# yknishidate/single-file-vulkan-pathtracing

Hardware: AMD Instinct MI355X
Metric: Mrays/s, Cornell Box 1920x1080 @ 8 bounces (ms/frame in ms_per_step) (higher is better)
Workload: dtype f32; 1 GPU; C2: CornellBox-Original.obj 1920x1080, 32 spp/frame x 771 frames, 8 bounces, fused pipeline (library default); pipeline=fused

## Files before the change

single-file-vulkan-pathtracing_amd/csrc/aov.hip:

```cpp
#include "wavefront_host.h"

#include <algorithm>

#define PT_EXTEND_TEMPLATES_ONLY
#include "extend_kernel.h"

namespace {
using namespace ptw;

struct AovConst {
    ptm::Camera cam;
    float tmin, tmax;
    uint32_t width, height, spp;
    FastDiv div_spp;
    uint32_t cull_on;
    int32_t cull[4];
};
struct AovPlanes {
    float *albedo, *normal, *emission, *depth, *alpha;
    uint2 *id;
};
constexpr size_t AOV_RAY_BYTES = sizeof(float4) + sizeof(float2) + sizeof(float4) + sizeof(uint32_t);
constexpr size_t AOV_MAX_CHUNK_RAYS = (size_t)1 << 26;
constexpr uint32_t AOV_NEXT_TILE = 32;

__device__ __forceinline__ void tile_pixel(const uint32_t *__restrict__ tiles, uint32_t pix, uint32_t &px, uint32_t &py)
{
    const uint32_t g = tiles[pix >> 6];
    px = (g & 0xFFFFu) * 8u + (pix & 7u);
    py = (g >> 16) * 8u + ((pix >> 3) & 7u);
}

struct Guide {
    float ar, ag, ab, nx, ny, nz, er, eg, eb, d, a;
};
__device__ __forceinline__ void guide_add(Guide &g, const Guide &v)
{
    g.ar = g.ar + v.ar; g.ag = g.ag + v.ag; g.ab = g.ab + v.ab;
    g.nx = g.nx + v.nx; g.ny = g.ny + v.ny; g.nz = g.nz + v.nz;
    g.er = g.er + v.er; g.eg = g.eg + v.eg; g.eb = g.eb + v.eb;
    g.d = g.d + v.d; g.a = g.a + v.a;
}
__device__ __forceinline__ float blend1(float sum, float spp, float old, bool first, float ff, float f1)
{
    return ptm::fdiv(ptm::fdiv(sum, spp) + (first ? 0.f : old) * ff, f1);
}
__device__ __forceinline__ void guide_blend(Guide &acc, const Guide &sum, float spp, int32_t frame)
{
    const float ff = (float)frame, f1 = (float)(frame + 1);
    const bool first = frame == 0;
    acc.ar = blend1(sum.ar, spp, acc.ar, first, ff, f1); acc.ag = blend1(sum.ag, spp, acc.ag, first, ff, f1); acc.ab = blend1(sum.ab, spp, acc.ab, first, ff, f1);
    acc.nx = blend1(sum.nx, spp, acc.nx, first, ff, f1); acc.ny = blend1(sum.ny, spp, acc.ny, first, ff, f1); acc.nz = blend1(sum.nz, spp, acc.nz, first, ff, f1);
    acc.er = blend1(sum.er, spp, acc.er, first, ff, f1); acc.eg = blend1(sum.eg, spp, acc.eg, first, ff, f1); acc.eb = blend1(sum.eb, spp, acc.eb, first, ff, f1);
    acc.d = blend1(sum.d, spp, acc.d, first, ff, f1); acc.a = blend1(sum.a, spp, acc.a, first, ff, f1);
}
__device__ __forceinline__ Guide guide_load(const AovPlanes &pl, size_t pix)
{
    Guide g;
    g.ar = pl.albedo[3 * pix + 0]; g.ag = pl.albedo[3 * pix + 1]; g.ab = pl.albedo[3 * pix + 2];
    g.nx = pl.normal[3 * pix + 0]; g.ny = pl.normal[3 * pix + 1]; g.nz = pl.normal[3 * pix + 2];
    g.er = pl.emission[3 * pix + 0]; g.eg = pl.emission[3 * pix + 1]; g.eb = pl.emission[3 * pix + 2];
    g.d = pl.depth[pix]; g.a = pl.alpha[pix];
    return g;
}
__device__ __forceinline__ void guide_store(const AovPlanes &pl, size_t pix, const Guide &g)
{
    pl.albedo[3 * pix + 0] = g.ar; pl.albedo[3 * pix + 1] = g.ag; pl.albedo[3 * pix + 2] = g.ab;
    pl.normal[3 * pix + 0] = g.nx; pl.normal[3 * pix + 1] = g.ny; pl.normal[3 * pix + 2] = g.nz;
    pl.emission[3 * pix + 0] = g.er; pl.emission[3 * pix + 1] = g.eg; pl.emission[3 * pix + 2] = g.eb;
    pl.depth[pix] = g.d; pl.alpha[pix] = g.a;
}

__global__ __launch_bounds__(TB) void k_aov_generate(AovConst ac, const uint32_t *__restrict__ tiles, uint32_t n_rays, int32_t frame,
                                                     float4 *__restrict__ rayA, float2 *__restrict__ rayB, uint32_t *__restrict__ count)
{
    for (uint32_t r = blockIdx.x * TB + threadIdx.x; r < n_rays; r += gridDim.x * TB) {
        const uint32_t pix = ac.div_spp.div(r), s = r - pix * ac.spp;
        uint32_t px, py;
        tile_pixel(tiles, pix, px, py);
        uint32_t seed = ptm::make_seed(px, py, s, frame, ac.spp);
        ptm::f3 org, dir;
        ptm::primary_ray(ac.cam, px, py, seed, org, dir);
        ptm::st_stream<true>(rayA + r, make_float4(org.x, org.y, org.z, dir.x));
        ptm::st_stream<true>(rayB + r, make_float2(dir.y, dir.z));
    }
    if (blockIdx.x == 0 && threadIdx.x == 0) *count = n_rays;
}

template <bool INST>
__global__ __launch_bounds__(TB) void k_aov_reduce(AovConst ac, const uint32_t *__restrict__ tiles, uint32_t n_pix, int32_t frame, int last_frame,
                                                   const float4 *__restrict__ hit, const uint32_t *__restrict__ hit_inst,
                                                   const float4 *__restrict__ tri4, const float4 *__restrict__ rec64,
                                                   const float *__restrict__ faces, const float4 *__restrict__ inst6,
                                                   const float4 *__restrict__ inst_frame, const uint32_t *__restrict__ inst_id, uint32_t n_tris,
                                                   AovPlanes planes, unsigned long long *stats, unsigned long long n_valid_rays)
{
    if (blockIdx.x == 0 && threadIdx.x == 0 && stats) atomicAdd(stats, n_valid_rays);
    const uint32_t pix = blockIdx.x * TB + threadIdx.x;
    if (pix >= n_pix) return;
    uint32_t px, py;
    tile_pixel(tiles, pix, px, py);
    if (px >= ac.width || py >= ac.height) return;
    Guide sum = {};
    uint2 id = make_uint2(PT_MISS, PT_MISS);
    for (uint32_t s = 0; s < ac.spp; s++) {
        const size_t r = (size_t)pix * ac.spp + s;
        const float4 h = ptm::ld_stream<true>(hit + r);
        const uint32_t pos = __float_as_uint(h.x);
        Guide v = {};
        if (pos != PT_MISS) {
            const uint32_t prim = __float_as_uint(tri4[3 * (size_t)pos].w);
            const float *f = faces + 6 * (size_t)prim;
            ptm::f3 nrm = { rec64[4 * (size_t)pos + 0].w, rec64[4 * (size_t)pos + 1].w, rec64[4 * (size_t)pos + 2].w };
            uint32_t inst = 0u;
            if (INST) {
                const uint32_t ip = hit_inst[r];
                inst = inst_id[ip];
                if (inst_frame) {
                    const float4 f0 = inst_frame[2 * ((size_t)ip * n_tris + pos)];
                    nrm = { f0.x, f0.y, f0.z };
                } else {
                    const float4 i0 = inst6[6 * (size_t)ip + 3], i1 = inst6[6 * (size_t)ip + 4], i2 = inst6[6 * (size_t)ip + 5];
                    const float nx = (i0.x * nrm.x + i1.x * nrm.y) + i2.x * nrm.z;
                    const float ny = (i0.y * nrm.x + i1.y * nrm.y) + i2.y * nrm.z;
                    const float nz = (i0.z * nrm.x + i1.z * nrm.y) + i2.z * nrm.z;
                    const float l = ptm::fsqrt((nx * nx + ny * ny) + nz * nz);
                    nrm = { ptm::fdiv(nx, l), ptm::fdiv(ny, l), ptm::fdiv(nz, l) };
                }
            }
            v = { f[0], f[1], f[2], nrm.x, nrm.y, nrm.z, f[3], f[4], f[5], h.y, 1.0f };
            if (s == 0u) id = make_uint2(prim, inst);
        }
        guide_add(sum, v);
    }
    const size_t o = (size_t)py * ac.width + px;
    Guide acc = {};
    if (frame != 0) acc = guide_load(planes, o);
    guide_blend(acc, sum, (float)ac.spp, frame);
    guide_store(planes, o, acc);
    if (last_frame) planes.id[o] = id;
}

constexpr int AOV_START_IDLE = 16;
#ifndef PT_AOV_WAVES
#define PT_AOV_WAVES 4
#endif
template <bool PAIRS>
__global__ __launch_bounds__(TB, PT_AOV_WAVES) void k_aov_fused(AovConst ac_arg, const uint32_t *__restrict__ tiles, uint32_t n_tiles, int32_t frame0, uint32_t n_frames,
                                                  const float4 *__restrict__ g_wide, const float4 *__restrict__ g_tri4,
                                                  const float4 *__restrict__ g_shade4, const float *__restrict__ g_faces, uint32_t n_wide,
                                                  uint32_t n_tris, int lds_stack, AovPlanes planes_arg, uint32_t *next_tile,
                                                  unsigned long long *stats)
{
    const AovConst ac = ptm::own_sgprs(ac_arg);
    const AovPlanes planes = ptm::own_sgprs(planes_arg);
    constexpr uint32_t LEAF_BIT = C14_LEAF, DONE = C14_DONE;
    extern __shared__ __attribute__((aligned(16))) char smem[];
    float4 *s_wide = reinterpret_cast<float4 *>(smem + (size_t)lds_stack * TB * sizeof(uint32_t));
    float4 *s_tri = s_wide + LDS_NODE_F4 * (size_t)n_wide;
    float4 *s_rec = s_tri + 9 * (size_t)n_tris;
    lds_stage_nodes<TB, true>(s_wide, g_wide, n_wide);
    lds_stage_tris<TB>(s_tri, g_tri4, n_tris);
    for (uint32_t pos = threadIdx.x; pos < n_tris; pos += TB) {
        const float4 n = g_shade4[3 * (size_t)pos];
        const float prim_bits = g_tri4[3 * (size_t)pos].w;
        const float *f = g_faces + 6 * (size_t)__float_as_uint(prim_bits);
        s_rec[3 * pos + 0] = make_float4(n.x, n.y, n.z, prim_bits);
        s_rec[3 * pos + 1] = make_float4(f[0], f[1], f[2], f[3]);
        s_rec[3 * pos + 2] = make_float4(f[4], f[5], 0.f, 0.f);
    }
    __syncthreads();
    const float4 *wide = s_wide, *tri4 = s_tri;
    lds_u32 *my_stack32 = (lds_u32 *)reinterpret_cast<uint32_t *>(smem) + threadIdx.x;
    const int lane = threadIdx.x & 63;
    const float tmin = ac.tmin, tmax = ac.tmax;
    const float fspp = (float)ac.spp;
    unsigned long long n_rays_wave = 0, n_cull_wave = 0;

    for (;;) {
        uint32_t t = 0;
        if (lane == 0) t = atomicAdd(next_tile, 1u);
        t = (uint32_t)__builtin_amdgcn_readfirstlane((int)t);
        if (t >= n_tiles) break;
        uint32_t px, py;
        tile_pixel(tiles, t * 64u + (uint32_t)lane, px, py);
        const bool valid = px < ac.width && py < ac.height;
        const uint32_t o = py * ac.width + px;
        const bool culled = ac.cull_on && ((int32_t)px < ac.cull[0] || (int32_t)px > ac.cull[2] || (int32_t)py < ac.cull[1] || (int32_t)py > ac.cull[3]);
        n_rays_wave += (unsigned long long)__popcll(__ballot(valid)) * ac.spp * n_frames;
        n_cull_wave += (unsigned long long)__popcll(__ballot(valid && culled)) * ac.spp * n_frames;
        for (uint32_t k = 0; k < n_frames; k++) {
            const int32_t frame = frame0 + (int32_t)k;
            Guide sum = {};
            uint32_t s = valid && !culled ? 0u : ac.spp;
            bool have = false;
            ptm::f3 inv{}, invf{}, on{}, of{}, orgp{};
            ptm::RayPre pre{};
            uint32_t ax = 0, ay = 0, az = 0, tri_base = 0;
            float best_t = tmax, best_V = 0.f, best_W = 0.f, best_det = 1.f;
            uint32_t best_pos = PT_MISS, best_prim = PT_MISS;
            uint32_t cur = DONE;
            int sp = 0;
            auto pop = [&]() -> uint32_t {
                while (sp > 0) {
                    sp--;
                    const uint32_t e = my_stack32[sp * TB];
                    if (__uint_as_float(e & 0xFFFFC000u) <= best_t) return e & 0x3FFFu;
                }
                return DONE;
            };
            for (;;) {
                const bool wants = !have && s < ac.spp;
                const int n_idle = __popcll(__ballot(wants)), n_have = __popcll(__ballot(have));
                if (n_idle == 0 && n_have == 0) break;
                if (wants && (n_idle >= AOV_START_IDLE || n_have == 0)) {
                    uint32_t seed = ptm::make_seed(px, py, s, frame, ac.spp);
                    ptm::f3 org, dir;
                    ptm::primary_ray(ac.cam, px, py, seed, org, dir);
                    pre = ptm::ray_setup<PAIRS>(org, dir);
                    inv = { ptm::safe_inv(dir.x), ptm::safe_inv(dir.y), ptm::safe_inv(dir.z) };
                    slab_setup(org, inv, invf, on, of);
                    ax = inv.x < 0.f ? 48u : 0u; ay = inv.y < 0.f ? 48u : 0u; az = inv.z < 0.f ? 48u : 0u;
                    tri_base = (uint32_t)pre.kz * 3u * n_tris;
                    orgp = { ptm::sel3(pre.kz, org.y, org.z, org.x), ptm::sel3(pre.kz, org.z, org.x, org.y), ptm::sel3(pre.kz, org.x, org.y, org.z) };
                    best_t = tmax; best_V = 0.f; best_W = 0.f; best_det = 1.f;
                    best_pos = PT_MISS; best_prim = PT_MISS;
                    cur = 0u;
                    sp = 0;
                    have = true;
                }
                bool do_node = have && !(cur & LEAF_BIT);
                const int n_walk = __popcll(__ballot(have));
                while (do_node) {
                    cur = compact_node_step<TB>(wide, cur, inv, invf, on, of, ax, ay, az, tmin, best_t, my_stack32, sp, pop);
                    do_node = !(cur & LEAF_BIT);
                    if (__popcll(__ballot(do_node)) * 6 < n_walk) break;
                }
                if (have) {
                    if (cur != DONE && (cur & LEAF_BIT)) {
                        const uint32_t first = cur & 0x7FFu;
                        if (PAIRS) {
                            const bool two = ((cur >> 11) & 3u) != 0u;
                            ptl::pair_leaf_test(tri4, (size_t)tri_base + 3 * (size_t)first, two, first, pre, orgp, tmin, tmax,
                                                [&](float t_, float V, float W, float det, uint32_t pos, uint32_t) {
                                                    ptl::closer_single_level(tri4, tri_base, t_, V, W, det, pos, best_t, best_V, best_W, best_det, best_pos);
                                                },
                                                [] {});
                        } else {
                            const uint32_t cnt = ((cur >> 11) & 3u) + 1u;
                            for (uint32_t j = 0; j < cnt; j++) {
                                const uint32_t pos = first + j;
                                const size_t ti = (size_t)tri_base + 3 * (size_t)pos;
                                const float4 a = tri4[ti + 0], b = tri4[ti + 1], c = tri4[ti + 2];
                                float t_, V, W, det;
                                if (ptm::tri_test_perm(pre, orgp, { a.x, a.y, a.z }, { b.x, b.y, b.z }, { c.x, c.y, c.z }, tmin, tmax, t_, V, W, det, nullptr)) {
                                    const uint32_t prim = __float_as_uint(a.w);
                                    if (t_ < best_t || (t_ == best_t && prim < best_prim)) {
                                        best_t = t_; best_V = V; best_W = W; best_det = det; best_pos = pos; best_prim = prim;
                                    }
                                }
                            }
                        }
                        cur = pop();
                    }
                    if (cur == DONE) {
                        Guide v = {};
                        if (best_pos != PT_MISS) {
                            const float4 r0 = s_rec[3 * best_pos + 0], r1 = s_rec[3 * best_pos + 1], r2 = s_rec[3 * best_pos + 2];
                            v = { r1.x, r1.y, r1.z, r0.x, r0.y, r0.z, r1.w, r2.x, r2.y, best_t, 1.0f };
                            if (s == 0u && k + 1u == n_frames) planes.id[o] = make_uint2(__float_as_uint(r0.w), 0u);
                        } else if (s == 0u && k + 1u == n_frames) {
                            planes.id[o] = make_uint2(PT_MISS, PT_MISS);
                        }
                        guide_add(sum, v);
                        s++;
                        have = false;
                    }
                }
            }
            if (valid && culled && k + 1u == n_frames) planes.id[o] = make_uint2(PT_MISS, PT_MISS);
            if (valid) {
                Guide acc = {};
                if (frame != 0) acc = guide_load(planes, o);
                guide_blend(acc, sum, fspp, frame);
                guide_store(planes, o, acc);
            }
        }
    }
    if (lane == 0 && n_rays_wave && stats) atomicAdd(stats, n_rays_wave);
    if (lane == 0 && n_cull_wave && stats) atomicAdd(stats + 19, n_cull_wave);
}

pt_status ensure_tiles(pt_film *f, uint32_t rank, uint32_t world)
{
    pt_film::Aov &a = f->aov;
    if (a.d_tiles && a.rank == rank && a.world == world) return PT_OK;
    std::vector<uint32_t> tiles;
    std::vector<uint64_t> prefix;
    const uint64_t valid = pt_rank_tiles(f->w, f->h, rank, world, &tiles, &prefix);
    const size_t held = a.d_tiles ? sizeof(uint32_t) * std::max<size_t>(a.n_tiles, 1) : 0;
    a.n_tiles = 0;
    const pt_status rc = pt_scratch_alloc(f->ctx, "guide-buffer workspace", { pt_buf_of(a.d_tiles, sizeof(uint32_t) * std::max<size_t>(tiles.size(), 1)) }, &a.bytes, held);
    if (rc != PT_OK) return rc;
    if (!tiles.empty()) PT_HIP(f->ctx, hipMemcpy(a.d_tiles, tiles.data(), sizeof(uint32_t) * tiles.size(), hipMemcpyHostToDevice));
    a.rank = rank; a.world = world; a.n_tiles = (uint32_t)tiles.size(); a.valid_pixels = valid;
    a.h_valid.swap(prefix);
    return PT_OK;
}

pt_status ensure_count(pt_film *f)
{
    pt_film::Aov &a = f->aov;
    if (a.d_count) return PT_OK;
    return pt_scratch_alloc(f->ctx, "guide-buffer workspace", { pt_buf_of(a.d_count, sizeof(uint32_t) * 64) }, &a.bytes, 0);
}

pt_status ensure_rays(pt_film *f, size_t rays)
{
    pt_film::Aov &a = f->aov;
    if (rays <= a.cap_rays) return PT_OK;
    const size_t held = a.cap_rays * AOV_RAY_BYTES;
    a.cap_rays = 0;
    const pt_status rc = pt_scratch_alloc(f->ctx, "guide-buffer workspace", { pt_buf_of(a.d_rayA, sizeof(float4) * rays), pt_buf_of(a.d_rayB, sizeof(float2) * rays),
                                                                              pt_buf_of(a.d_hit, sizeof(float4) * rays), pt_buf_of(a.d_hit_inst, sizeof(uint32_t) * rays) }, &a.bytes, held);
    if (rc == PT_OK) a.cap_rays = rays;
    return rc;
}

AovPlanes planes_of(const pt_film *f)
{
    const pt_film::Aov &a = f->aov;
    return { static_cast<float *>(a.plane[PT_AOV_ALBEDO]), static_cast<float *>(a.plane[PT_AOV_NORMAL]), static_cast<float *>(a.plane[PT_AOV_EMISSION]),
             static_cast<float *>(a.plane[PT_AOV_DEPTH]), static_cast<float *>(a.plane[PT_AOV_ALPHA]), static_cast<uint2 *>(a.plane[PT_AOV_ID]) };
}

struct AovFusedPlan { size_t smem = 0; int grid = 0; bool pairs = false; };
using AovFusedFn = decltype(&k_aov_fused<true>);
AovFusedFn pick_aov_fused(bool pairs) { return pairs ? k_aov_fused<true> : k_aov_fused<false>; }
pt_status plan_aov_fused(pt_scene *s, const pt_params *p, const ExtendPlan &pl, AovFusedPlan &fp)
{
    pt_ctx *ctx = s->ctx;
    const size_t smem = pl.smem + sizeof(float4) * 3 * (size_t)s->n_tris;
    if (s->n_inst || p->extend != PT_EXTEND_AUTO || pl.variant != PT_EXTEND_LDS || pl.spill || !(p->tmin > 0.f) || smem > 64 * 1024) {
        ctx->err = "pt_render_aov: PT_PIPELINE_FUSED is for single-level scenes whose BVH4 and triangles live in LDS (the compact kernels' class: <= 24 KB, "
                   "stack bound <= 16), tmin > 0 and params.extend = PT_EXTEND_AUTO";
        return PT_ERR_UNSUPPORTED;
    }
    fp.smem = smem;
    fp.pairs = pl.pairs;
    int per_cu = 0;
    const pt_status rc = ptw_prepare_kernel(ctx, reinterpret_cast<const void *>(pick_aov_fused(pl.pairs)), TB, smem, &per_cu);
    fp.grid = ctx->num_cus * per_cu;
    return rc;
}

pt_status render_aov_fused(pt_scene *s, pt_film *f, const pt_params *p, const ExtendPlan &pl, const AovFusedPlan &fp, const AovConst &ac)
{
    pt_ctx *ctx = s->ctx;
    pt_film::Aov &a = f->aov;
    hipStream_t st = ctx->stream;
    if (a.n_tiles == 0) return PT_OK;
    PT_HIP(ctx, hipMemsetAsync(a.d_count + AOV_NEXT_TILE, 0, sizeof(uint32_t), st));
    const int grid = (int)std::min<uint32_t>((uint32_t)fp.grid, (a.n_tiles + TB / 64 - 1) / (TB / 64));
    hipLaunchKernelGGL(pick_aov_fused(fp.pairs), dim3(grid), dim3(TB), (uint32_t)fp.smem, st, ac, a.d_tiles, a.n_tiles, p->frame, p->frame_count, s->d_wide, s->d_tri4,
                       s->d_shade4, s->d_faces, s->n_wide, s->n_tris, pl.lds_stack, planes_of(f), a.d_count + AOV_NEXT_TILE, ctx->d_stats);
    PT_HIP(ctx, hipGetLastError());
    ctx->stats.launches_extend++;
    return PT_OK;
}

pt_status render_aov_queues(pt_scene *s, pt_film *f, const pt_params *p, const ExtendPlan &pl, const AovConst &ac)
{
    pt_ctx *ctx = s->ctx;
    pt_film::Aov &a = f->aov;
    hipStream_t st = ctx->stream;
    if (a.n_tiles == 0) return PT_OK;
    const float4 *inst_frame = nullptr;
    if (s->n_inst && ctx->tune.inst_frames != 0) {
        const pt_status rcf = ptb_ensure_inst_frames(s);
        if (rcf != PT_OK) return rcf;
        inst_frame = s->d_inst_frame;
    }
    const size_t tile_rays = 64 * (size_t)p->spp_per_frame;
    const size_t held = f->work.bytes + (a.bytes - a.cap_rays * AOV_RAY_BYTES);
    size_t fit_rays = AOV_MAX_CHUNK_RAYS;
    if (ctx->mem_budget) fit_rays = std::min(fit_rays, ctx->mem_budget > held ? (ctx->mem_budget - held) / AOV_RAY_BYTES : 0);
    size_t chunk_tiles = std::min<size_t>(a.n_tiles, fit_rays / tile_rays);
    if (chunk_tiles == 0) {
        if (ctx->mem_budget && tile_rays * AOV_RAY_BYTES + held > ctx->mem_budget) {
            ctx->err = "guide-buffer workspace exceeds the memory budget (" + std::to_string((held + tile_rays * AOV_RAY_BYTES) >> 20) + " MB wanted for one tile, " +
                       std::to_string(ctx->mem_budget >> 20) + " MB allowed)";
            return PT_ERR_OOM;
        }
        chunk_tiles = 1;
    }
    pt_status rc = ensure_rays(f, chunk_tiles * tile_rays);
    if (rc != PT_OK) return rc;
    const AovPlanes planes = planes_of(f);
    const float4 *tri4 = pl.bvh8 ? s->d_tri4_8 : s->d_tri4, *rec64 = pl.bvh8 ? s->d_shade64_8 : s->d_shade64;
    for (uint32_t k = 0; k < p->frame_count; k++) {
        const int32_t frame = p->frame + (int32_t)k;
        const int last = k + 1 == p->frame_count ? 1 : 0;
        for (uint32_t t0 = 0; t0 < a.n_tiles; t0 += (uint32_t)chunk_tiles) {
            const uint32_t nt = std::min<uint32_t>((uint32_t)chunk_tiles, a.n_tiles - t0);
            const uint32_t n_pix = nt * 64u, n_rays = n_pix * p->spp_per_frame;
            const unsigned long long valid = a.h_valid[t0 + nt] - a.h_valid[t0];
            const int grid_g = (int)std::min<uint32_t>((n_rays + TB - 1) / TB, (uint32_t)ctx->num_cus * 32u);
            k_aov_generate<<<grid_g, TB, 0, st>>>(ac, a.d_tiles + t0, n_rays, frame, a.d_rayA, a.d_rayB, a.d_count);
            ptw_launch_extend(pl, s, a.d_rayA, a.d_rayB, a.d_hit, a.d_hit_inst, a.d_count, nullptr, nullptr, p->tmin, p->tmax, false, false, st);
            const int grid_r = (int)((n_pix + TB - 1) / TB);
            if (s->n_inst)
                k_aov_reduce<true><<<grid_r, TB, 0, st>>>(ac, a.d_tiles + t0, n_pix, frame, last, a.d_hit, a.d_hit_inst, tri4, rec64, s->d_faces, s->d_inst6, inst_frame,
                                                          s->d_tlas_prim_of, s->n_tris, planes, ctx->d_stats, valid * p->spp_per_frame);
            else
                k_aov_reduce<false><<<grid_r, TB, 0, st>>>(ac, a.d_tiles + t0, n_pix, frame, last, a.d_hit, nullptr, tri4, rec64, s->d_faces, nullptr, nullptr, nullptr,
                                                           s->n_tris, planes, ctx->d_stats, valid * p->spp_per_frame);
            PT_HIP(ctx, hipGetLastError());
            ctx->stats.launches_extend++;
            ctx->stats.launches_other += 2;
        }
    }
    return PT_OK;
}

}

size_t pta_plane_bytes(const pt_film *f, uint32_t which)
{
    const size_t n = (size_t)f->w * f->h;
    return which <= PT_AOV_EMISSION ? sizeof(float) * 3 * n : which <= PT_AOV_ALPHA ? sizeof(float) * n : sizeof(uint32_t) * 2 * n;
}

pt_status pta_enable(pt_film *f, void *const *device_planes)
{
    pt_ctx *ctx = f->ctx;
    pt_film::Aov &a = f->aov;
    if (a.enabled) { ctx->err = "the film already has guide buffers"; return PT_ERR_INVALID_ARG; }
    for (uint32_t k = 0; k < PT_AOV_COUNT; k++) {
        void *ext = device_planes ? device_planes[k] : nullptr;
        a.own[k] = ext == nullptr;
        a.plane[k] = ext;
        if (!ext) {
            const hipError_t e = hipMalloc(&a.plane[k], pta_plane_bytes(f, k));
            if (e != hipSuccess) {
                (void)hipGetLastError();
                a.plane[k] = nullptr;
                ctx->err = std::string("hipMalloc: ") + hipGetErrorString(e);
                pta_free(f);
                return PT_ERR_OOM;
            }
        }
    }
    a.enabled = true;
    const pt_status rc = pta_clear(f, ctx->stream);
    if (rc != PT_OK) { pta_free(f); return rc; }
    PT_HIP(ctx, hipStreamSynchronize(ctx->stream));
    return PT_OK;
}

pt_status pta_clear(pt_film *f, hipStream_t st)
{
    if (!f->aov.enabled) return PT_OK;
    for (uint32_t k = 0; k < PT_AOV_COUNT; k++) PT_HIP(f->ctx, hipMemsetAsync(f->aov.plane[k], 0, pta_plane_bytes(f, k), st));
    return PT_OK;
}

void pta_free(pt_film *f)
{
    pt_film::Aov &a = f->aov;
    for (uint32_t k = 0; k < PT_AOV_COUNT; k++) {
        if (a.own[k] && a.plane[k]) (void)hipFree(a.plane[k]);
        a.plane[k] = nullptr;
        a.own[k] = false;
    }
    pt_scratch_free({ pt_buf_of(a.d_tiles), pt_buf_of(a.d_rayA), pt_buf_of(a.d_rayB), pt_buf_of(a.d_hit), pt_buf_of(a.d_hit_inst), pt_buf_of(a.d_count) },
                    &a.bytes, a.bytes);
    a = pt_film::Aov{};
}

pt_status pta_render(pt_scene *s, pt_film *f, const pt_params *p)
{
    pt_ctx *ctx = s->ctx;
    pt_status rc = s->broken ? ptb_repair(s) : PT_OK;
    if (rc != PT_OK) return rc;
    if (!f->aov.enabled) { ctx->err = "the film has no guide buffers: pt_film_enable_aov first"; return PT_ERR_INVALID_ARG; }
    if (p->width != f->w || p->height != f->h) { ctx->err = "params width/height differ from the film's"; return PT_ERR_INVALID_ARG; }
    if (p->world == 0 || p->rank >= p->world) { ctx->err = "rank/world invalid"; return PT_ERR_INVALID_ARG; }
    if (p->spp_per_frame == 0 || p->spp_per_frame > 0xFFFFu) { ctx->err = "spp_per_frame must be in 1..65535"; return PT_ERR_INVALID_ARG; }
    if (p->frame < 0 || p->frame_count == 0) { ctx->err = "frame must be >= 0 and frame_count >= 1"; return PT_ERR_INVALID_ARG; }
    if (p->pipeline > PT_PIPELINE_AUTO) { ctx->err = "unknown pipeline"; return PT_ERR_UNSUPPORTED; }
    if (p->pipeline == PT_PIPELINE_WAVEFRONT_NEE) { ctx->err = "pt_render_aov: the guides do not depend on the estimator (PT_PIPELINE_WAVEFRONT, _FUSED or _AUTO)"; return PT_ERR_UNSUPPORTED; }
    if (p->flags & ~(uint32_t)PT_FLAG_NEE) { ctx->err = "pt_render_aov takes no flag but PT_FLAG_NEE (ignored): blocking, not instrumented"; return PT_ERR_UNSUPPORTED; }
    ExtendPlan pl;
    rc = ptw_plan_extend(s, p->extend, pl);
    if (rc != PT_OK) return rc;
    AovFusedPlan fp;
    bool fused = false;
    if (p->pipeline != PT_PIPELINE_WAVEFRONT) {
        const std::string keep = ctx->err;
        rc = plan_aov_fused(s, p, pl, fp);
        if (rc == PT_OK) fused = true;
        else if (p->pipeline == PT_PIPELINE_FUSED) return rc;
        else ctx->err = keep;
    }
    ctx->stats.pipeline = fused ? PT_PIPELINE_FUSED : PT_PIPELINE_WAVEFRONT;
    rc = ensure_tiles(f, p->rank, p->world);
    if (rc == PT_OK) rc = ensure_count(f);
    if (rc != PT_OK) return rc;
    AovConst ac{};
    ac.cam = ptw_camera(p);
    ac.tmin = p->tmin; ac.tmax = p->tmax;
    ac.width = p->width; ac.height = p->height; ac.spp = p->spp_per_frame;
    ac.div_spp.init(p->spp_per_frame);
    if (fused && ctx->tune.cull != 0) {
        int32_t rect[4];
        ptw_subject_rect(s, p, rect);
        ac.cull_on = rect[2] >= rect[0] && rect[3] >= rect[1] ? 1u : 0u;
        std::copy(rect, rect + 4, ac.cull);
    }
    hipStream_t st = ctx->stream;
    PT_HIP(ctx, hipEventRecord(ctx->ev_a, st));
    rc = fused ? render_aov_fused(s, f, p, pl, fp, ac) : render_aov_queues(s, f, p, pl, ac);
    if (rc != PT_OK) { (void)hipStreamSynchronize(st); return rc; }
    PT_HIP(ctx, hipEventRecord(ctx->ev_b, st));
    PT_HIP(ctx, hipStreamSynchronize(st));
    PT_HIP(ctx, hipGetLastError());
    float ms = 0.f;
    PT_HIP(ctx, hipEventElapsedTime(&ms, ctx->ev_a, ctx->ev_b));
    ctx->stats.ms_total += ms;
    ctx->stats.paths += f->aov.valid_pixels * p->spp_per_frame * p->frame_count;
    return PT_OK;
}
```

single-file-vulkan-pathtracing_amd/csrc/extend_inst.h:

```cpp
#pragma once
#include "extend_kernel.h"

namespace {

constexpr uint32_t EXIT_MARK = 0x7FFFFFFFu;

template <bool COUNT, bool LDS_BLAS, bool SHADOW = false>
__global__ __launch_bounds__(TB) void k_extend_inst(const float4 *__restrict__ tlas, const float4 *__restrict__ g_blas,
                                                    const float4 *__restrict__ g_tri4, uint32_t n_blas_wide,
                                                    uint32_t n_tris, const float4 *__restrict__ inst6,
                                                    const uint32_t *__restrict__ inst_id, const float4 *__restrict__ rayA,
                                                    const float2 *__restrict__ rayB, float4 *__restrict__ hit,
                                                    uint32_t *__restrict__ hit_inst, const uint32_t *__restrict__ count_in,
                                                    uint32_t *count_zero, unsigned long long *stats,
                                                    uint2 *__restrict__ spill, uint32_t spill_stride, int refill_min_idle,
                                                    float tmin, float tmax, int raw_hit, const float *__restrict__ ray_tmax)
{
    extern __shared__ __attribute__((aligned(16))) char smem[];
    uint2 *stack = reinterpret_cast<uint2 *>(smem);
    const float4 *blas = g_blas;
    const float4 *tri4 = g_tri4;
    if (LDS_BLAS) {
        float4 *s_blas = reinterpret_cast<float4 *>(smem + (size_t)LDS_STACK * TB * sizeof(uint2));
        float4 *s_tri = s_blas + LDS_NODE_F4 * (size_t)n_blas_wide;
        lds_stage_nodes<TB, false>(s_blas, g_blas, n_blas_wide);
        lds_stage_tris<TB>(s_tri, g_tri4, n_tris);
        __syncthreads();
        blas = s_blas;
        tri4 = s_tri;
    }
    const uint32_t n = *count_in;
    if (blockIdx.x == 0 && threadIdx.x == 0) {
        if (count_zero) *count_zero = 0u;
        if (stats) atomicAdd(stats, (unsigned long long)n);
    }
    lds_u64 *my_stack = (lds_u64 *)reinterpret_cast<unsigned long long *>(stack) + threadIdx.x;
    unsigned long long *my_spill = reinterpret_cast<unsigned long long *>(spill) + (size_t)blockIdx.x * TB + threadIdx.x;
    const float INF = __builtin_inff();
    const int lane = threadIdx.x & 63;
    const unsigned long long lt = (1ull << lane) - 1ull;

    bool have = false, exhausted = false, in_blas = false;
    uint32_t q = 0;
    ptm::f3 org_w{}, dir_w{}, inv_w{};
    ptm::f3 inv{}, invf{}, on{}, of{}, orgp{};
    uint32_t tri_base = 0;
    uint32_t ax = 0, ay = 0, az = 0;
    ptm::RayPre pre{};
    float best_t = tmax, best_V = 0.f, best_W = 0.f, best_det = 1.f;
    uint32_t best_pos = PT_MISS, best_prim = PT_MISS, best_ipos = PT_MISS, best_iid = PT_MISS;
    uint32_t cur = SENTINEL, cur_ipos = 0, cur_iid = 0;
    float cur_t = 0.f;
    int sp = 0;
    unsigned long long c_nodes = 0, c_tris = 0;
    const uint32_t wave_base = (blockIdx.x * (TB / 64) + (threadIdx.x >> 6)) * 64u;
    const uint32_t wave_stride = gridDim.x * TB;
    uint32_t cursor = 0;

    auto push = [&](uint32_t w, float t) {
        const unsigned long long e = stack_entry(w, t);
        if (sp < LDS_STACK) my_stack[sp * TB] = e;
        else my_spill[(size_t)(sp - LDS_STACK) * spill_stride] = e;
        sp++;
    };
    auto pop = [&]() -> uint32_t {
        while (sp > 0) {
            sp--;
            unsigned long long e64;
            if (sp < LDS_STACK) e64 = my_stack[sp * TB];
            else e64 = my_spill[(size_t)(sp - LDS_STACK) * spill_stride];
            const uint2 e = make_uint2((uint32_t)e64, (uint32_t)(e64 >> 32));
            if (e.x == EXIT_MARK) {
                inv = inv_w;
                slab_setup(org_w, inv_w, invf, on, of);
                ax = inv.x < 0.f ? 48u : 0u;
                ay = inv.y < 0.f ? 48u : 0u;
                az = inv.z < 0.f ? 48u : 0u;
                in_blas = false;
                continue;
            }
            if (__uint_as_float(e.y) <= best_t) {
                cur_t = __uint_as_float(e.y);
                return e.x;
            }
        }
        return SENTINEL;
    };

    for (;;) {
        const unsigned long long idle = __ballot(!have);
        const int n_idle = __popcll(idle);
        if (!exhausted && n_idle >= refill_min_idle) {
            if (!have) {
                const uint32_t v = cursor + (uint32_t)__popcll(idle & lt);
                const uint32_t qq = (v >> 6) * wave_stride + wave_base + (v & 63u);
                if (qq < n) {
                    q = qq;
                    const float4 ra = rayA[q];
                    const float2 rb = rayB[q];
                    org_w = { ra.x, ra.y, ra.z };
                    dir_w = { ra.w, rb.x, rb.y };
                    inv_w = { ptm::safe_inv(dir_w.x), ptm::safe_inv(dir_w.y), ptm::safe_inv(dir_w.z) };
                    inv = inv_w;
                    slab_setup(org_w, inv_w, invf, on, of);
                    ax = inv.x < 0.f ? 48u : 0u;
                    ay = inv.y < 0.f ? 48u : 0u;
                    az = inv.z < 0.f ? 48u : 0u;
                    in_blas = false;
                    best_t = SHADOW ? ray_tmax[q] : tmax; best_V = 0.f; best_W = 0.f; best_det = 1.f;
                    best_pos = PT_MISS; best_prim = PT_MISS; best_ipos = PT_MISS; best_iid = PT_MISS;
                    cur = 0u;
                    cur_t = tmin;
                    sp = 0;
                    have = true;
                }
            }
            cursor += (uint32_t)n_idle;
            exhausted = (cursor >> 6) * wave_stride + wave_base >= n;
        }
        if (__ballot(have) == 0ull) break;

        while (have && !(cur & PT_LEAF)) {
            float4 nx, fx, ny, fy, nz, fz, cw;
            if (LDS_BLAS && in_blas) {
                const char *nd = reinterpret_cast<const char *>(blas + LDS_NODE_F4 * (size_t)cur);
                nx = PT_F4(nd + ax); fx = PT_F4(nd - ax + 48); ny = PT_F4(nd + ay + 16); fy = PT_F4(nd - ay + 64);
                nz = PT_F4(nd + az + 32); fz = PT_F4(nd - az + 80); cw = PT_F4(nd + 96);
            } else {
                const char *nd = reinterpret_cast<const char *>((LDS_BLAS ? tlas : (in_blas ? g_blas : tlas)) + 8 * (size_t)cur);
                nx = PT_F4(nd + ax); fx = PT_F4(nd - ax + 48); ny = PT_F4(nd + ay + 16); fy = PT_F4(nd - ay + 64);
                nz = PT_F4(nd + az + 32); fz = PT_F4(nd - az + 80); cw = PT_F4(nd + 96);
            }
            if (COUNT) c_nodes++;
            float t0, t1, t2, t3;
            uint32_t w0 = __float_as_uint(cw.x), w1 = __float_as_uint(cw.y), w2 = __float_as_uint(cw.z),
                     w3 = __float_as_uint(cw.w);
            PT_SLAB4(t0, x)
            PT_SLAB4(t1, y)
            PT_SLAB4(t2, z)
            PT_SLAB4(t3, w)
#define PT_CSWAP(TA, WA, TB_, WB)                            \
    {                                                        \
        const bool sw = TB_ < TA;                            \
        const float ta = sw ? TB_ : TA, tb = sw ? TA : TB_;  \
        const uint32_t wa = sw ? WB : WA, wb = sw ? WA : WB; \
        TA = ta; TB_ = tb; WA = wa; WB = wb;                 \
    }
            PT_CSWAP(t0, w0, t1, w1)
            PT_CSWAP(t2, w2, t3, w3)
            PT_CSWAP(t0, w0, t2, w2)
            PT_CSWAP(t1, w1, t3, w3)
            PT_CSWAP(t1, w1, t2, w2)
#undef PT_CSWAP
            if (t3 < INF) push(w3, t3);
            if (t2 < INF) push(w2, t2);
            if (t1 < INF) push(w1, t1);
            if (t0 < INF) { cur = w0; cur_t = t0; }
            else cur = pop();
        }
        constexpr int ENTER_MIN = 16;
        const int n_enter = __popcll(__ballot(have && cur != SENTINEL && !in_blas));
        const bool others = __ballot(have && cur != SENTINEL && in_blas) != 0ull;
        const bool do_enter = n_enter >= ENTER_MIN || !others;
        if (have) {
            if (cur != SENTINEL && (in_blas || do_enter)) {
                const uint32_t first = cur & 0x0FFFFFFFu, cnt = ((cur >> 28) & 7u) + 1u;
                if (in_blas) {
                    if (COUNT) c_tris += cnt;
                    for (uint32_t k = 0; k < cnt; k++) {
                        const uint32_t pos = first + k;
                        const size_t ti = LDS_BLAS ? (size_t)tri_base + 3 * (size_t)pos : 3 * (size_t)pos;
                        const float4 a = tri4[ti + 0], b = tri4[ti + 1], c = tri4[ti + 2];
                        float t, V, W, det;
                        const bool th = LDS_BLAS
                            ? ptm::tri_test_perm(pre, orgp, { a.x, a.y, a.z }, { b.x, b.y, b.z }, { c.x, c.y, c.z }, tmin, tmax, t, V, W, det)
                            : ptm::tri_test(pre, { a.x, a.y, a.z }, { b.x, b.y, b.z }, { c.x, c.y, c.z }, tmin, tmax, t, V, W, det);
                        if (th) {
                            const uint32_t prim = __float_as_uint(a.w);
                            if (t < best_t || (t == best_t && (cur_iid < best_iid || (cur_iid == best_iid && prim < best_prim)))) {
                                best_t = t; best_V = V; best_W = W; best_det = det; best_pos = pos; best_prim = prim;
                                best_ipos = cur_ipos; best_iid = cur_iid;
                                if (SHADOW) sp = 0;
                            }
                        }
                    }
                    cur = pop();
                } else {
                    for (uint32_t k = cnt - 1u; k >= 1u; k--) push(PT_LEAF | (first + k), cur_t);
                    cur_ipos = first;
                    cur_iid = inst_id[first];
                    const float4 r0 = inst6[6 * (size_t)first + 3], r1 = inst6[6 * (size_t)first + 4],
                                 r2 = inst6[6 * (size_t)first + 5];
                    const ptm::f3 oo = { ((r0.x * org_w.x + r0.y * org_w.y) + r0.z * org_w.z) + r0.w,
                                         ((r1.x * org_w.x + r1.y * org_w.y) + r1.z * org_w.z) + r1.w,
                                         ((r2.x * org_w.x + r2.y * org_w.y) + r2.z * org_w.z) + r2.w };
                    const ptm::f3 od = { (r0.x * dir_w.x + r0.y * dir_w.y) + r0.z * dir_w.z,
                                         (r1.x * dir_w.x + r1.y * dir_w.y) + r1.z * dir_w.z,
                                         (r2.x * dir_w.x + r2.y * dir_w.y) + r2.z * dir_w.z };
                    inv = { ptm::safe_inv(od.x), ptm::safe_inv(od.y), ptm::safe_inv(od.z) };
                    slab_setup(oo, inv, invf, on, of);
                    ax = inv.x < 0.f ? 48u : 0u;
                    ay = inv.y < 0.f ? 48u : 0u;
                    az = inv.z < 0.f ? 48u : 0u;
                    pre = ptm::ray_setup(oo, od);
                    if (LDS_BLAS) {
                        tri_base = (uint32_t)pre.kz * 3u * n_tris;
                        orgp = { ptm::sel3(pre.kz, oo.y, oo.z, oo.x), ptm::sel3(pre.kz, oo.z, oo.x, oo.y),
                                 ptm::sel3(pre.kz, oo.x, oo.y, oo.z) };
                    }
                    push(EXIT_MARK, 0.f);
                    in_blas = true;
                    cur = 0u;
                    cur_t = tmin;
                }
            }
            if (cur == SENTINEL) {
                const bool miss = best_pos == PT_MISS;
                hit[q] = raw_hit ? make_float4(__uint_as_float(best_pos), best_V, best_W, best_det)
                                 : make_float4(__uint_as_float(best_pos), miss ? 0.f : best_t,
                                               miss ? 0.f : ptm::fdiv(best_V, best_det), miss ? 0.f : ptm::fdiv(best_W, best_det));
                if (!SHADOW) hit_inst[q] = best_ipos;
                have = false;
            }
        }
    }
    if (COUNT) {
        for (int o = 32; o > 0; o >>= 1) {
            c_nodes += __shfl_xor(c_nodes, o, 64);
            c_tris += __shfl_xor(c_tris, o, 64);
        }
        if (lane == 0 && stats) {
            atomicAdd(stats + 2, c_nodes);
            atomicAdd(stats + 3, c_tris);
        }
    }
}

}
```

single-file-vulkan-pathtracing_amd/csrc/extend_kernel.h:

```cpp
#pragma once
#include "pt_internal.h"
#include "pt_math.h"
#include "pair_leaf.h"
#include "lds_scene.h"

#include <hip/hip_ext.h>

namespace {

constexpr int LDS_STACK = 8;
typedef __attribute__((address_space(3))) unsigned long long lds_u64;
typedef __attribute__((address_space(3))) uint32_t lds_u32;
__device__ __forceinline__ unsigned long long stack_entry(uint32_t w, float t)
{
    return (unsigned long long)w | ((unsigned long long)__float_as_uint(t) << 32);
}

#define PT_F4(P) (*reinterpret_cast<const float4 *>(P))
#define PT_NODE_LOAD(ND)                                                                                 \
    const char *nb_ = reinterpret_cast<const char *>(ND);                                                \
    const float4 nx = PT_F4(nb_ + ax), fx = PT_F4(nb_ - ax + 48), ny = PT_F4(nb_ + ay + 16),             \
                 fy = PT_F4(nb_ - ay + 64), nz = PT_F4(nb_ + az + 32), fz = PT_F4(nb_ - az + 80),        \
                 cw = PT_F4(nb_ + 96);
#define PT_SLAB4(T, C)                                                                                           \
    {                                                                                                            \
        const float tn = fmaxf(fmaxf(__builtin_fmaf(nx.C, inv.x, on.x), __builtin_fmaf(ny.C, inv.y, on.y)),      \
                               max_raw_s(__builtin_fmaf(nz.C, inv.z, on.z), tmin));                              \
        const float tf = fminf(fminf(__builtin_fmaf(fx.C, invf.x, of.x), __builtin_fmaf(fy.C, invf.y, of.y)),    \
                               min_raw(__builtin_fmaf(fz.C, invf.z, of.z), best_t));                             \
        T = tn <= tf ? tn : INF;                                                                                 \
    }
__device__ __forceinline__ float max_raw_s(float a, float uniform_b)
{
    float r;
    asm("v_max_f32_e32 %0, %1, %2" : "=v"(r) : "s"(uniform_b), "v"(a));
    return r;
}
__device__ __forceinline__ float min_raw(float a, float b)
{
    float r;
    asm("v_min_f32_e32 %0, %1, %2" : "=v"(r) : "v"(a), "v"(b));
    return r;
}

template <int STRIDE, class Pop>
__device__ __forceinline__ uint32_t compact_node_step(const float4 *wide, uint32_t cur, const ptm::f3 &inv, const ptm::f3 &invf, const ptm::f3 &on,
                                                      const ptm::f3 &of, uint32_t ax, uint32_t ay, uint32_t az, float tmin, float best_t,
                                                      lds_u32 *my_stack32, int &sp, Pop &&pop)
{
    const float INF = __builtin_inff();
    float t0, t1, t2, t3;
    const float4 *nd = reinterpret_cast<const float4 *>(reinterpret_cast<const char *>(wide) + __umul24(cur, 16u * LDS_NODE_F4));
    PT_NODE_LOAD(nd)
    const uint32_t w0 = __float_as_uint(cw.x), w1 = __float_as_uint(cw.y), w2 = __float_as_uint(cw.z), w3 = __float_as_uint(cw.w);
    PT_SLAB4(t0, x)
    PT_SLAB4(t1, y)
    PT_SLAB4(t2, z)
    PT_SLAB4(t3, w)
    uint32_t k0 = (__float_as_uint(t0) & 0xFFFFC000u) | w0, k1 = (__float_as_uint(t1) & 0xFFFFC000u) | w1,
             k2 = (__float_as_uint(t2) & 0xFFFFC000u) | w2, k3 = (__float_as_uint(t3) & 0xFFFFC000u) | w3;
#define PT_KSWAP(A, B) { const uint32_t lo_ = min(A, B), hi_ = max(A, B); A = lo_; B = hi_; }
    PT_KSWAP(k0, k1)
    PT_KSWAP(k2, k3)
    PT_KSWAP(k0, k2)
    PT_KSWAP(k1, k3)
    PT_KSWAP(k1, k2)
#undef PT_KSWAP
    constexpr uint32_t KINF = 0x7F800000u;
    if (k3 < KINF) { my_stack32[sp * STRIDE] = k3; sp++; }
    if (k2 < KINF) { my_stack32[sp * STRIDE] = k2; sp++; }
    if (k1 < KINF) { my_stack32[sp * STRIDE] = k1; sp++; }
    return k0 < KINF ? (k0 & 0x3FFFu) : pop();
}
__device__ __forceinline__ void slab_setup(const ptm::f3 org, const ptm::f3 inv, ptm::f3 &invf, ptm::f3 &on, ptm::f3 &of)
{
    const float ox = -(org.x * inv.x), oy = -(org.y * inv.y), oz = -(org.z * inv.z);
    const float px = fabsf(ox) * 0x1p-21f, py = fabsf(oy) * 0x1p-21f, pz = fabsf(oz) * 0x1p-21f;
    on = { ox - px, oy - py, oz - pz };
    of = { (ox + px) * 1.0000004f, (oy + py) * 1.0000004f, (oz + pz) * 1.0000004f };
    invf = { inv.x * 1.0000004f, inv.y * 1.0000004f, inv.z * 1.0000004f };
}
struct NormBox { float cx, cy, cz, sx, sy, sz, rsx, rsy, rsz; };
inline NormBox norm_box(const float *c, const float *s, const float *rs) { return { c[0], c[1], c[2], s[0], s[1], s[2], rs[0], rs[1], rs[2] }; }
inline NormBox norm_box_blas(const pt_scene *s) { return norm_box(s->norm_c, s->norm_s, s->norm_rs); }
inline NormBox norm_box_tlas(const pt_scene *s) { return norm_box(s->tlas_norm_c, s->tlas_norm_s, s->tlas_norm_rs); }
#define PT_MIXH(DST, REG, HI, INVC, ONC) \
    asm("v_fma_mix_f32 %0, %1, %2, %3 op_sel:[" #HI ",0,0] op_sel_hi:[1,0,0]" : "=v"(DST) : "v"(REG), "v"(INVC), "v"(ONC))
#define PT_SLAB4H(T, REGC, HI)                                                                      \
    {                                                                                               \
        float nxv, nyv, nzv, fxv, fyv, fzv;                                                         \
        PT_MIXH(nxv, hnx.REGC, HI, inv.x, on.x); PT_MIXH(nyv, hny.REGC, HI, inv.y, on.y);           \
        PT_MIXH(nzv, hnz.REGC, HI, inv.z, on.z); PT_MIXH(fxv, hfx.REGC, HI, invf.x, of.x);          \
        PT_MIXH(fyv, hfy.REGC, HI, invf.y, of.y); PT_MIXH(fzv, hfz.REGC, HI, invf.z, of.z);         \
        const float tn = fmaxf(fmaxf(nxv, nyv), max_raw_s(nzv, tmin));                              \
        const float tf = fminf(fminf(fxv, fyv), min_raw(fzv, best_t));                              \
        T = tn <= tf ? tn : INF;                                                                    \
    }
#ifndef PT_HBM_SELECT_BFI
#define PT_HBM_SELECT_BFI 1
#endif
#if PT_HBM_SELECT_BFI
#define PT_BFI(M, A, B) (((M) & (A)) | (~(M) & (B)))
#else
#define PT_BFI(M, A, B) ((M) ? (A) : (B))
#endif
#ifndef PT_EXTEND_WAVES
#define PT_EXTEND_WAVES 7
#endif
constexpr int REFILL_MIN_IDLE = 16;

template <bool LDS_SCENE, bool COUNT, bool SPILL, bool PAIRS = false, bool REC64 = false>
__device__ __forceinline__ void extend_body(const float4 *__restrict__ g_wide, const uint2 *__restrict__ g_wide16,
                                               NormBox nb, const float4 *__restrict__ g_tri4,
                                               uint32_t n_wide, uint32_t n_tris, const float4 *__restrict__ rayA,
                                               const float2 *__restrict__ rayB, float4 *__restrict__ hit,
                                               const uint32_t *__restrict__ count_in, uint32_t *count_zero,
                                               unsigned long long *stats, uint2 *__restrict__ spill,
                                               uint32_t spill_stride, int refill_vote, float tmin, float tmax,
                                               int lds_stack, int raw_hit, const uint32_t *__restrict__ perm,
                                               const float *__restrict__ ray_tmax, const float4 *__restrict__ g_rec64 = nullptr)
{
    const int refill_min_idle = refill_vote & 0xFF, tri_enter = (refill_vote >> 8) & 0xFF;
    constexpr bool VOTE = !LDS_SCENE;
    constexpr int VOTE_NODE_NUM = 1, VOTE_NODE_DEN = 1;
    constexpr bool COMPACT = LDS_SCENE && !SPILL;
    static_assert(!PAIRS || COMPACT, "pair leaves are implemented for the compact LDS kernel");
    static_assert(!REC64 || (!LDS_SCENE && SPILL), "64-B triangle records are the vote-scheduled HBM kernel's");
    constexpr uint32_t LEAF_BIT = COMPACT ? C14_LEAF : PT_LEAF;
    constexpr uint32_t DONE = COMPACT ? C14_DONE : SENTINEL;

    extern __shared__ __attribute__((aligned(16))) char smem[];
    uint2 *stack = reinterpret_cast<uint2 *>(smem);
    const float4 *wide = g_wide;
    const float4 *tri4 = g_tri4;
    if (LDS_SCENE) {
        float4 *s_wide = reinterpret_cast<float4 *>(smem + (size_t)lds_stack * TB * (COMPACT ? sizeof(uint32_t) : sizeof(uint2)));
        float4 *s_tri = s_wide + LDS_NODE_F4 * (size_t)n_wide;
        lds_stage_nodes<TB, COMPACT>(s_wide, g_wide, n_wide);
        lds_stage_tris<TB>(s_tri, g_tri4, n_tris);
        __syncthreads();
        wide = s_wide;
        tri4 = s_tri;
    }
    const uint32_t n = *count_in;
    if (blockIdx.x == 0 && threadIdx.x == 0) {
        if (count_zero) *count_zero = 0u;
        if (stats) atomicAdd(stats, (unsigned long long)n);
    }
    lds_u64 *my_stack = (lds_u64 *)reinterpret_cast<unsigned long long *>(stack) + threadIdx.x;
    lds_u32 *my_stack32 = (lds_u32 *)reinterpret_cast<uint32_t *>(stack) + threadIdx.x;
    unsigned long long *my_spill = reinterpret_cast<unsigned long long *>(spill) + (size_t)blockIdx.x * TB + threadIdx.x;
    const float INF = __builtin_inff();
    const int lane = threadIdx.x & 63;
    const unsigned long long lt = (1ull << lane) - 1ull;

    bool have = false, exhausted = false;
    uint32_t q = 0;
    const uint32_t wave_base = (blockIdx.x * (TB / 64) + (threadIdx.x >> 6)) * 64u;
    const uint32_t wave_stride = gridDim.x * TB;
    uint32_t cursor = 0;
    ptm::f3 inv{}, invf{}, on{}, of{}, orgp{};
    ptm::RayPre pre{};
    uint32_t ax = 0, ay = 0, az = 0;
    uint32_t tri_base = 0;
    float best_t = tmax, best_V = 0.f, best_W = 0.f, best_det = 1.f;
    uint32_t best_pos = PT_MISS, best_prim = PT_MISS;
    uint32_t cur = DONE;
    int sp = 0;
    unsigned long long c_nodes = 0, c_tris = 0, c_node_steps = 0, c_tri_steps = 0;
    unsigned long long c_refills = 0, c_pops = 0, c_hit_blocks = 0, c_finishes = 0, c_iters = 0;
    unsigned long long c_leaf_lanes = 0, c_pop_lanes = 0, c_hit_lanes = 0;
#define PT_COUNT_WAVE(C) \
    if (COUNT && lane == __ffsll((long long)__ballot(1)) - 1) (C)++

    auto push = [&](uint32_t w, float t) {
        if (COMPACT) {
            my_stack32[sp * TB] = (__float_as_uint(t) & 0xFFFFC000u) | w;
            sp++;
            return;
        }
        const unsigned long long e = stack_entry(w, t);
        if (!SPILL || sp < lds_stack) my_stack[sp * TB] = e;
        else my_spill[(size_t)(sp - lds_stack) * spill_stride] = e;
        sp++;
    };
    auto pop = [&]() -> uint32_t {
        if (COMPACT) {
            while (sp > 0) {
                PT_COUNT_WAVE(c_pops);
                if (COUNT) c_pop_lanes++;
                sp--;
                const uint32_t e = my_stack32[sp * TB];
                if (__uint_as_float(e & 0xFFFFC000u) <= best_t) return e & 0x3FFFu;
            }
            return DONE;
        }
        while (sp > 0) {
            PT_COUNT_WAVE(c_pops);
            if (COUNT) c_pop_lanes++;
            sp--;
            unsigned long long e;
            if (!SPILL || sp < lds_stack) e = my_stack[sp * TB];
            else e = my_spill[(size_t)(sp - lds_stack) * spill_stride];
            if (__uint_as_float((uint32_t)(e >> 32)) <= best_t) return (uint32_t)e;
        }
        return DONE;
    };

    for (;;) {
        PT_COUNT_WAVE(c_iters);
        const unsigned long long idle = __ballot(!have);
        const int n_idle = __popcll(idle);
        if (!exhausted && n_idle >= refill_min_idle) {
            if (!have) {
                const uint32_t v = cursor + (PAIRS ? __builtin_amdgcn_mbcnt_hi((uint32_t)(idle >> 32), __builtin_amdgcn_mbcnt_lo((uint32_t)idle, 0u))
                                                       : (uint32_t)__popcll(idle & lt));
                const uint32_t qq = (v >> 6) * wave_stride + wave_base + (v & 63u);
                if (qq < n) {
                    PT_COUNT_WAVE(c_refills);
                    q = (!LDS_SCENE && perm) ? perm[qq] : qq;
                    const float4 ra = ptm::ld_stream<false>(rayA + q);
                    const float2 rb = ptm::ld_stream<false>(rayB + q);
                    const ptm::f3 org = { ra.x, ra.y, ra.z };
                    const ptm::f3 dir = { ra.w, rb.x, rb.y };
                    pre = ptm::ray_setup<!(LDS_SCENE && !PAIRS)>(org, dir);
                    inv = { ptm::safe_inv(dir.x), ptm::safe_inv(dir.y), ptm::safe_inv(dir.z) };
                    if (LDS_SCENE) {
                        slab_setup(org, inv, invf, on, of);
                    } else {
                        const ptm::f3 orgn = { (org.x - nb.cx) * nb.rsx, (org.y - nb.cy) * nb.rsy, (org.z - nb.cz) * nb.rsz };
                        inv = { inv.x * nb.sx, inv.y * nb.sy, inv.z * nb.sz };
                        slab_setup(orgn, inv, invf, on, of);
                    }
                    ax = inv.x < 0.f ? (LDS_SCENE ? 48u : 24u) : 0u;
                    ay = inv.y < 0.f ? (LDS_SCENE ? 48u : 24u) : 0u;
                    az = inv.z < 0.f ? (LDS_SCENE ? 48u : 24u) : 0u;
                    if (LDS_SCENE) {
                        tri_base = (uint32_t)pre.kz * 3u * n_tris;
                        orgp = { ptm::sel3(pre.kz, org.y, org.z, org.x), ptm::sel3(pre.kz, org.z, org.x, org.y),
                                 ptm::sel3(pre.kz, org.x, org.y, org.z) };
                    }
                    best_t = ray_tmax ? ray_tmax[q] : tmax; best_V = 0.f; best_W = 0.f; best_det = 1.f;
                    best_pos = PT_MISS; best_prim = PT_MISS;
                    cur = 0u;
                    sp = 0;
                    have = true;
                }
            }
            cursor += (uint32_t)n_idle;
            exhausted = (cursor >> 6) * wave_stride + wave_base >= n;
        }
        if (__ballot(have) == 0ull) break;

        bool do_leaf = true;
        bool do_node = have && !(cur & LEAF_BIT);
        const int n_have = __popcll(__ballot(have));
        if (VOTE) {
            const bool want_leaf = have && (cur & LEAF_BIT) && cur != DONE;
            const int nn = __popcll(__ballot(do_node)), nl = __popcll(__ballot(want_leaf));
            const bool node_turn = nn * VOTE_NODE_NUM >= nl * VOTE_NODE_DEN && !(tri_enter && nl >= tri_enter);
            do_node = do_node && node_turn;
            do_leaf = !node_turn;
        }
        while (do_node) {
            if (COUNT) {
                c_nodes++;
                if (lane == __ffsll((long long)__ballot(1)) - 1) c_node_steps++;
            }
            if constexpr (LDS_SCENE && COMPACT) {
                cur = compact_node_step<TB>(wide, cur, inv, invf, on, of, ax, ay, az, tmin, best_t, my_stack32, sp, pop);
            } else {
            float t0, t1, t2, t3;
            uint32_t w0, w1, w2, w3;
            if (LDS_SCENE) {
                const float4 *nd = reinterpret_cast<const float4 *>(reinterpret_cast<const char *>(wide) + __umul24(cur, 16u * LDS_NODE_F4));
                PT_NODE_LOAD(nd)
                w0 = __float_as_uint(cw.x); w1 = __float_as_uint(cw.y); w2 = __float_as_uint(cw.z); w3 = __float_as_uint(cw.w);
                PT_SLAB4(t0, x)
                PT_SLAB4(t1, y)
                PT_SLAB4(t2, z)
                PT_SLAB4(t3, w)
            } else {
                const char *nb_ = reinterpret_cast<const char *>(g_wide16) + 64 * (size_t)cur;
                const uint4 q0 = *reinterpret_cast<const uint4 *>(nb_), q1 = *reinterpret_cast<const uint4 *>(nb_ + 16),
                            q2 = *reinterpret_cast<const uint4 *>(nb_ + 32);
                const uint4 cw = *reinterpret_cast<const uint4 *>(nb_ + 48);
                const uint32_t mx = ax ? 0xFFFFFFFFu : 0u, my = ay ? 0xFFFFFFFFu : 0u, mz = az ? 0xFFFFFFFFu : 0u;
                const uint2 hnx = { PT_BFI(mx, q1.z, q0.x), PT_BFI(mx, q1.w, q0.y) }, hfx = { PT_BFI(mx, q0.x, q1.z), PT_BFI(mx, q0.y, q1.w) };
                const uint2 hny = { PT_BFI(my, q2.x, q0.z), PT_BFI(my, q2.y, q0.w) }, hfy = { PT_BFI(my, q0.z, q2.x), PT_BFI(my, q0.w, q2.y) };
                const uint2 hnz = { PT_BFI(mz, q2.z, q1.x), PT_BFI(mz, q2.w, q1.y) }, hfz = { PT_BFI(mz, q1.x, q2.z), PT_BFI(mz, q1.y, q2.w) };
                w0 = cw.x; w1 = cw.y; w2 = cw.z; w3 = cw.w;
                PT_SLAB4H(t0, x, 0)
                PT_SLAB4H(t1, x, 1)
                PT_SLAB4H(t2, y, 0)
                PT_SLAB4H(t3, y, 1)
            }
            {
#define PT_CSWAP(TA, WA, TB_, WB)                            \
    {                                                        \
        const bool sw = TB_ < TA;                            \
        const float ta = sw ? TB_ : TA, tb = sw ? TA : TB_;  \
        const uint32_t wa = sw ? WB : WA, wb = sw ? WA : WB; \
        TA = ta; TB_ = tb; WA = wa; WB = wb;                 \
    }
            PT_CSWAP(t0, w0, t1, w1)
            PT_CSWAP(t2, w2, t3, w3)
            PT_CSWAP(t0, w0, t2, w2)
            PT_CSWAP(t1, w1, t3, w3)
            PT_CSWAP(t1, w1, t2, w2)
#undef PT_CSWAP
            if (t3 < INF) push(w3, t3);
            if (t2 < INF) push(w2, t2);
            if (t1 < INF) push(w1, t1);
            cur = t0 < INF ? w0 : pop();
            }
            }
            do_node = !VOTE && !(cur & LEAF_BIT);
            if (!VOTE) {
                const int n_cont = __popcll(__ballot(do_node));
                if (n_cont * 6 < n_have) break;
            }
        }
        if (have) {
            if (PAIRS) {
                if (cur != DONE && (cur & LEAF_BIT)) {
                    const uint32_t first = cur & 0x7FFu;
                    const bool two = ((cur >> 11) & 3u) != 0u;
                    if (COUNT) { c_tris += two ? 2u : 1u; c_leaf_lanes++; }
                    PT_COUNT_WAVE(c_tri_steps);
                    ptl::pair_leaf_test(tri4, (size_t)tri_base + 3 * (size_t)first, two, first, pre, orgp, tmin, tmax,
                                        [&](float t, float V, float W, float det, uint32_t pos, uint32_t) {
                                            if (ptl::closer_single_level(tri4, tri_base, t, V, W, det, pos, best_t, best_V, best_W, best_det, best_pos) && ray_tmax)
                                                sp = 0;
                                        },
                                        [&] {
                                            PT_COUNT_WAVE(c_hit_blocks);
                                            if (COUNT) c_hit_lanes++;
                                        });
                    cur = pop();
                }
            } else
            if (cur != DONE && (cur & LEAF_BIT) && (!VOTE || do_leaf)) {
                const uint32_t first = COMPACT ? (cur & 0x7FFu) : (cur & 0x0FFFFFFFu);
                const uint32_t cnt = (COMPACT ? ((cur >> 11) & 3u) : ((cur >> 28) & 7u)) + 1u;
                if (COUNT) c_tris += cnt;
                for (uint32_t k = 0; k < cnt; k++) {
                    if (COUNT && lane == __ffsll((long long)__ballot(1)) - 1) c_tri_steps++;
                    if (COUNT) c_leaf_lanes++;
                    const uint32_t pos = first + k;
                    const size_t ti = LDS_SCENE ? (size_t)tri_base + 3 * (size_t)pos : (REC64 ? 4 : 3) * (size_t)pos;
                    const float4 *tp = REC64 ? g_rec64 : tri4;
                    const float4 a = tp[ti + 0], b = tp[ti + 1], c = tp[ti + 2];
                    float t, V, W, det;
                    bool divided = false;
                    const bool th = LDS_SCENE
                        ? ptm::tri_test_perm(pre, orgp, { a.x, a.y, a.z }, { b.x, b.y, b.z }, { c.x, c.y, c.z }, tmin, tmax, t, V, W, det, COUNT ? &divided : nullptr)
                        : ptm::tri_test(pre, { a.x, a.y, a.z }, { b.x, b.y, b.z }, { c.x, c.y, c.z }, tmin, tmax, t, V, W, det, COUNT ? &divided : nullptr);
                    if (COUNT && divided) { PT_COUNT_WAVE(c_hit_blocks); c_hit_lanes++; }
                    if (th) {
                        if constexpr (REC64) {
                            bool closer = t < best_t;
                            if (!closer && t == best_t)
                                closer = best_pos == PT_MISS ||
                                         __float_as_uint(g_tri4[3 * (size_t)pos].w) < __float_as_uint(g_tri4[3 * (size_t)best_pos].w);
                            if (closer) {
                                best_t = t; best_V = V; best_W = W; best_det = det; best_pos = pos;
                                if (ray_tmax) sp = 0;
                            }
                        } else {
                        const uint32_t prim = __float_as_uint(a.w);
                        if (t < best_t || (t == best_t && prim < best_prim)) {
                            best_t = t; best_V = V; best_W = W; best_det = det; best_pos = pos; best_prim = prim;
                            if (ray_tmax) sp = 0;
                        }
                        }
                    }
                }
                cur = pop();
            }
            if (cur == DONE) {
                PT_COUNT_WAVE(c_finishes);
                const bool miss = best_pos == PT_MISS;
                ptm::st_stream<false>(hit + q, raw_hit ? make_float4(__uint_as_float(best_pos), best_V, best_W, best_det)
                                 : make_float4(__uint_as_float(best_pos), miss ? 0.f : best_t,
                                               miss ? 0.f : ptm::fdiv(best_V, best_det), miss ? 0.f : ptm::fdiv(best_W, best_det)));
                have = false;
            }
        }
    }
#undef PT_COUNT_WAVE
    if (COUNT) {
        for (int o = 32; o > 0; o >>= 1) {
            c_nodes += __shfl_xor(c_nodes, o, 64);
            c_tris += __shfl_xor(c_tris, o, 64);
            c_node_steps += __shfl_xor(c_node_steps, o, 64);
            c_tri_steps += __shfl_xor(c_tri_steps, o, 64);
            c_refills += __shfl_xor(c_refills, o, 64);
            c_pops += __shfl_xor(c_pops, o, 64);
            c_hit_blocks += __shfl_xor(c_hit_blocks, o, 64);
            c_finishes += __shfl_xor(c_finishes, o, 64);
            c_iters += __shfl_xor(c_iters, o, 64);
            c_leaf_lanes += __shfl_xor(c_leaf_lanes, o, 64);
            c_pop_lanes += __shfl_xor(c_pop_lanes, o, 64);
            c_hit_lanes += __shfl_xor(c_hit_lanes, o, 64);
        }
        if (lane == 0 && stats) {
            atomicAdd(stats + 2, c_nodes);
            atomicAdd(stats + 3, c_tris);
            atomicAdd(stats + 4, c_node_steps);
            atomicAdd(stats + 5, c_tri_steps);
            atomicAdd(stats + 8, c_refills);
            atomicAdd(stats + 9, c_pops);
            atomicAdd(stats + 10, c_hit_blocks);
            atomicAdd(stats + 11, c_finishes);
            atomicAdd(stats + 12, c_iters);
            atomicAdd(stats + 13, c_leaf_lanes);
            atomicAdd(stats + 14, c_pop_lanes);
            atomicAdd(stats + 15, c_hit_lanes);
        }
    }
}

#define PT_EXTEND_PARAMS                                                                                    \
    const float4 *__restrict__ g_wide, const uint2 *__restrict__ g_wide16, NormBox nb,                \
        const float4 *__restrict__ g_tri4, uint32_t n_wide, uint32_t n_tris, const float4 *__restrict__ rayA,       \
        const float2 *__restrict__ rayB, float4 *__restrict__ hit, const uint32_t *__restrict__ count_in,           \
        uint32_t *count_zero, unsigned long long *stats, uint2 *__restrict__ spill, uint32_t spill_stride,          \
        int refill_min_idle, float tmin, float tmax, int lds_stack, int raw_hit, const uint32_t *__restrict__ perm,       \
        const float *__restrict__ ray_tmax, const float4 *__restrict__ g_rec64
#define PT_EXTEND_ARGS                                                                                               \
    g_wide, g_wide16, nb, g_tri4, n_wide, n_tris, rayA, rayB, hit, count_in, count_zero, stats, spill, spill_stride, \
        refill_min_idle, tmin, tmax, lds_stack, raw_hit, perm, ray_tmax, g_rec64
template <bool LDS_SCENE, bool COUNT, bool SPILL, bool PAIRS = false, bool REC64 = false>
__global__ __launch_bounds__(TB) void k_extend(PT_EXTEND_PARAMS)
{
    extend_body<LDS_SCENE, COUNT, SPILL, PAIRS, REC64>(PT_EXTEND_ARGS);
}
#ifndef PT_EXTEND_TEMPLATES_ONLY
#define PT_EXTEND_ARGS_PLAIN                                                                                         \
    g_wide, g_wide16, nb, g_tri4, n_wide, n_tris, rayA, rayB, hit, count_in, count_zero, stats, spill, spill_stride, \
        refill_min_idle, tmin, tmax, lds_stack, raw_hit, nullptr, nullptr
__global__ __launch_bounds__(TB, PT_EXTEND_WAVES) void k_extend_lds7(PT_EXTEND_PARAMS)
{
    extend_body<true, false, false>(PT_EXTEND_ARGS_PLAIN);
}
__global__ __launch_bounds__(TB, PT_EXTEND_WAVES) void k_extend_lds7_sh(PT_EXTEND_PARAMS)
{
    extend_body<true, false, false>(PT_EXTEND_ARGS);
}
__global__ __launch_bounds__(TB, PT_EXTEND_WAVES) void k_extend_lds7p(PT_EXTEND_PARAMS)
{
    extend_body<true, false, false, true>(PT_EXTEND_ARGS_PLAIN);
}
__global__ __launch_bounds__(TB, PT_EXTEND_WAVES) void k_extend_lds7p_sh(PT_EXTEND_PARAMS)
{
    extend_body<true, false, false, true>(PT_EXTEND_ARGS);
}
#undef PT_EXTEND_ARGS_PLAIN
#endif
#undef PT_EXTEND_PARAMS
#undef PT_EXTEND_ARGS

}
```

single-file-vulkan-pathtracing_amd/csrc/extend_launch.hip:

```cpp
#include "wavefront_host.h"

#include <algorithm>

#include "extend_kernel.h"
#include "extend_inst16.h"
#include "extend_inst.h"

namespace {

using ExtendFn = decltype(&k_extend<true, false, true>);
ExtendFn pick_extend_lds(bool compact, bool pairs, bool count, bool shadow)
{
    if (!compact) return count ? k_extend<true, true, true> : k_extend<true, false, true>;
    if (count) return pairs ? k_extend<true, true, false, true> : k_extend<true, true, false>;
    if (pairs) return shadow ? k_extend_lds7p_sh : k_extend_lds7p;
    return shadow ? k_extend_lds7_sh : k_extend_lds7;
}
using ExtendInstFn = decltype(&k_extend_inst<false, false>);
ExtendInstFn pick_extend_inst(bool lds_blas, bool count, bool shadow)
{
    if (shadow) return lds_blas ? k_extend_inst<false, true, true> : k_extend_inst<false, false, true>;
    if (count) return lds_blas ? k_extend_inst<true, true> : k_extend_inst<true, false>;
    return lds_blas ? k_extend_inst<false, true> : k_extend_inst<false, false>;
}
using ExtendInst16Fn = decltype(&k_extend_inst16<false, false>);
ExtendInst16Fn pick_extend_inst16(bool pairs, bool count, bool shadow)
{
    if (shadow) return pairs ? k_extend_inst16<false, true, true> : k_extend_inst16<false, false, true>;
    if (count) return pairs ? k_extend_inst16<true, true> : k_extend_inst16<true, false>;
    return pairs ? k_extend_inst16<false, true> : k_extend_inst16<false, false>;
}

}

pt_status ptw_plan_extend(pt_scene *s, uint32_t want, ExtendPlan &pl)
{
    pt_ctx *ctx = s->ctx;
    if (want > PT_EXTEND_HBM8) { ctx->err = "unknown extend variant"; return PT_ERR_INVALID_ARG; }
    if (want == PT_EXTEND_FLAT_REMOVED) {
        ctx->err = "PT_EXTEND_FLAT (the brute-force loop, never AUTO) was removed in API version 5: every tree walk returns the brute-force closest hit";
        return PT_ERR_UNSUPPORTED;
    }
    if (s->broken) {
        const pt_status rcb = ptb_repair(s);
        if (rcb != PT_OK) return rcb;
    }
    const uint64_t ws4 = 64ull * (s->n_wide16t ? s->n_wide16t : s->n_wide) + 64ull * s->n_tris;
    const bool auto8_big = want == PT_EXTEND_AUTO && ctx->tune.hbm8 != 0 && ws4 > (1ull << 20) && s->n_tris > PT_SAH_MAX_TRIS;
    if ((want == PT_EXTEND_HBM8 || (want == PT_EXTEND_AUTO && ctx->tune.hbm8 == 1) || auto8_big) && !s->n_inst && !s->d_wide8) {
        const pt_status rc8 = ptb_ensure_wide8(s);
        if (rc8 != PT_OK) return rc8;
    }
    if (want == PT_EXTEND_HBM8 && (s->n_inst || !s->d_wide8)) { ctx->err = "no 8-wide nodes for this scene (instanced, or <= 2048 triangles)"; return PT_ERR_UNSUPPORTED; }
    if (s->n_inst) {
        if (want == PT_EXTEND_LDS) { ctx->err = "instanced scenes only have the HBM extend variant"; return PT_ERR_UNSUPPORTED; }
        pl.variant = PT_EXTEND_HBM;
        const size_t blas_bytes = lds_scene_bytes(s->n_wide, s->n_tris);
        pl.lds_scene = blas_bytes <= 24 * 1024;
        pl.smem = (size_t)LDS_STACK * TB * sizeof(uint2) + (pl.lds_scene ? blas_bytes : 0);
        int per_cu_i = 0;
        const pt_status rci = ptw_prepare_kernel(ctx, reinterpret_cast<const void *>(pick_extend_inst(pl.lds_scene, false, false)), TB, pl.smem, &per_cu_i);
        if (rci != PT_OK) return rci;
        pl.refill = 64;
        pl.refill = pt_tuned(ctx->tune.refill, pl.refill, 1, 64);
        pl.grid = ctx->num_cus * per_cu_i;
        pl.smem_inst_fallback = pl.smem; pl.grid_inst_fallback = pl.grid;
        const size_t smem16_scene = lds_scene16_bytes(s->n_wide, s->n_tris);
        const int lds16 = pt_tuned(ctx->tune.lds_stack, 16, 1, 32);
        pl.inst16 = s->d_tlas16 && s->d_wide16 && s->n_inst < 32768u && s->n_tlas16 < 32767u && s->n_wide < 32767u && s->n_tris <= 2047u &&
                    smem16_scene <= 24 * 1024 && ctx->tune.inst16 != 0;
        if (pl.inst16) {
            pl.lds_stack = lds16;
            const size_t tlas_lds_bytes = (size_t)pt_tuned(ctx->tune.tlas_lds_kb, 8, 0, 96) * 1024;
            pl.n_tlas_lds = (uint32_t)std::min<size_t>(s->n_tlas16, tlas_lds_bytes / lds_nodes16_bytes(1));
            pl.smem = (size_t)lds16 * TB * sizeof(uint32_t) + smem16_scene + lds_nodes16_bytes(pl.n_tlas_lds);
            int per16 = 0;
            const auto prepare16 = [&](bool count, bool shadow, int *per_cu) {
                return ptw_prepare_kernel(ctx, reinterpret_cast<const void *>(pick_extend_inst16(s->pair_leaves, count, shadow)), TB, pl.smem, per_cu);
            };
            pt_status rc16 = prepare16(true, false, nullptr);
            if (rc16 == PT_OK) rc16 = prepare16(false, true, nullptr);
            if (rc16 == PT_OK) rc16 = prepare16(false, false, &per16);
            if (rc16 != PT_OK) return rc16;
            per16 = pt_tuned(ctx->tune.inst16_blocks, std::min(per16, 4), 1, 8);
            pl.grid = ctx->num_cus * per16;
            pl.refill = pt_tuned(ctx->tune.refill, 48, 1, 64);
        }
        const uint32_t blas_bound = s->stack_need != 0xFFFFFFFFu ? s->stack_need + 1u : 3u * (s->height_tree / 2u + 1u);
        const uint32_t bound_i = 3u * (std::max(s->tlas_height / 2u + 1u, s->tlas16_levels)) + 4u + blas_bound + 2u;
        pl.spill_levels = bound_i > (uint32_t)LDS_STACK ? bound_i - (uint32_t)LDS_STACK : 0u;
        return ptw_reserve_spill(ctx, PT_MAX_PIPES * (size_t)std::max(pl.spill_levels, 1u) * (size_t)std::max(pl.grid, pl.grid_inst_fallback) * TB * sizeof(uint2));
    }
    const size_t scene_bytes = lds_scene_bytes(s->n_wide, s->n_tris);
    const bool auto8 = want == PT_EXTEND_AUTO && scene_bytes > 24 * 1024 && s->d_wide8 && (ctx->tune.hbm8 == 1 || auto8_big);
    if (want == PT_EXTEND_HBM8 || auto8) {
        pl.variant = PT_EXTEND_HBM8;
        pl.bvh8 = true;
        pl.lds_scene = false;
        const uint32_t bound8 = s->levels8 + 1u;
        pl.lds_stack = pt_tuned(ctx->tune.lds_stack, (int)std::min(std::max(bound8, 4u), 12u), 1, 32);
        pl.smem = (size_t)pl.lds_stack * TB * sizeof(uint2);
        const bool spills8 = bound8 > (uint32_t)pl.lds_stack;
        pl.waves7 = !spills8 && pl.lds_stack <= 10 &&
                    (ctx->tune.extend_blocks == 7 || (ctx->tune.extend_blocks < 0 && 64ull * s->n_wide8 + 64ull * s->n_tris > (256ull << 20)));
        int per_cu8 = 0;
        const pt_status rc8b = ptw_prepare_kernel(ctx, ptw_extend8_fn(false, spills8, pl.waves7), TB, pl.smem, &per_cu8);
        if (rc8b != PT_OK) return rc8b;
        pl.refill = pt_tuned(ctx->tune.refill, 12, 1, 64);
        pl.grid = ctx->num_cus * per_cu8;
        pl.spill_levels = bound8 > (uint32_t)pl.lds_stack ? bound8 - (uint32_t)pl.lds_stack : 0u;
        return ptw_reserve_spill(ctx, PT_MAX_PIPES * (size_t)std::max(pl.spill_levels, 1u) * (size_t)pl.grid * TB * sizeof(uint2));
    }
    if (want == PT_EXTEND_LDS && scene_bytes > 96 * 1024) { ctx->err = "scene does not fit LDS"; return PT_ERR_UNSUPPORTED; }
    pl.lds_scene = want == PT_EXTEND_LDS || (want == PT_EXTEND_AUTO && scene_bytes <= 24 * 1024);
    pl.variant = pl.lds_scene ? PT_EXTEND_LDS : PT_EXTEND_HBM;
    pl.lds_stack = pl.lds_scene ? LDS_STACK : 12;
    pl.spill = !(pl.lds_scene && s->stack_need <= 16u && s->n_tris <= 2047u && s->n_wide <= 8191u);
    if (!pl.spill) pl.lds_stack = (int)std::max(s->stack_need, 1u);
    pl.pairs = !pl.spill && s->pair_leaves && ctx->tune.pair_kernel != 0;
    pl.smem_wide_entries = (size_t)pl.lds_stack * TB * sizeof(uint2) + (pl.lds_scene ? scene_bytes : 0);
    pl.smem = pl.spill ? pl.smem_wide_entries : (size_t)pl.lds_stack * TB * sizeof(uint32_t) + scene_bytes;
    const auto kernel_of = [&](bool compact, bool count, bool shadow) {
        return pl.lds_scene ? reinterpret_cast<const void *>(pick_extend_lds(compact, pl.pairs, count, shadow)) : ptw_extend_hbm_fn(count, ctx->tune.rec64 != 0);
    };
    int per_cu = 0;
    pt_status rck = PT_OK;
    if (!pl.spill)
        for (const bool count : { false, true })
            if (rck == PT_OK) rck = ptw_prepare_kernel(ctx, kernel_of(false, count, false), TB, pl.smem_wide_entries);
    if (rck == PT_OK) rck = ptw_prepare_kernel(ctx, kernel_of(!pl.spill, true, false), TB, pl.smem);
    if (rck == PT_OK && !pl.spill) rck = ptw_prepare_kernel(ctx, kernel_of(true, false, true), TB, pl.smem);
    if (rck == PT_OK) rck = ptw_prepare_kernel(ctx, kernel_of(!pl.spill, false, false), TB, pl.smem, &per_cu);
    if (rck != PT_OK) return rck;
    per_cu = ptw_tuned_blocks(ctx, per_cu);
    pl.refill = pt_tuned(ctx->tune.refill, pl.lds_scene ? REFILL_MIN_IDLE : 32, 1, 64);
    pl.grid = ctx->num_cus * per_cu;
    pl.topdown4 = !pl.lds_scene && s->bvh4_builder != 1 && s->d_wide16t && ctx->tune.topdown4 != 0;
    const uint32_t bound = pl.topdown4 ? 3u * s->levels4t + 1u
                           : s->stack_need != 0xFFFFFFFFu ? s->stack_need + 1u : 3u * (s->height_tree / 2u + 1u) + 1u;
    pl.spill_levels = bound > (uint32_t)pl.lds_stack ? bound - (uint32_t)pl.lds_stack : 0u;
    return ptw_reserve_spill(ctx, PT_MAX_PIPES * (size_t)std::max(pl.spill_levels, 1u) * (size_t)pl.grid * TB * sizeof(uint2));
}

void ptw_launch_extend(const ExtendPlan &pl, pt_scene *s, const float4 *rayA, const float2 *rayB, float4 *hit, uint32_t *hit_inst,
                       const uint32_t *count_in, uint32_t *count_zero, unsigned long long *stats, float tmin, float tmax, bool count,
                       bool raw_hit, hipStream_t st, int pipe, hipEvent_t ev0, hipEvent_t ev1, const uint32_t *perm, const float *ray_tmax)
{
    const int raw = raw_hit ? 1 : 0;
    const size_t spill_off = (size_t)pipe * std::max(pl.spill_levels, 1u) * (size_t)pl.grid * TB;
    if (s->n_inst && pl.inst16 && tmin > 0.f) {
        uint32_t *sp32 = reinterpret_cast<uint32_t *>(reinterpret_cast<uint2 *>(s->ctx->d_spill) + (size_t)pipe * std::max(pl.spill_levels, 1u) * (size_t)std::max(pl.grid, pl.grid_inst_fallback) * TB);
        const uint32_t str = (uint32_t)pl.grid * TB;
        const int enter_min = pt_tuned(s->ctx->tune.enter_min, 16, 1, 64);
        const int leaf_min = pt_tuned(s->ctx->tune.leaf_min, 14, 1, 64);
        const int node_yield = pt_tuned(s->ctx->tune.node_yield, 6, 0, 64);
        hipExtLaunchKernelGGL(pick_extend_inst16(s->pair_leaves, count, ray_tmax != nullptr), dim3(pl.grid), dim3(TB), (uint32_t)pl.smem, st, ev0, ev1, 0u, s->d_tlas16,
                              norm_box_tlas(s), reinterpret_cast<const uint4 *>(s->d_wide16), norm_box_blas(s), s->d_tri4, s->n_wide, s->n_tris, s->d_inst6,
                              s->d_tlas_prim_of, rayA, rayB, hit, hit_inst, count_in, count_zero, stats, sp32, str, pl.refill, tmin,
                              tmax, raw, pl.lds_stack, enter_min, leaf_min, node_yield, pl.n_tlas_lds, ray_tmax);
        return;
    }
    if (s->n_inst) {
        const int grid_i = pl.inst16 ? pl.grid_inst_fallback : pl.grid;
        const size_t smem_i = pl.inst16 ? pl.smem_inst_fallback : pl.smem;
        uint2 *sp = reinterpret_cast<uint2 *>(s->ctx->d_spill) + (size_t)pipe * std::max(pl.spill_levels, 1u) * (size_t)std::max(pl.grid, pl.grid_inst_fallback) * TB;
        const uint32_t str = (uint32_t)grid_i * TB;
        hipExtLaunchKernelGGL(pick_extend_inst(pl.lds_scene, count, ray_tmax != nullptr), dim3(grid_i), dim3(TB), (uint32_t)smem_i, st, ev0, ev1, 0u, s->d_tlas_wide,
                              s->d_wide, s->d_tri4, s->n_wide, s->n_tris, s->d_inst6, s->d_tlas_prim_of, rayA, rayB, hit,
                              hit_inst, count_in, count_zero, stats, sp, str, pl.refill, tmin, tmax, raw, ray_tmax);
        return;
    }
    uint2 *spill = reinterpret_cast<uint2 *>(s->ctx->d_spill) + spill_off;
    const uint32_t stride = (uint32_t)pl.grid * TB;
    if (pl.bvh8) {
        const int tri_enter = pt_tuned(s->ctx->tune.tri_enter, 16, 1, 64), tri_stay = pt_tuned(s->ctx->tune.tri_stay, 65, 1, 65);
        ptw_launch_extend8(count, pl.spill_levels > 0u, pl.waves7, pl.grid, pl.smem, st, ev0, ev1, s->d_wide8, s->norm_c, s->norm_s, s->norm_rs, s->d_tri4_8, s->d_shade64_8, rayA, rayB, hit,
                           count_in, count_zero, stats, spill, stride, pl.refill | (tri_enter << 8) | (tri_stay << 16), tmin, tmax, pl.lds_stack, raw, perm, ray_tmax);
        return;
    }
    const bool no_spill = !pl.spill && tmin > 0.f;
    const size_t smem = (!pl.spill && !no_spill) ? pl.smem_wide_entries : pl.smem;
    if (!pl.lds_scene) {
        ptw_launch_extend_hbm(count, s->ctx->tune.rec64 != 0, pl.grid, smem, st, ev0, ev1, s->d_wide, pl.topdown4 ? reinterpret_cast<const uint2 *>(s->d_wide16t) : s->d_wide16, s->norm_c, s->norm_s, s->norm_rs, s->d_tri4,
                              s->d_shade64, s->n_wide, s->n_tris, rayA, rayB, hit, count_in, count_zero, stats, spill, stride,
                              pl.refill | (pt_tuned(s->ctx->tune.tri_enter, 0, 0, 64) << 8), tmin, tmax, pl.lds_stack, raw, perm, ray_tmax);
        return;
    }
    hipExtLaunchKernelGGL(pick_extend_lds(no_spill, pl.pairs, count, ray_tmax != nullptr), dim3(pl.grid), dim3(TB), (uint32_t)smem, st, ev0, ev1, 0u, s->d_wide,
                          s->d_wide16, norm_box_blas(s), s->d_tri4, s->n_wide, s->n_tris, rayA, rayB, hit, count_in, count_zero, stats, spill, stride,
                          pl.refill, tmin, tmax, pl.lds_stack, raw, nullptr, ray_tmax, nullptr);
}
```

single-file-vulkan-pathtracing_amd/csrc/fused.hip:

```cpp
#include "wavefront_host.h"

#include <algorithm>

#define PT_EXTEND_TEMPLATES_ONLY
#include "extend_kernel.h"
#include "extend_inst16.h"

#ifdef PT_FUSED_TIMELINE
__device__ unsigned long long *g_fused_timeline = nullptr;
extern "C" int pt_debug_fused_timeline(void *device_u64x4_per_wave)
{
    return (int)hipMemcpyToSymbol(HIP_SYMBOL(g_fused_timeline), &device_u64x4_per_wave, sizeof(void *));
}
#endif

#ifdef PT_FUSED_HIST
__device__ uint32_t *g_fused_hist = nullptr;
extern "C" int pt_debug_fused_hist(void *device_u32_2x8192x16)
{
    return (int)hipMemcpyToSymbol(HIP_SYMBOL(g_fused_hist), &device_u32_2x8192x16, sizeof(void *));
}
#endif

#include "fused_cull.h"
#include "nee_sample.h"

namespace {
using namespace ptw;
#include "fused_dev.h"
#include "fused_kernel.h"
#include "fused_inst_kernel.h"
constexpr size_t FUSED_COUNT_LDS = sizeof(uint32_t) * 2 * FB_N * (FTB / 64);
static_assert((int)FB_N == (int)PT_FB_COUNT && FB_N <= PT_N_BLOCKS, "fused_kernel.h FusedBlock mirrors include/pt_api.h pt_fused_block");

using FusedFn = decltype(&k_fused<0, true>);
template <int MODE>
FusedFn pick_fused_mode(bool pairs, bool count)
{
    if (count) return k_fused_count<MODE, true>;
    return pairs ? k_fused<MODE, true> : k_fused<MODE, false>;
}
FusedFn pick_fused(int mode, bool pairs, bool count)
{
    return mode == 2 ? pick_fused_mode<2>(pairs, count) : mode == 1 ? pick_fused_mode<1>(pairs, count) : pick_fused_mode<0>(pairs, count);
}
using FusedNeeFn = decltype(&k_fused_nee<true>);
FusedNeeFn pick_fused_nee(bool pairs) { return pairs ? k_fused_nee<true> : k_fused_nee<false>; }
using FusedInstFn = decltype(&k_fused_inst<false, true>);
FusedInstFn pick_fused_inst(bool grouped, bool pairs)
{
    if (grouped) return pairs ? k_fused_inst<true, true> : k_fused_inst<true, false>;
    return pairs ? k_fused_inst<false, true> : k_fused_inst<false, false>;
}

template <class Prepare>
pt_status fused_blocks_per_cu(pt_ctx *ctx, int family, size_t smem, bool pairs, int &per_cu, Prepare &&prepare)
{
    const size_t key = (smem << 1) | (pairs ? 1u : 0u);
    if (ctx->fused_smem[family] != key || ctx->fused_per_cu[family] <= 0) {
        int n = 0;
        const pt_status rc = prepare(&n);
        if (rc != PT_OK) return rc;
        ctx->fused_smem[family] = key;
        ctx->fused_per_cu[family] = n;
    }
    per_cu = ptw_tuned_blocks(ctx, ctx->fused_per_cu[family]);
    return PT_OK;
}

pt_status plan_fused_inst(pt_scene *s, const ExtendPlan &pl, float tmin, FusedPlan &fp)
{
    pt_ctx *ctx = s->ctx;
    const size_t tables = sizeof(float4) * 3 * (size_t)s->n_tris;
    if (!pl.inst16 || !(tmin > 0.f) || tables > 16 * 1024) {
        ctx->err = "PT_PIPELINE_FUSED takes instanced scenes of the fp16 two-level kernel's class: 2 .. 32767 instances, a BLAS of <= 2047 "
                   "triangles that fits LDS, tmin > 0";
        return PT_ERR_UNSUPPORTED;
    }
    fp.inst = true;
    fp.lds_stack = pl.lds_stack;
    const size_t tlas_lds_bytes = (size_t)pt_tuned(ctx->tune.tlas_lds_kb, PT_FUSEDI_TLAS_KB, 0, 96) * 1024;
    fp.n_tlas_lds = (uint32_t)std::min<size_t>(s->n_tlas16, tlas_lds_bytes / lds_nodes16_bytes(1));
    fp.smem = (size_t)fp.lds_stack * FITB * sizeof(uint32_t) + lds_nodes16_bytes((size_t)s->n_wide + fp.n_tlas_lds) + lds_tris_bytes(s->n_tris) + tables +
              sizeof(uint32_t) * FS_FIELDS * FITB + sizeof(uint32_t) * (FITB / 64) * PT_FUSED_WTILES;
    if (fp.smem > 160 * 1024) { ctx->err = "PT_PIPELINE_FUSED: the two-level kernel's LDS plan exceeds 160 KB (pt_tuning lds_stack / tlas_lds_kb)"; return PT_ERR_UNSUPPORTED; }
    int per_cu = 0;
    const pt_status rcp = fused_blocks_per_cu(ctx, 1, fp.smem, s->pair_leaves, per_cu, [&](int *n) {
        const pt_status rcg = ptw_prepare_kernel(ctx, reinterpret_cast<const void *>(pick_fused_inst(true, s->pair_leaves)), FITB, fp.smem);
        return rcg != PT_OK ? rcg : ptw_prepare_kernel(ctx, reinterpret_cast<const void *>(pick_fused_inst(false, s->pair_leaves)), FITB, fp.smem, n);
    });
    if (rcp != PT_OK) return rcp;
    fp.grid = ctx->num_cus * per_cu;
    fp.block = FITB;
    fp.refill = pt_tuned(ctx->tune.refill, 48, 1, 64);
    const pt_status rcs = ptw_reserve_spill(ctx, (size_t)std::max(pl.spill_levels, 1u) * (size_t)fp.grid * FITB * sizeof(uint32_t));
    if (rcs != PT_OK) return rcs;
    fp.spill = reinterpret_cast<uint32_t *>(ctx->d_spill);
    if (ctx->tune.inst_frames != 0) {
        const pt_status rcf = ptb_ensure_inst_frames(s);
        if (rcf != PT_OK) return rcf;
        fp.inst_frame = s->d_inst_frame;
    }
    return PT_OK;
}
}

pt_status ptw_plan_fused(pt_scene *s, const ExtendPlan &pl, float tmin, FusedPlan &fp, bool nee)
{
    pt_ctx *ctx = s->ctx;
    if (s->n_inst && nee) {
        ctx->err = "PT_PIPELINE_FUSED with PT_FLAG_NEE is for single-level scenes (instanced scenes: PT_PIPELINE_WAVEFRONT_NEE)";
        return PT_ERR_UNSUPPORTED;
    }
    if (s->n_inst) return plan_fused_inst(s, pl, tmin, fp);
    const size_t tables = sizeof(float4) * 5 * (size_t)s->n_tris;
    if (pl.variant != PT_EXTEND_LDS || pl.spill || !(tmin > 0.f) || tables > 16 * 1024) {
        ctx->err = "PT_PIPELINE_FUSED is for single-level scenes whose BVH4, triangles and shading tables fit LDS (the compact "
                   "kernels' class: <= 2047 triangles in <= 24 KB, stack bound <= 16, tmin > 0)";
        return PT_ERR_UNSUPPORTED;
    }
    fp.lds_stack = pl.lds_stack + 1;
    fp.smem = (size_t)fp.lds_stack * FTB * sizeof(uint32_t) + lds_scene_bytes(s->n_wide, s->n_tris) + tables +
              sizeof(uint32_t) * FS_FIELDS * FTB + sizeof(uint32_t) * (FTB / 64) * PT_FUSED_WTILES;
    fp.pairs = pl.pairs;
    fp.block = FTB;
    int per_cu = 0;
    pt_status rcp;
    if (nee) {
        fp.nee = true;
        fp.smem += sizeof(uint32_t) * FS_NEE_FIELDS * FTB;
        rcp = fused_blocks_per_cu(ctx, 2, fp.smem, pl.pairs, per_cu,
                                  [&](int *n) { return ptw_prepare_kernel(ctx, reinterpret_cast<const void *>(pick_fused_nee(pl.pairs)), FTB, fp.smem, n); });
    } else {
        rcp = fused_blocks_per_cu(ctx, 0, fp.smem, pl.pairs, per_cu, [&](int *n) {
            pt_status rc = PT_OK;
            for (int mode = 2; mode >= 0 && rc == PT_OK; mode--) {
                rc = ptw_prepare_kernel(ctx, reinterpret_cast<const void *>(pick_fused(mode, pl.pairs, true)), FTB, fp.smem + FUSED_COUNT_LDS);
                if (rc == PT_OK) rc = ptw_prepare_kernel(ctx, reinterpret_cast<const void *>(pick_fused(mode, pl.pairs, false)), FTB, fp.smem, mode == 0 ? n : nullptr);
            }
            return rc;
        });
    }
    if (rcp != PT_OK) return rcp;
    fp.grid = ctx->num_cus * per_cu;
    fp.refill = pt_tuned(ctx->tune.refill, 36, 1, 64);
    return PT_OK;
}

void ptw_launch_fused(const FusedPlan &fp, bool grouped, const ptw::RenderConst &rc, const uint32_t *tiles, const ptw::Radiance &rad,
                      const pt_scene *s, uint32_t n_slots, uint32_t *next_slot, unsigned long long *stats, float tmin, float tmax,
                      hipStream_t st, hipEvent_t ev0, hipEvent_t ev1)
{
    if (fp.inst) {
        const int enter_min = pt_tuned(s->ctx->tune.enter_min, 12, 1, 64), leaf_min = pt_tuned(s->ctx->tune.leaf_min, 14, 1, 64);
        const int node_yield = pt_tuned(s->ctx->tune.node_yield, 6, 0, 64);
        hipExtLaunchKernelGGL(pick_fused_inst(grouped, s->pair_leaves), dim3(fp.grid), dim3(FITB), (uint32_t)fp.smem, st, ev0, ev1, 0u, rc, tiles, rad, s->d_tlas16,
                              norm_box_tlas(s), reinterpret_cast<const uint4 *>(s->d_wide16), norm_box_blas(s), s->d_tri4, s->d_shade4, s->n_wide, s->n_tris, s->d_inst6,
                              s->d_tlas_prim_of, fp.inst_frame, 0u, n_slots, next_slot, stats, fp.spill, (uint32_t)fp.grid * FITB, fp.refill,
                              tmin, tmax, fp.lds_stack, enter_min, leaf_min, node_yield, fp.n_tlas_lds);
        return;
    }
    FastDiv div_frames;
    div_frames.init(std::max(rc.lanes_active, 1u));
    const int mode = rc.tail ? 2 : (grouped ? 1 : 0);
    if (fp.nee) {
        if (mode != 0) return;
        hipExtLaunchKernelGGL(pick_fused_nee(fp.pairs), dim3(fp.grid), dim3(FTB), (uint32_t)fp.smem, st, ev0, ev1, 0u, rc, tiles, rad, s->d_wide, s->d_tri4, s->d_shade4,
                              s->d_frame4, s->n_wide, s->n_tris, 0u, n_slots, next_slot, stats, fp.refill, tmin, tmax, fp.lds_stack, div_frames, s->d_lights,
                              s->n_lights, s->light_area);
        return;
    }
    hipExtLaunchKernelGGL(pick_fused(mode, fp.pairs, fp.count), dim3(fp.grid), dim3(FTB), (uint32_t)(fp.smem + (fp.count ? FUSED_COUNT_LDS : 0)), st, ev0, ev1, 0u, rc, tiles,
                          rad, s->d_wide, s->d_tri4, s->d_shade4, s->d_frame4, s->n_wide, s->n_tris, 0u, n_slots, next_slot, stats, fp.refill, tmin, tmax, fp.lds_stack,
                          div_frames);
}
```

single-file-vulkan-pathtracing_amd/csrc/fused_inst_kernel.h:

```cpp
#pragma once

#ifndef PT_FUSEDI_WAVES
#define PT_FUSEDI_WAVES 4
#endif
#ifndef PT_FUSEDI_TB
#define PT_FUSEDI_TB 512
#endif
#ifndef PT_FUSEDI_TLAS_KB
#define PT_FUSEDI_TLAS_KB 8
#endif
constexpr int FITB = PT_FUSEDI_TB;

template <bool GROUPED, bool PAIRS>
__global__ __launch_bounds__(FITB, PT_FUSEDI_WAVES) void k_fused_inst(
    RenderConst rc_arg, const uint32_t *__restrict__ tiles_arg, Radiance rad_arg, const uint4 *__restrict__ tlas16_arg, NormBox nbt_arg,
    const uint4 *__restrict__ g_blas16, NormBox nbb_arg, const float4 *__restrict__ g_tri4, const float4 *__restrict__ g_shade4,
    uint32_t n_blas_wide, uint32_t n_tris, const float4 *__restrict__ inst6_arg, const uint32_t *__restrict__ inst_id_arg,
    const float4 *__restrict__ inst_frame_arg, uint32_t slot_base_arg, uint32_t n_slots_arg, uint32_t *next_slot_arg, unsigned long long *stats_arg,
    uint32_t *__restrict__ spill_arg, uint32_t spill_stride_arg, int refill_arg, float tmin_arg, float tmax_arg, int lds_stack, int enter_min_arg,
    int leaf_min_arg, int node_yield_arg, uint32_t n_tlas_lds_arg)
{
    const RenderConst rc = ptm::own_sgprs(rc_arg);
    const Radiance rad = ptm::own_sgprs(rad_arg);
    const NormBox nbt = ptm::own_sgprs(nbt_arg), nbb = ptm::own_sgprs(nbb_arg);
    const uint32_t *tiles = ptm::own_sgprs(static_cast<const uint32_t *>(tiles_arg));
    const uint4 *tlas16 = ptm::own_sgprs(static_cast<const uint4 *>(tlas16_arg));
    const float4 *inst6 = ptm::own_sgprs(static_cast<const float4 *>(inst6_arg)), *inst_frame = ptm::own_sgprs(static_cast<const float4 *>(inst_frame_arg));
    const uint32_t *inst_id = ptm::own_sgprs(static_cast<const uint32_t *>(inst_id_arg));
    uint32_t *next_slot = ptm::own_sgprs(next_slot_arg), *spill = ptm::own_sgprs(static_cast<uint32_t *>(spill_arg));
    unsigned long long *stats = ptm::own_sgprs(stats_arg);
    const uint32_t slot_base = ptm::own_sgprs(slot_base_arg), n_slots = ptm::own_sgprs(n_slots_arg), spill_stride = ptm::own_sgprs(spill_stride_arg),
                   n_tlas_lds = ptm::own_sgprs(n_tlas_lds_arg);
    const int refill = ptm::own_sgprs(refill_arg), enter_min = ptm::own_sgprs(enter_min_arg), leaf_min = ptm::own_sgprs(leaf_min_arg),
              node_yield = ptm::own_sgprs(node_yield_arg);
    const float tmin = ptm::own_sgprs(tmin_arg), tmax = ptm::own_sgprs(tmax_arg);
    extern __shared__ __attribute__((aligned(16))) char smem[];
    uint32_t *s_stack = reinterpret_cast<uint32_t *>(smem);
    uint32_t *s_blas = s_stack + (size_t)lds_stack * FITB;
    float4 *s_tri = reinterpret_cast<float4 *>(s_blas + (size_t)I16_NODE_DW * (n_blas_wide + n_tlas_lds));
    float4 *s_shade = s_tri + 9 * (size_t)n_tris;
    lds_u32 *my_state = (lds_u32 *)reinterpret_cast<uint32_t *>(s_shade + 3 * (size_t)n_tris) + threadIdx.x;
    for (uint32_t i = threadIdx.x; i < 4 * n_tlas_lds; i += FITB)
        *reinterpret_cast<uint4 *>(s_blas + (size_t)(n_blas_wide + (i >> 2)) * I16_NODE_DW + 4 * (i & 3u)) = tlas16[i];
    for (uint32_t i = threadIdx.x; i < 4 * n_blas_wide; i += FITB) {
        uint4 v = g_blas16[i];
        if ((i & 3u) == 3u) {
            auto code = [](uint32_t w) {
                if (w == SENTINEL) return I16_DONE;
                return (w & PT_LEAF) ? (I16_LEAF | (((w >> 28) & 3u) << 11) | (w & 0x7FFu)) : (w & 0x7FFFu);
            };
            v = make_uint4(code(v.x), code(v.y), code(v.z), code(v.w));
        }
        *reinterpret_cast<uint4 *>(s_blas + (size_t)(i >> 2) * I16_NODE_DW + 4 * (i & 3u)) = v;
    }
    for (uint32_t i = threadIdx.x; i < 3 * n_tris; i += FITB) {
        const float4 v = g_tri4[i];
        s_tri[i] = make_float4(v.y, v.z, v.x, v.w);
        s_tri[3 * n_tris + i] = make_float4(v.z, v.x, v.y, v.w);
        s_tri[6 * n_tris + i] = v;
        s_shade[i] = g_shade4[i];
    }
    __syncthreads();
    const float4 *verts = s_tri + 6 * (size_t)n_tris;

    lds_u32 *my_stack = (lds_u32 *)s_stack + threadIdx.x;
    uint32_t *my_spill = spill + (size_t)blockIdx.x * FITB + threadIdx.x;
    const float INF = __builtin_inff();
    const int lane = threadIdx.x & 63;

    bool out_of_slots = false, in_blas = false;
    uint32_t n_rays_wave = 0, n_cull_wave = 0;
    uint32_t w_next = 0, w_end = 0, w_base = 0;
    uint32_t w_part = blockIdx.x % (uint32_t)PT_FUSED_PARTS, w_tried = 0;
    const uint32_t part_len = ((n_slots + PT_FUSED_PARTS - 1) / PT_FUSED_PARTS + 63u) & ~63u;
    lds_u32 *s_wtile = (lds_u32 *)reinterpret_cast<uint32_t *>(s_shade + 3 * (size_t)n_tris) + FS_FIELDS * FITB + (threadIdx.x >> 6) * PT_FUSED_WTILES;
    ptm::f3 org_w{}, dir_w{};
    ptm::f3 inv{}, invf{}, on{}, of{}, orgp{};
    uint32_t mx = 0, my = 0, mz = 0;
    ptm::f3 w_inv{}, w_invf{}, w_on{}, w_of{};
    uint32_t w_mx = 0, w_my = 0, w_mz = 0;
    uint32_t tri_base = 0;
    ptm::RayPre pre{};
    float best_t = tmax, best_V = 0.f, best_W = 0.f, best_det = 1.f;
    uint32_t best_pos = PT_MISS, best_prim = PT_MISS, best_ipos = PT_MISS, best_iid = PT_MISS;
    uint32_t cur = I16_DONE, cur_ipos = 0, cur_iid = 0;
    int sp = -1, sp_exit = 0;

    auto level_setup = [&](const ptm::f3 o, const ptm::f3 d, const NormBox &nb) {
        const ptm::f3 on_ = { (o.x - nb.cx) * nb.rsx, (o.y - nb.cy) * nb.rsy, (o.z - nb.cz) * nb.rsz };
        inv = { ptm::safe_inv(d.x) * nb.sx, ptm::safe_inv(d.y) * nb.sy, ptm::safe_inv(d.z) * nb.sz };
        slab_setup(on_, inv, invf, on, of);
        mx = inv.x < 0.f ? 0xFFFFFFFFu : 0u; my = inv.y < 0.f ? 0xFFFFFFFFu : 0u; mz = inv.z < 0.f ? 0xFFFFFFFFu : 0u;
    };
    auto push = [&](uint32_t e) {
        if (sp < lds_stack) my_stack[sp * FITB] = e;
        else my_spill[(size_t)(sp - lds_stack) * spill_stride] = e;
        sp++;
    };
    auto pop = [&]() -> uint32_t {
        constexpr uint32_t PENDING = 0xFFFFFFFFu;
        uint32_t r = PENDING;
        while (__ballot(r == PENDING)) {
            if (r == PENDING) {
                if (sp > 0) {
                    if (in_blas && sp == sp_exit) in_blas = false;
                    sp--;
                    uint32_t e;
                    if (sp < lds_stack) e = my_stack[sp * FITB];
                    else e = my_spill[(size_t)(sp - lds_stack) * spill_stride];
                    r = __uint_as_float(e & 0xFFFF0000u) <= best_t ? (e & 0xFFFFu) : PENDING;
                } else {
                    in_blas = false;
                    r = I16_DONE;
                }
            }
        }
        return r;
    };
    auto pop_and_restore = [&]() -> uint32_t {
        const bool was_in = in_blas;
        const uint32_t c = pop();
        if (was_in && !in_blas) {
            inv = w_inv; invf = w_invf; on = w_on; of = w_of;
            mx = w_mx; my = w_my; mz = w_mz;
        }
        return c;
    };

    for (;;) {
        const bool have = cur != I16_DONE, path = sp >= 0;
        const unsigned long long m_have = __ballot(have), m_path = __ballot(path);
        const unsigned long long m_in_blk = ~m_have & (out_of_slots ? m_path : ~0ull);
        const bool in_blk = !have && (path || !out_of_slots);
        const int n_work = __popcll(m_in_blk);
        if (n_work && n_work * 64 >= refill * (n_work + __popcll(m_have))) {
            uint32_t slot = 0, ctr = 0, seed = 0, pxy = 0;
            float wr = 0.f, wg = 0.f, wb = 0.f;
            ptm::f3 org{}, dir{};
            bool got_ray = false, need_primary = false, bounce = false;
            if (in_blk && path) {
                slot = my_state[FS_SLOT * FITB]; ctr = my_state[FS_CTR * FITB]; seed = my_state[FS_SEED * FITB];
                wr = __uint_as_float(my_state[FS_WR * FITB]); wg = __uint_as_float(my_state[FS_WG * FITB]); wb = __uint_as_float(my_state[FS_WB * FITB]);
                pxy = my_state[FS_PXY * FITB];
                uint32_t sample = ctr & 0xFFFFu, depth = ctr >> 16;
                float er, eg, eb;
                bool terminated, add;
                const uint32_t pos = best_pos;
                if (pos == PT_MISS) {
                    er = wr * rc.env[0]; eg = wg * rc.env[1]; eb = wb * rc.env[2];
                    add = true;
                    terminated = true;
                } else {
                    const float4 s1 = s_shade[3 * pos + 1], s2 = s_shade[3 * pos + 2];
                    er = wr * s1.z; eg = wg * s1.w; eb = wb * s2.x;
                    add = !(er == 0.f && eg == 0.f && eb == 0.f);
                    depth++;
                    terminated = depth >= rc.max_depth;
                }
                if (add) {
                    if (!GROUPED) {
                        my_state[FS_A * FITB] = __float_as_uint(__uint_as_float(my_state[FS_A * FITB]) + er);
                        my_state[FS_B * FITB] = __float_as_uint(__uint_as_float(my_state[FS_B * FITB]) + eg);
                        my_state[FS_C * FITB] = __float_as_uint(__uint_as_float(my_state[FS_C * FITB]) + eb);
                    } else {
                        const uint32_t k = my_state[FS_A * FITB];
                        if (k < rc.term_pcap) ptm::st_stream<true>(rad.terms + ((size_t)k * rc.n_slots + slot), make_float4(er, eg, eb, 0.f));
                        else if (k < rc.term_cap) ptm::st_stream<true>(rad.dev->terms_over + ((size_t)slot * (rc.term_cap - rc.term_pcap) + (k - rc.term_pcap)), make_float4(er, eg, eb, 0.f));
                        else {
                            const Radiance rr = *rad.dev;
                            const unsigned long long idx = atomicAdd(rr.spill_count, 1ull);
                            if (idx < rr.spill_cap) {
                                rr.spill[idx] = make_float4(er, eg, eb, __uint_as_float(k == rc.term_cap ? SPILL_NONE : rr.spill_head[slot]));
                                rr.spill_head[slot] = (uint32_t)idx;
                            } else {
                                *rr.overflow = 1ull;
                            }
                        }
                        my_state[FS_A * FITB] = k + 1u;
                    }
                }
                if (!terminated) {
                    bounce = true;
                } else {
                    sample++;
                    depth = 0;
                    bool more;
                    if (!GROUPED) {
                        more = sample < rc.spp;
                    } else {
                        const uint32_t lane_slot = rc.div_spl.div(slot);
                        const uint32_t g = lane_slot - rc.div_groups.div(lane_slot) * rc.groups;
                        more = sample < min(rc.spp, (g + 1u) * rc.group_size);
                    }
                    if (more) {
                        need_primary = true;
                    } else {
                        if (!GROUPED) rad.color[slot] = make_float4(__uint_as_float(my_state[FS_A * FITB]), __uint_as_float(my_state[FS_B * FITB]),
                                                                   __uint_as_float(my_state[FS_C * FITB]), 0.f);
                        else rad.nterm[slot] = my_state[FS_A * FITB];
                        sp = -1;
                    }
                }
                ctr = sample | (depth << 16);
            }
            const unsigned long long m_want = __ballot(in_blk && sp < 0);
            if (m_want && !out_of_slots) {
                if (w_next >= w_end) {
                    for (;;) {
                        const uint32_t part_begin = w_part * part_len, part_end = min(part_begin + part_len, n_slots);
                        uint32_t rel = 0, size = 0;
                        if (lane == 0) {
                            uint32_t *cnt = next_slot + w_part * (uint32_t)PT_FUSED_PART_STRIDE;
                            size = (uint32_t)(GROUPED ? PT_FUSED_BATCH : PT_FUSED_BATCH1);
                            rel = atomicAdd(cnt, size);
                        }
                        rel = __builtin_amdgcn_readfirstlane(rel);
                        size = __builtin_amdgcn_readfirstlane(size);
                        if (part_begin < part_end && rel < part_end - part_begin) {
                            w_base = w_next = part_begin + rel;
                            w_end = min(w_next + size, part_end);
                            break;
                        }
                        w_part = (w_part + 1u) % (uint32_t)PT_FUSED_PARTS;
                        if (++w_tried >= (uint32_t)PT_FUSED_PARTS) { out_of_slots = true; w_end = w_next; break; }
                    }
                    if (!out_of_slots && (uint32_t)lane < (w_end - w_base + 63u) / 64u) {
                        const uint32_t c = slot_base + w_base + 64u * (uint32_t)lane;
                        s_wtile[lane] = tiles[(c - rc.div_spl.div(c) * rc.slots_per_lane) >> 6];
                    }
                    __builtin_amdgcn_wave_barrier();
                }
                const uint32_t take = min((uint32_t)__popcll(m_want), w_end - w_next);
                const uint32_t rank = (uint32_t)__popcll(m_want & ((1ull << lane) - 1ull));
                uint32_t cull_n = 0u;
                if (in_blk && sp < 0 && rank < take) {
                    const uint32_t mine = w_next + rank;
                    slot = slot_base + mine;
                    const uint32_t lane_slot = rc.div_spl.div(slot);
                    const uint32_t f = rc.div_groups.div(lane_slot), g = lane_slot - f * rc.groups;
                    const uint32_t local = slot - lane_slot * rc.slots_per_lane;
                    const uint32_t tw = s_wtile[(mine - w_base) >> 6];
                    const uint32_t px = (tw & 0xFFFFu) * 8u + (local & 7u), py = (tw >> 16) * 8u + ((local >> 3) & 7u);
                    const uint32_t sample0 = g * rc.group_size;
                    const bool in_image = px < rc.width && py < rc.height && f < rc.lanes_active && sample0 < rc.spp;
                    if (in_image && ptc::pixel_culled(rc, px, py)) {
                        cull_n = GROUPED ? ptc::finish_group(rc, rad, slot, g) : ptc::finish_plain(rc, rad, slot);
                    } else if (in_image) {
                        pxy = px | (py << 16);
                        ctr = sample0;
                        my_state[FS_A * FITB] = 0u;
                        if (!GROUPED) { my_state[FS_B * FITB] = 0u; my_state[FS_C * FITB] = 0u; }
                        my_state[FS_MB * FITB] = (uint32_t)((int32_t)rc.spp * (rc.frame_base + (int32_t)f)) + 1u;
                        sp = 0;
                        need_primary = true;
                    } else if (GROUPED) {
                        rad.nterm[slot] = 0u;
                    }
                }
                w_next += take;
                if (rc.cull_on) {
                    const uint32_t n_c = ptc::rays_finished<GROUPED>(rc, cull_n);
                    n_rays_wave += n_c;
                    n_cull_wave += n_c;
                }
            }
            if (need_primary) {
                const uint32_t m = (ctr & 0xFFFFu) + my_state[FS_MB * FITB];
                const uint2 sd = ptm::pcg2d(make_uint2((pxy & 0xFFFFu) * m, (pxy >> 16) * m));
                seed = sd.x + sd.y;
                wr = wg = wb = 1.0f;
            }
            if (bounce || need_primary) {
                const float r1 = ptm::rnd(seed);
                const float r2 = ptm::rnd(seed);
                float vx = 0.f, vy = 0.f, vz = 0.f, sq_arg;
                if (need_primary) {
                    ptm::primary_target(rc.cam, pxy & 0xFFFFu, pxy >> 16, r1, r2, vx, vy, vz);
                    sq_arg = (vx * vx + vy * vy) + vz * vz;
                } else {
                    sq_arg = 1.0f - r1 * r1;
                }
                const float sq = ptm::fsqrt(sq_arg);
                float q1, q2, q3;
                ptm::div3_dominant(need_primary ? vx : best_V, need_primary ? vy : best_W, need_primary ? vz : best_W, need_primary ? sq : best_det, q1, q2, q3);
                if (need_primary) {
                    org = { rc.cam.ox, rc.cam.oy, rc.cam.oz };
                    dir = { q1, q2, q3 };
                } else {
                    const uint32_t pos = best_pos;
                    const float4 s0 = s_shade[3 * pos + 0], s1 = s_shade[3 * pos + 1];
                    const float4 a = verts[3 * pos + 0], b = verts[3 * pos + 1], c = verts[3 * pos + 2];
                    const float hu = q1, hv = q2;
                    const float b0 = (1.0f - hu) - hv;
                    org = { (a.x * b0 + b.x * hu) + c.x * hv, (a.y * b0 + b.y * hu) + c.y * hv, (a.z * b0 + b.z * hu) + c.z * hv };
                    ptm::f3 nrm = { s0.x, s0.y, s0.z };
                    ptm::f3 tng{};
                    const uint32_t ip = best_ipos;
                    const float4 m0 = inst6[6 * (size_t)ip + 0], m1 = inst6[6 * (size_t)ip + 1], m2 = inst6[6 * (size_t)ip + 2];
                    const ptm::f3 pw = { ((m0.x * org.x + m0.y * org.y) + m0.z * org.z) + m0.w,
                                         ((m1.x * org.x + m1.y * org.y) + m1.z * org.z) + m1.w,
                                         ((m2.x * org.x + m2.y * org.y) + m2.z * org.z) + m2.w };
                    org = pw;
                    if (inst_frame) {
                        const size_t e = 2 * ((size_t)ip * n_tris + pos);
                        const float4 f0 = inst_frame[e], f1 = inst_frame[e + 1];
                        nrm = { f0.x, f0.y, f0.z };
                        tng = { f0.w, f1.x, f1.y };
                        const ptm::f3 btg = { nrm.y * tng.z - nrm.z * tng.y, nrm.z * tng.x - nrm.x * tng.z, nrm.x * tng.y - nrm.y * tng.x };
                        dir = ptm::sample_direction_frame_sq(r1, r2, sq, nrm, tng, btg);
                    } else {
                        const float4 i0 = inst6[6 * (size_t)ip + 3], i1 = inst6[6 * (size_t)ip + 4], i2 = inst6[6 * (size_t)ip + 5];
                        const float nx = (i0.x * nrm.x + i1.x * nrm.y) + i2.x * nrm.z;
                        const float ny = (i0.y * nrm.x + i1.y * nrm.y) + i2.y * nrm.z;
                        const float nz = (i0.z * nrm.x + i1.z * nrm.y) + i2.z * nrm.z;
                        const float l = ptm::fsqrt((nx * nx + ny * ny) + nz * nz);
                        nrm = { ptm::fdiv(nx, l), ptm::fdiv(ny, l), ptm::fdiv(nz, l) };
                        ptm::f3 T, B;
                        ptm::tangent_frame(nrm, T, B);
                        dir = ptm::sample_direction_frame_sq(r1, r2, sq, nrm, T, B);
                    }
                    const float dt = (dir.x * nrm.x + dir.y * nrm.y) + dir.z * nrm.z;
                    float fr = s0.w * dt, fg = s1.x * dt, fb = s1.y * dt;
                    ptm::div3_by_pdf(fr, fg, fb);
                    wr = wr * fr; wg = wg * fg; wb = wb * fb;
                }
                got_ray = true;
            }
            if (got_ray) {
                my_state[FS_SLOT * FITB] = slot; my_state[FS_CTR * FITB] = ctr; my_state[FS_SEED * FITB] = seed;
                my_state[FS_WR * FITB] = __float_as_uint(wr); my_state[FS_WG * FITB] = __float_as_uint(wg); my_state[FS_WB * FITB] = __float_as_uint(wb);
                my_state[FS_PXY * FITB] = pxy;
                org_w = org;
                dir_w = dir;
                level_setup(org_w, dir_w, nbt);
                w_inv = inv; w_invf = invf; w_on = on; w_of = of; w_mx = mx; w_my = my; w_mz = mz;
                in_blas = false;
                best_t = tmax; best_V = 0.f; best_W = 0.f; best_det = 1.f;
                best_pos = PT_MISS; best_prim = PT_MISS; best_ipos = PT_MISS; best_iid = PT_MISS;
                cur = 0u;
                sp = 0;
            }
            n_rays_wave += (uint32_t)__popcll(__ballot(got_ray));
        }
        const bool tracing = cur != I16_DONE;
        const unsigned long long m_tracing = __ballot(tracing);
        if (m_tracing == 0ull && __ballot(sp >= 0) == 0ull && out_of_slots) break;

        const int n_have = __popcll(m_tracing);
        bool do_node = cur < I16_LEAF;
        if (__ballot(do_node) != 0ull) for (;;) {
            if (do_node) {
            uint4 q0, q1, q2, cw;
            if (in_blas || cur < n_tlas_lds) {
                typedef uint32_t u32x4 __attribute__((ext_vector_type(4)));
                typedef __attribute__((address_space(3))) const u32x4 lds_cu4;
                const uint32_t li = in_blas ? cur : cur + n_blas_wide;
                lds_cu4 *nd = (lds_cu4 *)reinterpret_cast<const u32x4 *>(s_blas + (size_t)li * I16_NODE_DW);
                const u32x4 r0 = nd[0], r1 = nd[1], r2 = nd[2], r3 = nd[3];
                q0 = make_uint4(r0.x, r0.y, r0.z, r0.w); q1 = make_uint4(r1.x, r1.y, r1.z, r1.w);
                q2 = make_uint4(r2.x, r2.y, r2.z, r2.w); cw = make_uint4(r3.x, r3.y, r3.z, r3.w);
                PT_REG_BARRIER16(q0, q1, q2, cw)
            } else {
                const uint4 *nd = tlas16 + 4 * (size_t)cur;
                q0 = nd[0]; q1 = nd[1]; q2 = nd[2]; cw = nd[3];
                PT_REG_BARRIER16(q0, q1, q2, cw)
            }
            auto sel = [](uint32_t m, uint32_t a, uint32_t b) { return (m & a) | (~m & b); };
            const uint2 hnx = { sel(mx, q1.z, q0.x), sel(mx, q1.w, q0.y) }, hfx = { sel(mx, q0.x, q1.z), sel(mx, q0.y, q1.w) };
            const uint2 hny = { sel(my, q2.x, q0.z), sel(my, q2.y, q0.w) }, hfy = { sel(my, q0.z, q2.x), sel(my, q0.w, q2.y) };
            const uint2 hnz = { sel(mz, q2.z, q1.x), sel(mz, q2.w, q1.y) }, hfz = { sel(mz, q1.x, q2.z), sel(mz, q1.y, q2.w) };
            float t0, t1, t2, t3;
            PT_SLAB4H(t0, x, 0)
            PT_SLAB4H(t1, x, 1)
            PT_SLAB4H(t2, y, 0)
            PT_SLAB4H(t3, y, 1)
            uint32_t k0 = (__float_as_uint(t0) & 0xFFFF0000u) | cw.x, k1 = (__float_as_uint(t1) & 0xFFFF0000u) | cw.y,
                     k2 = (__float_as_uint(t2) & 0xFFFF0000u) | cw.z, k3 = (__float_as_uint(t3) & 0xFFFF0000u) | cw.w;
#define PT_KSWAP(A, B) { const uint32_t lo_ = min(A, B), hi_ = max(A, B); A = lo_; B = hi_; }
            PT_KSWAP(k0, k1)
            PT_KSWAP(k2, k3)
            PT_KSWAP(k0, k2)
            PT_KSWAP(k1, k3)
            PT_KSWAP(k1, k2)
#undef PT_KSWAP
            constexpr uint32_t KINF = 0x7F800000u;
            if (k3 < KINF) push(k3);
            if (k2 < KINF) push(k2);
            if (k1 < KINF) push(k1);
            cur = k0 < KINF ? (k0 & 0xFFFFu) : pop_and_restore();
            }
            do_node = cur < I16_LEAF;
            const int n_cont = __popcll(__ballot(do_node));
            if (n_cont == 0 || (node_yield > 0 && n_cont * node_yield < n_have)) break;
        }
        const bool at_leaf = (uint32_t)(cur - I16_LEAF) < I16_DONE - I16_LEAF;
        const int n_enter = __popcll(__ballot(at_leaf && !in_blas));
        const int n_leaf = __popcll(__ballot(at_leaf && in_blas));
        const bool descending = __ballot(cur < I16_LEAF) != 0ull;
        const bool do_leaf = n_leaf >= leaf_min || !(descending || n_enter >= enter_min);
        const bool others = descending || (do_leaf && n_leaf > 0);
        const bool do_enter = n_enter >= enter_min || !others;
        {
            if (at_leaf && in_blas && do_leaf) {
                const uint32_t first = cur & 0x7FFu, cnt = ((cur >> 11) & 3u) + 1u;
                auto accept = [&](float t, float V, float W, float det, uint32_t pos, uint32_t prim) {
                    ptl::closer_instanced(t, V, W, det, pos, prim, cur_ipos, cur_iid, best_t, best_V, best_W, best_det, best_pos, best_prim, best_ipos, best_iid);
                };
                if (PAIRS) {
                    ptl::pair_leaf_test<true>(s_tri, (size_t)tri_base + 3 * (size_t)first, cnt == 2u, first, pre, orgp, tmin, tmax, accept,
                                        [] {});
                } else {
                    for (uint32_t k = 0; k < cnt; k++) {
                        const uint32_t pos = first + k;
                        const size_t ti = (size_t)tri_base + 3 * (size_t)pos;
                        const float4 a = s_tri[ti + 0], b = s_tri[ti + 1], c = s_tri[ti + 2];
                        float t, V, W, det;
                        if (ptm::tri_test_perm(pre, orgp, { a.x, a.y, a.z }, { b.x, b.y, b.z }, { c.x, c.y, c.z }, tmin, tmax, t, V, W, det, nullptr))
                            accept(t, V, W, det, pos, __float_as_uint(a.w));
                    }
                }
                cur = pop_and_restore();
            } else if (at_leaf && !in_blas && do_enter) {
                const uint32_t first = cur & 0x7FFFu;
                cur_ipos = first;
                cur_iid = inst_id[first];
                const float4 r0 = inst6[6 * (size_t)first + 3], r1 = inst6[6 * (size_t)first + 4], r2 = inst6[6 * (size_t)first + 5];
                const ptm::f3 oo = { ((r0.x * org_w.x + r0.y * org_w.y) + r0.z * org_w.z) + r0.w,
                                     ((r1.x * org_w.x + r1.y * org_w.y) + r1.z * org_w.z) + r1.w,
                                     ((r2.x * org_w.x + r2.y * org_w.y) + r2.z * org_w.z) + r2.w };
                const ptm::f3 od = { (r0.x * dir_w.x + r0.y * dir_w.y) + r0.z * dir_w.z,
                                     (r1.x * dir_w.x + r1.y * dir_w.y) + r1.z * dir_w.z,
                                     (r2.x * dir_w.x + r2.y * dir_w.y) + r2.z * dir_w.z };
                level_setup(oo, od, nbb);
                pre = ptm::ray_setup(oo, od);
                tri_base = (uint32_t)pre.kz * 3u * n_tris;
                orgp = { ptm::sel3(pre.kz, oo.y, oo.z, oo.x), ptm::sel3(pre.kz, oo.z, oo.x, oo.y), ptm::sel3(pre.kz, oo.x, oo.y, oo.z) };
                sp_exit = sp;
                in_blas = true;
                cur = 0u;
            }
        }
    }
    if (lane == 0 && n_rays_wave) atomicAdd(stats, (unsigned long long)n_rays_wave);
    if (lane == 0 && n_cull_wave) atomicAdd(stats + 19, (unsigned long long)n_cull_wave);
}
```

single-file-vulkan-pathtracing_amd/csrc/fused_kernel.h:

```cpp
#pragma once

#ifndef PT_FUSED_WAVES
#define PT_FUSED_WAVES 6
#endif

#ifndef PT_FUSED_TB
#define PT_FUSED_TB 512
#endif
constexpr int FTB = PT_FUSED_TB;

#ifndef PT_FUSED_BATCH
#define PT_FUSED_BATCH 256
#endif
#ifndef PT_FUSED_BATCH1
#define PT_FUSED_BATCH1 64
#endif
#define PT_FUSED_WTILES (PT_FUSED_BATCH / 64)
#define PT_FUSED_PARTS 8
#define PT_FUSED_PART_STRIDE 32

enum : int { FS_SLOT = 0, FS_CTR, FS_SEED, FS_WR, FS_WG, FS_WB, FS_PXY, FS_A, FS_B, FS_C, FS_MB, FS_FIELDS };
enum : int { FS_NEE_POS = 0, FS_NEE_R, FS_NEE_G, FS_NEE_B, FS_NEE_FIELDS };
#ifndef PT_FUSED_WAVES_NEE
#define PT_FUSED_WAVES_NEE 4
#endif

#ifndef PT_FUSED_NODE_EXIT
#define PT_FUSED_NODE_EXIT 3
#endif
#ifndef PT_FUSED_NODE_EXIT_B
#define PT_FUSED_NODE_EXIT_B 1
#endif
enum FusedBlock : int {
    FB_ITER = 0,
    FB_SHADE,
    FB_HIT,
    FB_MISS,
    FB_SURFACE,
    FB_ADD,
    FB_BOUNCE,
    FB_NEXT,
    FB_DONE,
    FB_HANDOUT,
    FB_DRAW,
    FB_TAKE,
    FB_CULLED,
    FB_PRIMARY,
    FB_SETUP,
    FB_NODE,
    FB_POP,
    FB_LEAF,
    FB_DIV,
    FB_FINISH,
    FB_TRACE,
    FB_SPAWN,
    FB_PTARGET,
    FB_PDIR,
    FB_POPTOP,
    FB_N
};
template <int MODE, bool PAIRS, bool COUNT, bool NEE = false>
__device__ __forceinline__ void fused_body(RenderConst rc_arg, const uint32_t *__restrict__ tiles_arg, Radiance rad_arg,
                                           const float4 *__restrict__ g_wide, const float4 *__restrict__ g_tri4,
                                           const float4 *__restrict__ g_shade4, const float4 *__restrict__ g_frame4,
                                           uint32_t n_wide, uint32_t n_tris, uint32_t slot_base_arg, uint32_t n_slots_arg,
                                           uint32_t *next_slot_arg, unsigned long long *stats_arg, int refill_arg, float tmin_arg,
                                           float tmax_arg, int lds_stack, FastDiv div_frames_arg,
                                           const float4 *__restrict__ lights_arg = nullptr, uint32_t n_lights_arg = 0u, float light_area_arg = 0.f)
{
    constexpr uint32_t LEAF_BIT = C14_LEAF, DONE = C14_DONE;
    constexpr bool GROUPED = MODE == 1, HYB = MODE == 2;
    static_assert(!NEE || (MODE == 0 && !COUNT), "NEE: one sample group, no instrumented twin");
    const RenderConst rc = ptm::own_sgprs(rc_arg);
    const Radiance rad = ptm::own_sgprs(rad_arg);
    const FastDiv div_frames = ptm::own_sgprs(div_frames_arg);
    const uint32_t *tiles = ptm::own_sgprs(static_cast<const uint32_t *>(tiles_arg));
    uint32_t *next_slot = ptm::own_sgprs(next_slot_arg);
    unsigned long long *stats = ptm::own_sgprs(stats_arg);
    const uint32_t slot_base = ptm::own_sgprs(slot_base_arg), n_slots = ptm::own_sgprs(n_slots_arg);
    const int refill = ptm::own_sgprs(refill_arg);
    const float tmin = ptm::own_sgprs(tmin_arg), tmax = ptm::own_sgprs(tmax_arg);
    const float4 *lights = nullptr;
    uint32_t n_lights = 0u;
    float light_area = 0.f;
    if constexpr (NEE) {
        lights = ptm::own_sgprs(lights_arg);
        n_lights = ptm::own_sgprs(n_lights_arg);
        light_area = ptm::own_sgprs(light_area_arg);
    }
    extern __shared__ __attribute__((aligned(16))) char smem[];
    float4 *s_wide = reinterpret_cast<float4 *>(smem + (size_t)lds_stack * FTB * sizeof(uint32_t));
    float4 *s_tri = s_wide + LDS_NODE_F4 * (size_t)n_wide;
    float4 *s_shade = s_tri + 9 * (size_t)n_tris;
    float4 *s_frame = s_shade + 3 * (size_t)n_tris;
    lds_u32 *my_state = (lds_u32 *)reinterpret_cast<uint32_t *>(s_frame + 2 * (size_t)n_tris) + threadIdx.x;
    lds_stage_nodes<FTB, true>(s_wide, g_wide, n_wide);
    lds_stage_tris<FTB, true>(s_tri, g_tri4, n_tris, s_shade, g_shade4);
    for (uint32_t i = threadIdx.x; i < 2 * n_tris; i += FTB) s_frame[i] = g_frame4[i];
    __syncthreads();
    const float4 *wide = s_wide, *tri4 = s_tri;
    const float4 *verts = s_tri + 6 * (size_t)n_tris;

    lds_u32 *my_stack32 = (lds_u32 *)reinterpret_cast<uint32_t *>(smem) + FTB + threadIdx.x;
    const int lane = threadIdx.x & 63;

    FusedDev dev;
    dev.kernel_begin();
    lds_u32 *s_fb = (lds_u32 *)reinterpret_cast<uint32_t *>(s_frame + 2 * (size_t)n_tris) + FS_FIELDS * FTB + (FTB / 64) * PT_FUSED_WTILES + (threadIdx.x >> 6) * (2 * FB_N);
    if constexpr (COUNT) {
        if (lane < 2 * FB_N) s_fb[lane] = 0u;
    }
#define PT_FB(B)                                                                                        \
    if constexpr (COUNT) {                                                                              \
        const unsigned long long m_fb = __ballot(1);                                                    \
        if (lane == __ffsll((long long)m_fb) - 1) { s_fb[2 * (B)] += 1u; s_fb[2 * (B) + 1] += (uint32_t)__popcll(m_fb); } \
    }
    bool out_of_slots = false;
    uint32_t n_rays_wave = 0;
    uint32_t n_cull_wave = 0;
    uint32_t w_next = 0, w_end = 0, w_base = 0;
    uint32_t w_part = blockIdx.x % (uint32_t)PT_FUSED_PARTS, w_tried = 0;
    bool w_tails = false;
    const uint32_t n_tail_slots = HYB ? rc.lanes_active * rc.tail * rc.slots_per_lane : 0u;
    const uint32_t part_len = ((n_slots + PT_FUSED_PARTS - 1) / PT_FUSED_PARTS + 63u) & ~63u;
    lds_u32 *s_wtile = (lds_u32 *)reinterpret_cast<uint32_t *>(s_frame + 2 * (size_t)n_tris) + FS_FIELDS * FTB + (threadIdx.x >> 6) * PT_FUSED_WTILES;
    lds_u32 *my_nee = (lds_u32 *)reinterpret_cast<uint32_t *>(s_frame + 2 * (size_t)n_tris) + FS_FIELDS * FTB + (FTB / 64) * PT_FUSED_WTILES + threadIdx.x;
    ptm::f3 inv{}, invf{}, on{}, of{}, orgp{};
    ptm::RayPre pre{};
    uint32_t ax = 0, ay = 0, az = 0, tri_base = 0;
    float best_t = tmax, best_V = 0.f, best_W = 0.f, best_det = 1.f;
    uint32_t best_pos = PT_MISS;
    uint32_t cur = DONE;
    int sp = -1;

    constexpr uint32_t PENDING = 0xFFFFFFFFu;
    auto pop_pending = [&](uint32_t r) -> uint32_t {
        while (__ballot(r == PENDING)) {
            if (r == PENDING) {
                PT_FB(FB_POP)
                sp--;
                const uint32_t e = my_stack32[sp * FTB];
                const uint32_t miss = sp == 0 ? DONE : PENDING;
                r = __uint_as_float(e & 0xFFFFC000u) <= best_t ? (e & 0x3FFFu) : miss;
            }
        }
        return r;
    };
    auto pop = [&]() -> uint32_t { return pop_pending(sp > 0 ? PENDING : DONE); };

    for (;;) {
        PT_FB(FB_ITER)
        const bool have = cur != DONE, path = sp >= 0;
        const unsigned long long m_have = __ballot(have), m_path = __ballot(path);
        const unsigned long long m_in_blk = ~m_have & (out_of_slots ? m_path : ~0ull);
        const bool in_blk = !have && (path || !out_of_slots);
        const int n_work = __popcll(m_in_blk);
        if (n_work && n_work * 64 >= refill * (n_work + __popcll(m_have))) {
            uint32_t slot = 0, ctr = 0, seed = 0, pxy = 0;
            float wr = 0.f, wg = 0.f, wb = 0.f;
            ptm::f3 org{}, dir{};
            bool got_ray = false, need_primary = false, bounce = false;
            bool shadow = false;
            uint32_t bpos = 0u;
            float4 nc{};
            if (in_blk) { PT_FB(FB_SHADE) }
            if (in_blk && path) {
                PT_FB(FB_HIT)
                slot = my_state[FS_SLOT * FTB]; ctr = my_state[FS_CTR * FTB]; seed = my_state[FS_SEED * FTB];
                wr = __uint_as_float(my_state[FS_WR * FTB]); wg = __uint_as_float(my_state[FS_WG * FTB]); wb = __uint_as_float(my_state[FS_WB * FTB]);
                pxy = my_state[FS_PXY * FTB];
                uint32_t sample = ctr & 0xFFFFu, depth = ctr >> 16;
                float er, eg, eb;
                bool terminated, add;
                const uint32_t pos = best_pos;
                const uint32_t npos = NEE ? (uint32_t)my_nee[FS_NEE_POS * FTB] : PT_MISS;
                if (NEE && npos != PT_MISS) {
                    er = __uint_as_float(my_nee[FS_NEE_R * FTB]); eg = __uint_as_float(my_nee[FS_NEE_G * FTB]); eb = __uint_as_float(my_nee[FS_NEE_B * FTB]);
                    add = pos == PT_MISS;
                    terminated = false;
                    bpos = npos;
                    org = { ptm::sel3(pre.kz, orgp.z, orgp.y, orgp.x), ptm::sel3(pre.kz, orgp.x, orgp.z, orgp.y), ptm::sel3(pre.kz, orgp.y, orgp.x, orgp.z) };
                } else if (pos == PT_MISS) {
                    PT_FB(FB_MISS)
                    er = wr * rc.env[0]; eg = wg * rc.env[1]; eb = wb * rc.env[2];
                    add = true;
                    terminated = true;
                } else {
                    PT_FB(FB_SURFACE)
                    const float4 s1 = s_shade[3 * pos + 1], s2 = s_shade[3 * pos + 2];
                    er = wr * s1.z; eg = wg * s1.w; eb = wb * s2.x;
                    add = !(er == 0.f && eg == 0.f && eb == 0.f);
                    if (NEE) add = add && depth == 0u;
                    depth++;
                    terminated = depth >= rc.max_depth;
                    if (NEE && !terminated) {
                        float hu, hv;
                        ptm::div2_dominant(best_V, best_W, best_det, hu, hv);
                        const float4 a = verts[3 * pos + 0], b = verts[3 * pos + 1], c = verts[3 * pos + 2];
                        const float b0 = (1.0f - hu) - hv;
                        org = { (a.x * b0 + b.x * hu) + c.x * hv, (a.y * b0 + b.y * hu) + c.y * hv, (a.z * b0 + b.z * hu) + c.z * hv };
                        bpos = pos;
                        if (n_lights) {
                            const float4 s0 = s_shade[3 * pos + 0];
                            ptm::f3 wi;
                            shadow = ptn::nee_sample(lights, n_lights, light_area, seed, org, { s0.x, s0.y, s0.z }, s0.w, s1.x, s1.y, wr, wg, wb, wi, nc);
                            if (shadow) dir = wi;
                        }
                    }
                }
                const bool logs = GROUPED || (HYB && slot >= rc.n_head);
                const uint32_t lslot = HYB ? slot - rc.n_head : slot;
                const uint32_t lstride = HYB ? rc.n_tail : rc.n_slots;
                if (add) {
                    PT_FB(FB_ADD)
                    if (!logs) {
                        my_state[FS_A * FTB] = __float_as_uint(__uint_as_float(my_state[FS_A * FTB]) + er);
                        my_state[FS_B * FTB] = __float_as_uint(__uint_as_float(my_state[FS_B * FTB]) + eg);
                        my_state[FS_C * FTB] = __float_as_uint(__uint_as_float(my_state[FS_C * FTB]) + eb);
                    } else {
                        const uint32_t k = my_state[FS_A * FTB];
                        if (dbg_no_terms && k != 0xFFFFFFFFu) {}
                        else if (k < rc.term_pcap) ptm::st_stream<true>(rad.terms + ((size_t)k * lstride + lslot), make_float4(er, eg, eb, 0.f));
                        else if (k < rc.term_cap) ptm::st_stream<true>(rad.dev->terms_over + ((size_t)lslot * (rc.term_cap - rc.term_pcap) + (k - rc.term_pcap)), make_float4(er, eg, eb, 0.f));
                        else {
                            const Radiance rr = *rad.dev;
                            const unsigned long long idx = atomicAdd(rr.spill_count, 1ull);
                            if (idx < rr.spill_cap) {
                                rr.spill[idx] = make_float4(er, eg, eb, __uint_as_float(k == rc.term_cap ? SPILL_NONE : rr.spill_head[lslot]));
                                rr.spill_head[lslot] = (uint32_t)idx;
                            } else {
                                *rr.overflow = 1ull;
                            }
                        }
                        my_state[FS_A * FTB] = k + 1u;
                    }
                }
                if (!terminated) {
                    bounce = !shadow;
                    got_ray = shadow;
                } else {
                    PT_FB(FB_NEXT)
                    sample++;
                    depth = 0;
                    bool more;
                    if (HYB) {
                        more = !logs && sample < rc.head_samples;
                    } else if (!GROUPED) {
                        more = sample < rc.spp;
                    } else {
                        const uint32_t lane_slot = rc.div_spl.div(slot);
                        const uint32_t g = lane_slot - rc.div_groups.div(lane_slot) * rc.groups;
                        more = sample < min(rc.spp, (g + 1u) * rc.group_size);
                    }
                    if (more) {
                        need_primary = true;
                    } else {
                        PT_FB(FB_DONE)
                        if (!logs) rad.color[slot] = make_float4(__uint_as_float(my_state[FS_A * FTB]), __uint_as_float(my_state[FS_B * FTB]),
                                                                   __uint_as_float(my_state[FS_C * FTB]), 0.f);
                        else if (!dbg_no_nterm) rad.nterm[lslot] = my_state[FS_A * FTB];
                        sp = -1;
                        dev.slot_end(slot);
                    }
                }
                ctr = sample | (depth << 16);
            }
            const unsigned long long m_want = __ballot(in_blk && sp < 0);
            if (m_want && !out_of_slots) {
                if (in_blk && sp < 0) { PT_FB(FB_HANDOUT) }
                if (w_next >= w_end) {
                    PT_FB(FB_DRAW)
                    for (;;) {
                        const bool grp = GROUPED || (HYB && w_tails);
                        const uint32_t ns = (HYB && w_tails) ? n_tail_slots : n_slots;
                        const uint32_t plen = HYB ? ((ns + PT_FUSED_PARTS - 1) / PT_FUSED_PARTS + 63u) & ~63u : part_len;
                        const uint32_t part_begin = grp ? w_part * plen : 0u,
                                       part_end = grp ? min(part_begin + plen, ns)
                                                      : (((ns >> 6) + (uint32_t)PT_FUSED_PARTS - 1u - w_part) / (uint32_t)PT_FUSED_PARTS) << 6;
                        uint32_t rel = 0, size = 0;
                        if (lane == 0) {
                            uint32_t *cnt = next_slot + (w_part + ((HYB && w_tails) ? (uint32_t)PT_FUSED_PARTS : 0u)) * (uint32_t)PT_FUSED_PART_STRIDE;
                            size = (uint32_t)(grp ? PT_FUSED_BATCH : PT_FUSED_BATCH1);
                            rel = atomicAdd(cnt, size);
                        }
                        rel = __builtin_amdgcn_readfirstlane(rel);
                        size = __builtin_amdgcn_readfirstlane(size);
                        if (part_begin < part_end && rel < part_end - part_begin) {
                            w_base = w_next = part_begin + rel;
                            w_end = min(w_next + size, part_end);
                            break;
                        }
                        w_part = (w_part + 1u) % (uint32_t)PT_FUSED_PARTS;
                        if (++w_tried >= (uint32_t)PT_FUSED_PARTS) {
                            if (HYB && !w_tails && n_tail_slots) {
                                w_tails = true;
                                w_tried = 0;
                                w_part = blockIdx.x % (uint32_t)PT_FUSED_PARTS;
                                continue;
                            }
                            out_of_slots = true;
                            w_end = w_next;
                            break;
                        }
                    }
                    if (out_of_slots) dev.out_of_slots();
                    if (!out_of_slots && (uint32_t)lane < (w_end - w_base + 63u) / 64u) {
                        if (GROUPED || (HYB && w_tails)) {
                            const uint32_t c = slot_base + w_base + 64u * (uint32_t)lane;
                            s_wtile[lane] = tiles[(c - rc.div_spl.div(c) * rc.slots_per_lane) >> 6];
                        } else {
                            s_wtile[lane] = tiles[div_frames.div(((w_base >> 6) + (uint32_t)lane) * (uint32_t)PT_FUSED_PARTS + w_part)];
                        }
                    }
                    __builtin_amdgcn_wave_barrier();
                }
                const uint32_t take = min((uint32_t)__popcll(m_want), w_end - w_next);
                const uint32_t rank = (uint32_t)__popcll(m_want & ((1ull << lane) - 1ull));
                uint32_t cull_n = 0u;
                if (in_blk && sp < 0 && rank < take) {
                    PT_FB(FB_TAKE)
                    const uint32_t mine = w_next + rank;
                    uint32_t f, g, local;
                    if (HYB && w_tails) {
                        const uint32_t lane_slot = rc.div_spl.div(mine);
                        f = rc.div_tail.div(lane_slot); g = lane_slot - f * rc.tail;
                        local = mine - lane_slot * rc.slots_per_lane;
                        slot = rc.n_head + mine;
                    } else if (GROUPED) {
                        slot = slot_base + mine;
                        const uint32_t lane_slot = rc.div_spl.div(slot);
                        f = rc.div_groups.div(lane_slot); g = lane_slot - f * rc.groups;
                        local = slot - lane_slot * rc.slots_per_lane;
                    } else {
                        const uint32_t q = (mine >> 6) * (uint32_t)PT_FUSED_PARTS + w_part;
                        const uint32_t t = div_frames.div(q);
                        f = q - t * rc.lanes_active; g = 0u;
                        local = t * 64u + (mine & 63u);
                        slot = slot_base + f * rc.slots_per_lane + local;
                    }
                    const uint32_t tw = s_wtile[(mine - w_base) >> 6];
                    const uint32_t px = (tw & 0xFFFFu) * 8u + (local & 7u), py = (tw >> 16) * 8u + ((local >> 3) & 7u);
                    const uint32_t sample0 = (HYB && w_tails) ? rc.head_samples + g : g * rc.group_size;
                    const bool in_image = px < rc.width && py < rc.height && f < rc.lanes_active && sample0 < rc.spp;
                    if (in_image && ptc::pixel_culled(rc, px, py)) {
                        PT_FB(FB_CULLED)
                        if (GROUPED) cull_n = ptc::finish_group(rc, rad, slot, g);
                        else if (!(HYB && w_tails)) cull_n = ptc::finish_plain(rc, rad, slot);
                    } else if (in_image) {
                        pxy = px | (py << 16);
                        ctr = sample0;
                        my_state[FS_A * FTB] = 0u;
                        if (!GROUPED) { my_state[FS_B * FTB] = 0u; my_state[FS_C * FTB] = 0u; }
                        my_state[FS_MB * FTB] = (uint32_t)((int32_t)rc.spp * (rc.frame_base + (int32_t)f)) + 1u;
                        sp = 0;
                        need_primary = true;
                        dev.slot_begin();
                    } else if (GROUPED) {
                        rad.nterm[slot] = 0u;
                    } else if (HYB && w_tails) {
                        rad.nterm[slot - rc.n_head] = 0u;
                    }
                }
                w_next += take;
                if (rc.cull_on) {
                    const uint32_t n_c = ptc::rays_finished<GROUPED>(rc, cull_n);
                    n_rays_wave += n_c;
                    n_cull_wave += n_c;
                }
            }
            if (need_primary) {
                PT_FB(FB_PRIMARY)
                const uint32_t m = (ctr & 0xFFFFu) + my_state[FS_MB * FTB];
                const uint2 sd = ptm::pcg2d(make_uint2((pxy & 0xFFFFu) * m, (pxy >> 16) * m));
                seed = sd.x + sd.y;
                wr = wg = wb = 1.0f;
            }
            if (bounce || need_primary) {
                PT_FB(FB_SPAWN)
                const float r1 = ptm::rnd(seed);
                const float r2 = ptm::rnd(seed);
                float vx = 0.f, vy = 0.f, vz = 0.f, sq_arg;
                if (need_primary) {
                    PT_FB(FB_PTARGET)
                    ptm::primary_target(rc.cam, pxy & 0xFFFFu, pxy >> 16, r1, r2, vx, vy, vz);
                    sq_arg = (vx * vx + vy * vy) + vz * vz;
                } else {
                    sq_arg = 1.0f - r1 * r1;
                }
                const float sq = ptm::fsqrt(sq_arg);
                float q1, q2, q3;
                ptm::div3_dominant(need_primary ? vx : best_V, need_primary ? vy : best_W, need_primary ? vz : best_W, need_primary ? sq : best_det, q1, q2, q3);
                if (need_primary) {
                    PT_FB(FB_PDIR)
                    org = { rc.cam.ox, rc.cam.oy, rc.cam.oz };
                    dir = { q1, q2, q3 };
                } else {
                    PT_FB(FB_BOUNCE)
                    const uint32_t pos = NEE ? bpos : best_pos;
                    const float4 s0 = s_shade[3 * pos + 0], s1 = s_shade[3 * pos + 1];
                    const ptm::f3 nrm = { s0.x, s0.y, s0.z };
                    const float4 f0 = s_frame[2 * pos + 0], f1 = s_frame[2 * pos + 1];
                    dir = ptm::sample_direction_frame_sq(r1, r2, sq, nrm, { f0.x, f0.y, f0.z }, { f0.w, f1.x, f1.y });
                    const float dt = (dir.x * nrm.x + dir.y * nrm.y) + dir.z * nrm.z;
                    float fr = s0.w * dt, fg = s1.x * dt, fb = s1.y * dt;
                    ptm::div3_by_pdf(fr, fg, fb);
                    wr = wr * fr; wg = wg * fg; wb = wb * fb;
                    if (!NEE) {
                        const float4 a = verts[3 * pos + 0], b = verts[3 * pos + 1], c = verts[3 * pos + 2];
                        const float hu = q1, hv = q2;
                        const float b0 = (1.0f - hu) - hv;
                        org = { (a.x * b0 + b.x * hu) + c.x * hv, (a.y * b0 + b.y * hu) + c.y * hv, (a.z * b0 + b.z * hu) + c.z * hv };
                    }
                }
                got_ray = true;
            }
            if (got_ray) {
                PT_FB(FB_SETUP)
                my_state[FS_SLOT * FTB] = slot; my_state[FS_CTR * FTB] = ctr; my_state[FS_SEED * FTB] = seed;
                my_state[FS_WR * FTB] = __float_as_uint(wr); my_state[FS_WG * FTB] = __float_as_uint(wg); my_state[FS_WB * FTB] = __float_as_uint(wb);
                my_state[FS_PXY * FTB] = pxy;
                if constexpr (NEE) {
                    my_nee[FS_NEE_POS * FTB] = shadow ? bpos : PT_MISS;
                    if (shadow) {
                        my_nee[FS_NEE_R * FTB] = __float_as_uint(nc.x); my_nee[FS_NEE_G * FTB] = __float_as_uint(nc.y); my_nee[FS_NEE_B * FTB] = __float_as_uint(nc.z);
                    }
                }
                pre = ptm::ray_setup<true>(org, dir);
                inv = { ptm::safe_inv(dir.x), ptm::safe_inv(dir.y), ptm::safe_inv(dir.z) };
                slab_setup(org, inv, invf, on, of);
                ax = inv.x < 0.f ? 48u : 0u;
                ay = inv.y < 0.f ? 48u : 0u;
                az = inv.z < 0.f ? 48u : 0u;
                tri_base = (uint32_t)pre.kz * 3u * n_tris;
                orgp = { ptm::sel3(pre.kz, org.y, org.z, org.x), ptm::sel3(pre.kz, org.z, org.x, org.y), ptm::sel3(pre.kz, org.x, org.y, org.z) };
                best_t = (NEE && shadow) ? nc.w : tmax;
                best_V = 0.f; best_W = 0.f; best_det = 1.f;
                best_pos = PT_MISS;
                cur = 0u;
                sp = 0;
            }
            const uint32_t n_started = (uint32_t)__popcll(__ballot(got_ray));
            n_rays_wave += n_started;
            dev.rays_started(n_started, HYB && w_tails, lane);
        }
        const bool tracing = cur != DONE;
        const unsigned long long m_tracing = __ballot(tracing);
        if (m_tracing == 0ull && __ballot(sp >= 0) == 0ull && out_of_slots) break;

        const int n_have = __popcll(m_tracing);
        if (tracing) { PT_FB(FB_TRACE) }
        {
            bool dn = cur < LEAF_BIT;
            if (__ballot(dn) != 0ull) {
                int n_cont;
                do {
                    if (dn) {
                        PT_FB(FB_NODE)
                        const uint32_t e_top = my_stack32[(sp - 1) * FTB];
                        cur = compact_node_step<FTB>(wide, cur, inv, invf, on, of, ax, ay, az, tmin, best_t, my_stack32, sp, [&]() -> uint32_t {
                            PT_FB(FB_POPTOP)
                            const bool any = sp > 0;
                            sp -= any ? 1 : 0;
                            const uint32_t below = sp > 0 ? PENDING : DONE;
                            const uint32_t top = __uint_as_float(e_top & 0xFFFFC000u) <= best_t ? (e_top & 0x3FFFu) : below;
                            return pop_pending(any ? top : DONE);
                        });
                    }
                    dn = cur < LEAF_BIT;
                    n_cont = __popcll(__ballot(dn));
                } while (n_cont * PT_FUSED_NODE_EXIT >= n_have * PT_FUSED_NODE_EXIT_B);
            }
        }
        {
            if ((uint32_t)(cur - LEAF_BIT) < DONE - LEAF_BIT) {
                PT_FB(FB_LEAF)
                if (PAIRS) {
                    const uint32_t first = cur & 0x7FFu;
                    ptl::pair_leaf_test<true>(tri4, (size_t)tri_base + 3 * (size_t)first, ((cur >> 11) & 3u) != 0u, first, pre, orgp, tmin, tmax,
                                        [&](float t, float V, float W, float det, uint32_t pos, uint32_t) {
                                            [[maybe_unused]] const bool closer =
                                                ptl::closer_single_level(tri4, tri_base, t, V, W, det, pos, best_t, best_V, best_W, best_det, best_pos);
                                            if constexpr (NEE) {
                                                if (closer && my_nee[FS_NEE_POS * FTB] != PT_MISS) sp = 0;
                                            }
                                        },
                                        [&] { PT_FB(FB_DIV) });
                } else {
                    const uint32_t first = cur & 0x7FFu, cnt = ((cur >> 11) & 3u) + 1u;
                    for (uint32_t k = 0; k < cnt; k++) {
                        const uint32_t pos = first + k;
                        const size_t ti = (size_t)tri_base + 3 * (size_t)pos;
                        const float4 a = tri4[ti + 0], b = tri4[ti + 1], c = tri4[ti + 2];
                        float t, V, W, det;
                        if (ptm::tri_test_perm(pre, orgp, { a.x, a.y, a.z }, { b.x, b.y, b.z }, { c.x, c.y, c.z }, tmin, tmax, t, V, W, det, nullptr)) {
                            bool closer = t < best_t;
                            if (!closer && t == best_t)
                                closer = best_pos == PT_MISS || __float_as_uint(a.w) < __float_as_uint(tri4[(size_t)tri_base + 3 * (size_t)best_pos].w);
                            if (closer) {
                                best_t = t; best_V = V; best_W = W; best_det = det; best_pos = pos;
                                if (NEE && my_nee[FS_NEE_POS * FTB] != PT_MISS) sp = 0;
                            }
                        }
                    }
                }
                cur = pop();
            }
            if (tracing && cur == DONE) {
                PT_FB(FB_FINISH)
            }
        }
    }
    if (lane == 0 && n_rays_wave) atomicAdd(stats, (unsigned long long)n_rays_wave);
    if (lane == 0 && n_cull_wave) atomicAdd(stats + 19, (unsigned long long)n_cull_wave);
    dev.kernel_end(lane, n_rays_wave, FTB);
    if constexpr (COUNT) {
        if (lane < 2 * FB_N) atomicAdd(stats + PT_N_STATS + lane, (unsigned long long)s_fb[lane]);
    }
#undef PT_FB
}

template <int MODE, bool PAIRS>
__global__ __launch_bounds__(FTB, PT_FUSED_WAVES) void k_fused(RenderConst rc, const uint32_t *__restrict__ tiles, Radiance rad,
                                                              const float4 *__restrict__ g_wide, const float4 *__restrict__ g_tri4,
                                                              const float4 *__restrict__ g_shade4, const float4 *__restrict__ g_frame4,
                                                              uint32_t n_wide, uint32_t n_tris, uint32_t slot_base, uint32_t n_slots,
                                                              uint32_t *next_slot, unsigned long long *stats, int refill, float tmin,
                                                              float tmax, int lds_stack, FastDiv div_frames)
{
    fused_body<MODE, PAIRS, false>(rc, tiles, rad, g_wide, g_tri4, g_shade4, g_frame4, n_wide, n_tris, slot_base, n_slots, next_slot, stats, refill, tmin,
                                   tmax, lds_stack, div_frames);
}
template <bool PAIRS>
__global__ __launch_bounds__(FTB, PT_FUSED_WAVES_NEE) void k_fused_nee(RenderConst rc, const uint32_t *__restrict__ tiles, Radiance rad,
                                                                      const float4 *__restrict__ g_wide, const float4 *__restrict__ g_tri4,
                                                                      const float4 *__restrict__ g_shade4, const float4 *__restrict__ g_frame4,
                                                                      uint32_t n_wide, uint32_t n_tris, uint32_t slot_base, uint32_t n_slots,
                                                                      uint32_t *next_slot, unsigned long long *stats, int refill, float tmin,
                                                                      float tmax, int lds_stack, FastDiv div_frames,
                                                                      const float4 *__restrict__ lights, uint32_t n_lights, float light_area)
{
    fused_body<0, PAIRS, false, true>(rc, tiles, rad, g_wide, g_tri4, g_shade4, g_frame4, n_wide, n_tris, slot_base, n_slots, next_slot, stats, refill,
                                      tmin, tmax, lds_stack, div_frames, lights, n_lights, light_area);
}
template <int MODE, bool PAIRS>
__global__ __launch_bounds__(FTB, PT_FUSED_WAVES) void k_fused_count(RenderConst rc, const uint32_t *__restrict__ tiles, Radiance rad,
                                                                    const float4 *__restrict__ g_wide, const float4 *__restrict__ g_tri4,
                                                                    const float4 *__restrict__ g_shade4, const float4 *__restrict__ g_frame4,
                                                                    uint32_t n_wide, uint32_t n_tris, uint32_t slot_base, uint32_t n_slots,
                                                                    uint32_t *next_slot, unsigned long long *stats, int refill, float tmin,
                                                                    float tmax, int lds_stack, FastDiv div_frames)
{
    fused_body<MODE, PAIRS, true>(rc, tiles, rad, g_wide, g_tri4, g_shade4, g_frame4, n_wide, n_tris, slot_base, n_slots, next_slot, stats, refill, tmin,
                                  tmax, lds_stack, div_frames);
}
```

single-file-vulkan-pathtracing_amd/csrc/lds_scene.h:

```cpp
#pragma once
#include "pt_internal.h"
#include "pt_math.h"

namespace {

constexpr uint32_t LDS_NODE_F4 = 9;
constexpr uint32_t C14_LEAF = 0x2000u, C14_DONE = 0x3FFFu;
constexpr uint32_t I16_EXIT = 0x7FFFu, I16_DONE = 0xFFFFu, I16_LEAF = 0x8000u;
constexpr uint32_t I16_NODE_DW = 20;

__host__ __device__ constexpr size_t lds_nodes_bytes(size_t n_wide) { return 16 * LDS_NODE_F4 * n_wide; }
__host__ __device__ constexpr size_t lds_nodes16_bytes(size_t n_nodes) { return sizeof(uint32_t) * I16_NODE_DW * n_nodes; }
__host__ __device__ constexpr size_t lds_tris_bytes(size_t n_tris) { return sizeof(float4) * 9 * n_tris; }
__host__ __device__ constexpr size_t lds_scene_bytes(size_t n_wide, size_t n_tris) { return lds_nodes_bytes(n_wide) + lds_tris_bytes(n_tris); }
__host__ __device__ constexpr size_t lds_scene16_bytes(size_t n_wide, size_t n_tris) { return lds_nodes16_bytes(n_wide) + lds_tris_bytes(n_tris); }

template <int BLOCK, bool COMPACT>
__device__ __forceinline__ void lds_stage_nodes(float4 *s_wide, const float4 *g_wide, uint32_t n_wide)
{
    for (uint32_t i = threadIdx.x; i < 8 * n_wide; i += BLOCK) {
        float4 v = g_wide[i];
        if (COMPACT && (i & 7u) == 6u) {
            auto cw = [](float f) {
                const uint32_t w = __float_as_uint(f);
                const uint32_t c = (w & PT_LEAF) ? (C14_LEAF | (((w >> 28) & 3u) << 11) | (w & 0x7FFu)) : (w & 0x1FFFu);
                return __uint_as_float(w == SENTINEL ? C14_DONE : c);
            };
            v = make_float4(cw(v.x), cw(v.y), cw(v.z), cw(v.w));
        }
        s_wide[(i >> 3) * LDS_NODE_F4 + (i & 7u)] = v;
    }
}

__device__ __forceinline__ uint32_t lds_code16(uint32_t w)
{
    if (w == SENTINEL) return I16_DONE;
    return (w & PT_LEAF) ? (I16_LEAF | (((w >> 28) & 3u) << 11) | (w & 0x7FFu)) : (w & 0x7FFFu);
}
template <int BLOCK>
__device__ __forceinline__ void lds_stage_tlas16(uint32_t *s_blas, uint32_t n_blas_wide, const uint4 *__restrict__ tlas16, uint32_t n_tlas_lds)
{
    for (uint32_t i = threadIdx.x; i < 4 * n_tlas_lds; i += BLOCK)
        *reinterpret_cast<uint4 *>(s_blas + (size_t)(n_blas_wide + (i >> 2)) * I16_NODE_DW + 4 * (i & 3u)) = tlas16[i];
}
template <int BLOCK>
__device__ __forceinline__ void lds_stage_nodes16(uint32_t *s_blas, const uint4 *__restrict__ g_blas16, uint32_t n_blas_wide, const uint4 *__restrict__ tlas16, uint32_t n_tlas_lds)
{
    lds_stage_tlas16<BLOCK>(s_blas, n_blas_wide, tlas16, n_tlas_lds);
    for (uint32_t i = threadIdx.x; i < 4 * n_blas_wide; i += BLOCK) {
        uint4 v = g_blas16[i];
        if ((i & 3u) == 3u) {
            v = make_uint4(lds_code16(v.x), lds_code16(v.y), lds_code16(v.z), lds_code16(v.w));
        }
        *reinterpret_cast<uint4 *>(s_blas + (size_t)(i >> 2) * I16_NODE_DW + 4 * (i & 3u)) = v;
    }
}

template <int BLOCK, bool EXTRA = false>
__device__ __forceinline__ void lds_stage_tris(float4 *s_tri, const float4 *g_tri4, uint32_t n_tris, float4 *s_extra = nullptr, const float4 *g_extra = nullptr)
{
    for (uint32_t i = threadIdx.x; i < 3 * n_tris; i += BLOCK) {
        const float4 v = g_tri4[i];
        s_tri[i] = make_float4(v.y, v.z, v.x, v.w);
        s_tri[3 * n_tris + i] = make_float4(v.z, v.x, v.y, v.w);
        s_tri[6 * n_tris + i] = v;
        if (EXTRA) s_extra[i] = g_extra[i];
    }
}

}
```

single-file-vulkan-pathtracing_amd/csrc/pair_leaf.h:

```cpp
#pragma once
#include "pt_math.h"

namespace ptl {

template <bool LOAD_D_FIRST = false, class Accept, class HitBlock>
__device__ __forceinline__ void pair_leaf_test(const float4 *tri4, size_t ti, bool two, uint32_t first, const ptm::RayPre &pre,
                                               const ptm::f3 &orgp, float tmin, float tmax, Accept &&accept, HitBlock &&hit_block)
{
    const float4 a = tri4[ti + 0], b = tri4[ti + 1], c = tri4[ti + 2];
    float4 d = make_float4(0.f, 0.f, 0.f, 0.f);
    if (LOAD_D_FIRST) {
        d = tri4[ti + 5];
        asm volatile("" : "+v"(d.x), "+v"(d.y), "+v"(d.z), "+v"(d.w));
    }
    const float Az_ = a.z - orgp.z, Bz_ = b.z - orgp.z, Cz_ = c.z - orgp.z;
    const float Ax = (a.x - orgp.x) - pre.Sx * Az_, Ay = (a.y - orgp.y) - pre.Sy * Az_;
    const float Bx = (b.x - orgp.x) - pre.Sx * Bz_, By = (b.y - orgp.y) - pre.Sy * Bz_;
    const float Cx = (c.x - orgp.x) - pre.Sx * Cz_, Cy = (c.y - orgp.y) - pre.Sy * Cz_;
    const float pAC = Ax * Cy, qAC = Ay * Cx;
    auto inside = [](float U, float V, float W) {
        const bool neg = fminf(fminf(U, V), W) < 0.0f, pos = fmaxf(fmaxf(U, V), W) > 0.0f, nz = ((U + V) + W) != 0.0f;
        return bool(!(neg & pos) & nz);
    };
    auto finish = [&](float U, float V, float W, float z0, float z1, float z2, uint32_t pos, uint32_t prim) {
        const float det = (U + V) + W;
        hit_block();
        const float T = (U * (pre.Sz * z0) + V * (pre.Sz * z1)) + W * (pre.Sz * z2);
        const float t = ptm::fdiv(T, det);
        accept(((t > tmin) & (t < tmax)) ? t : __builtin_nanf(""), V, W, det, pos, prim);
    };
    const float UA = Cx * By - Cy * Bx, VA = pAC - qAC, WA = Bx * Ay - By * Ax;
    const bool inA = inside(UA, VA, WA);
    float UB = 0.f, VB = 0.f, WB = 0.f, Dz_ = 0.f;
    uint32_t primB = 0u;
    bool inB = false;
    if (LOAD_D_FIRST || two) {
        if (!LOAD_D_FIRST) d = tri4[ti + 5];
        Dz_ = d.z - orgp.z;
        const float Dx = (d.x - orgp.x) - pre.Sx * Dz_, Dy = (d.y - orgp.y) - pre.Sy * Dz_;
        UB = Dx * Cy - Dy * Cx; VB = Ax * Dy - Ay * Dx; WB = qAC - pAC;
        primB = __float_as_uint(d.w);
        inB = bool(two & inside(UB, VB, WB));
    }
    if (inA || inB) {
        const bool sb = !inA;
        finish(sb ? UB : UA, sb ? VB : VA, sb ? WB : WA, Az_, sb ? Cz_ : Bz_, sb ? Dz_ : Cz_, sb ? first + 1u : first, sb ? primB : __float_as_uint(a.w));
    }
    if (inA && inB) finish(UB, VB, WB, Az_, Cz_, Dz_, first + 1u, primB);
}

__device__ __forceinline__ bool closer_single_level(const float4 *tri4, uint32_t tri_base, float t, float V, float W, float det, uint32_t pos,
                                                    float &best_t, float &best_V, float &best_W, float &best_det, uint32_t &best_pos)
{
    bool closer = t < best_t;
    if (closer) {
        best_t = t; best_V = V; best_W = W; best_det = det; best_pos = pos;
    } else if (t == best_t) {
        if (best_pos == PT_MISS || __float_as_uint(tri4[(size_t)tri_base + 3 * (size_t)pos + 2].w) <
                                       __float_as_uint(tri4[(size_t)tri_base + 3 * (size_t)best_pos + 2].w)) {
            best_t = t; best_V = V; best_W = W; best_det = det; best_pos = pos;
            closer = true;
        }
    }
    return closer;
}

__device__ __forceinline__ bool closer_instanced(float t, float V, float W, float det, uint32_t pos, uint32_t prim, uint32_t cur_ipos, uint32_t cur_iid,
                                                 float &best_t, float &best_V, float &best_W, float &best_det, uint32_t &best_pos, uint32_t &best_prim,
                                                 uint32_t &best_ipos, uint32_t &best_iid)
{
    if (t < best_t || (t == best_t && (cur_iid < best_iid || (cur_iid == best_iid && prim < best_prim)))) {
        best_t = t; best_V = V; best_W = W; best_det = det; best_pos = pos; best_prim = prim;
        best_ipos = cur_ipos; best_iid = cur_iid;
        return true;
    }
    return false;
}

}
```

Baseline: 58590 Mrays/s.

## Interleave near/far slab planes in LDS nodes and move traversal stack after scene

Changes the LDS node layout from 9 to 10 float4s per node, duplicating the min planes so each axis's near/far pair sits in adjacent float4s selected by a 16-byte sign offset. The per-lane traversal stack moves to the end of the LDS region and is wrapped in a pointer-based LaneStack that pre-reads the stack top during the node step, which simplifies the pop-top path in the fused kernel. Instanced BLAS staging keeps the old 9-float4 layout through new 128-byte helpers. The aim is cheaper address arithmetic and fewer dependent LDS reads per node step, paid for with about 11% more LDS per node, which may lower occupancy or stop larger scenes from fitting in LDS.

```diff
diff --git a/single-file-vulkan-pathtracing_amd/csrc/aov.hip b/single-file-vulkan-pathtracing_amd/csrc/aov.hip
--- a/single-file-vulkan-pathtracing_amd/csrc/aov.hip
+++ b/single-file-vulkan-pathtracing_amd/csrc/aov.hip
@@ -149,14 +149,14 @@
 __global__ __launch_bounds__(TB, PT_AOV_WAVES) void k_aov_fused(AovConst ac_arg, const uint32_t *__restrict__ tiles, uint32_t n_tiles, int32_t frame0, uint32_t n_frames,
                                                   const float4 *__restrict__ g_wide, const float4 *__restrict__ g_tri4,
                                                   const float4 *__restrict__ g_shade4, const float *__restrict__ g_faces, uint32_t n_wide,
-                                                  uint32_t n_tris, int lds_stack, AovPlanes planes_arg, uint32_t *next_tile,
+                                                  uint32_t n_tris, AovPlanes planes_arg, uint32_t *next_tile,
                                                   unsigned long long *stats)
 {
     const AovConst ac = ptm::own_sgprs(ac_arg);
     const AovPlanes planes = ptm::own_sgprs(planes_arg);
     constexpr uint32_t LEAF_BIT = C14_LEAF, DONE = C14_DONE;
     extern __shared__ __attribute__((aligned(16))) char smem[];
-    float4 *s_wide = reinterpret_cast<float4 *>(smem + (size_t)lds_stack * TB * sizeof(uint32_t));
+    float4 *s_wide = reinterpret_cast<float4 *>(smem);
     float4 *s_tri = s_wide + LDS_NODE_F4 * (size_t)n_wide;
     float4 *s_rec = s_tri + 9 * (size_t)n_tris;
     lds_stage_nodes<TB, true>(s_wide, g_wide, n_wide);
@@ -171,7 +171,7 @@
     }
     __syncthreads();
     const float4 *wide = s_wide, *tri4 = s_tri;
-    lds_u32 *my_stack32 = (lds_u32 *)reinterpret_cast<uint32_t *>(smem) + threadIdx.x;
+    LaneStack<TB> stk((lds_u32 *)reinterpret_cast<uint32_t *>(s_rec + 3 * (size_t)n_tris) + threadIdx.x);
     const int lane = threadIdx.x & 63;
     const float tmin = ac.tmin, tmax = ac.tmax;
     const float fspp = (float)ac.spp;
@@ -200,11 +200,10 @@
             float best_t = tmax, best_V = 0.f, best_W = 0.f, best_det = 1.f;
             uint32_t best_pos = PT_MISS, best_prim = PT_MISS;
             uint32_t cur = DONE;
-            int sp = 0;
+            stk.clear();
             auto pop = [&]() -> uint32_t {
-                while (sp > 0) {
-                    sp--;
-                    const uint32_t e = my_stack32[sp * TB];
+                while (stk.has_entries()) {
+                    const uint32_t e = stk.pop();
                     if (__uint_as_float(e & 0xFFFFC000u) <= best_t) return e & 0x3FFFu;
                 }
                 return DONE;
@@ -220,19 +219,19 @@
                     pre = ptm::ray_setup<PAIRS>(org, dir);
                     inv = { ptm::safe_inv(dir.x), ptm::safe_inv(dir.y), ptm::safe_inv(dir.z) };
                     slab_setup(org, inv, invf, on, of);
-                    ax = inv.x < 0.f ? 48u : 0u; ay = inv.y < 0.f ? 48u : 0u; az = inv.z < 0.f ? 48u : 0u;
+                    ax = inv.x < 0.f ? LDS_NEG_AXIS : 0u; ay = inv.y < 0.f ? LDS_NEG_AXIS : 0u; az = inv.z < 0.f ? LDS_NEG_AXIS : 0u;
                     tri_base = (uint32_t)pre.kz * 3u * n_tris;
                     orgp = { ptm::sel3(pre.kz, org.y, org.z, org.x), ptm::sel3(pre.kz, org.z, org.x, org.y), ptm::sel3(pre.kz, org.x, org.y, org.z) };
                     best_t = tmax; best_V = 0.f; best_W = 0.f; best_det = 1.f;
                     best_pos = PT_MISS; best_prim = PT_MISS;
                     cur = 0u;
-                    sp = 0;
+                    stk.clear();
                     have = true;
                 }
                 bool do_node = have && !(cur & LEAF_BIT);
                 const int n_walk = __popcll(__ballot(have));
                 while (do_node) {
-                    cur = compact_node_step<TB>(wide, cur, inv, invf, on, of, ax, ay, az, tmin, best_t, my_stack32, sp, pop);
+                    cur = compact_node_step<TB>(wide, cur, inv, invf, on, of, ax, ay, az, tmin, best_t, stk, [&](uint32_t) { return pop(); });
                     do_node = !(cur & LEAF_BIT);
                     if (__popcll(__ballot(do_node)) * 6 < n_walk) break;
                 }
@@ -363,7 +362,7 @@
     PT_HIP(ctx, hipMemsetAsync(a.d_count + AOV_NEXT_TILE, 0, sizeof(uint32_t), st));
     const int grid = (int)std::min<uint32_t>((uint32_t)fp.grid, (a.n_tiles + TB / 64 - 1) / (TB / 64));
     hipLaunchKernelGGL(pick_aov_fused(fp.pairs), dim3(grid), dim3(TB), (uint32_t)fp.smem, st, ac, a.d_tiles, a.n_tiles, p->frame, p->frame_count, s->d_wide, s->d_tri4,
-                       s->d_shade4, s->d_faces, s->n_wide, s->n_tris, pl.lds_stack, planes_of(f), a.d_count + AOV_NEXT_TILE, ctx->d_stats);
+                       s->d_shade4, s->d_faces, s->n_wide, s->n_tris, planes_of(f), a.d_count + AOV_NEXT_TILE, ctx->d_stats);
     PT_HIP(ctx, hipGetLastError());
     ctx->stats.launches_extend++;
     return PT_OK;
diff --git a/single-file-vulkan-pathtracing_amd/csrc/extend_inst.h b/single-file-vulkan-pathtracing_amd/csrc/extend_inst.h
--- a/single-file-vulkan-pathtracing_amd/csrc/extend_inst.h
+++ b/single-file-vulkan-pathtracing_amd/csrc/extend_inst.h
@@ -22,8 +22,8 @@
     const float4 *tri4 = g_tri4;
     if (LDS_BLAS) {
         float4 *s_blas = reinterpret_cast<float4 *>(smem + (size_t)LDS_STACK * TB * sizeof(uint2));
-        float4 *s_tri = s_blas + LDS_NODE_F4 * (size_t)n_blas_wide;
-        lds_stage_nodes<TB, false>(s_blas, g_blas, n_blas_wide);
+        float4 *s_tri = s_blas + LDS_NODE128_F4 * (size_t)n_blas_wide;
+        lds_stage_nodes128<TB>(s_blas, g_blas, n_blas_wide);
         lds_stage_tris<TB>(s_tri, g_tri4, n_tris);
         __syncthreads();
         blas = s_blas;
@@ -123,7 +123,7 @@
         while (have && !(cur & PT_LEAF)) {
             float4 nx, fx, ny, fy, nz, fz, cw;
             if (LDS_BLAS && in_blas) {
-                const char *nd = reinterpret_cast<const char *>(blas + LDS_NODE_F4 * (size_t)cur);
+                const char *nd = reinterpret_cast<const char *>(blas + LDS_NODE128_F4 * (size_t)cur);
                 nx = PT_F4(nd + ax); fx = PT_F4(nd - ax + 48); ny = PT_F4(nd + ay + 16); fy = PT_F4(nd - ay + 64);
                 nz = PT_F4(nd + az + 32); fz = PT_F4(nd - az + 80); cw = PT_F4(nd + 96);
             } else {
diff --git a/single-file-vulkan-pathtracing_amd/csrc/extend_kernel.h b/single-file-vulkan-pathtracing_amd/csrc/extend_kernel.h
--- a/single-file-vulkan-pathtracing_amd/csrc/extend_kernel.h
+++ b/single-file-vulkan-pathtracing_amd/csrc/extend_kernel.h
@@ -17,11 +17,12 @@
 }
 
 #define PT_F4(P) (*reinterpret_cast<const float4 *>(P))
-#define PT_NODE_LOAD(ND)                                                                                 \
-    const char *nb_ = reinterpret_cast<const char *>(ND);                                                \
-    const float4 nx = PT_F4(nb_ + ax), fx = PT_F4(nb_ - ax + 48), ny = PT_F4(nb_ + ay + 16),             \
-                 fy = PT_F4(nb_ - ay + 64), nz = PT_F4(nb_ + az + 32), fz = PT_F4(nb_ - az + 80),        \
-                 cw = PT_F4(nb_ + 96);
+constexpr uint32_t LDS_NEG_AXIS = 16;
+#define PT_NODE_LOAD(ND)                                                                                              \
+    const char *nb_ = reinterpret_cast<const char *>(ND);                                                             \
+    const char *px_ = nb_ + ax, *py_ = nb_ + ay + 16 * LDS_NODE_AXIS_F4, *pz_ = nb_ + az + 32 * LDS_NODE_AXIS_F4;     \
+    const float4 nx = PT_F4(px_), fx = PT_F4(px_ + 16), ny = PT_F4(py_), fy = PT_F4(py_ + 16), nz = PT_F4(pz_),       \
+                 fz = PT_F4(pz_ + 16), cw = PT_F4(nb_ + 16 * LDS_NODE_CW_F4);
 #define PT_SLAB4(T, C)                                                                                           \
     {                                                                                                            \
         const float tn = fmaxf(fmaxf(__builtin_fmaf(nx.C, inv.x, on.x), __builtin_fmaf(ny.C, inv.y, on.y)),      \
@@ -43,15 +44,36 @@
     return r;
 }
 
+template <int STRIDE>
+struct LaneStack {
+    lds_u32 *top;
+    lds_u32 *under;
+    __device__ __forceinline__ explicit LaneStack(lds_u32 *lane_base) : top(lane_base), under(lane_base) {}
+    __device__ __forceinline__ bool empty() const { return top <= under; }
+    __device__ __forceinline__ bool has_entries() const { return top > under; }
+    __device__ __forceinline__ void clear() { top = under; }
+    __device__ __forceinline__ void push(uint32_t e) { top += STRIDE; *top = e; }
+    __device__ __forceinline__ uint32_t peek() const { return *top; }
+    __device__ __forceinline__ uint32_t pop() { const uint32_t e = *top; top -= STRIDE; return e; }
+    __device__ __forceinline__ void drop() { top -= STRIDE; }
+    static constexpr uint32_t BOTTOM = 0xFF800000u | C14_DONE;
+    __device__ __forceinline__ void arm_bottom() { under[STRIDE] = BOTTOM; }
+    __device__ __forceinline__ void clear_to_bottom() { top = under + STRIDE; }
+    __device__ __forceinline__ void park() { top = under - 1; }
+    __device__ __forceinline__ bool parked() const { return top < under; }
+};
+__host__ __device__ constexpr size_t compact_stack_bytes(size_t threads, size_t levels) { return sizeof(uint32_t) * threads * (levels + 1); }
+
 template <int STRIDE, class Pop>
 __device__ __forceinline__ uint32_t compact_node_step(const float4 *wide, uint32_t cur, const ptm::f3 &inv, const ptm::f3 &invf, const ptm::f3 &on,
                                                       const ptm::f3 &of, uint32_t ax, uint32_t ay, uint32_t az, float tmin, float best_t,
-                                                      lds_u32 *my_stack32, int &sp, Pop &&pop)
+                                                      LaneStack<STRIDE> &stk, Pop &&pop)
 {
     const float INF = __builtin_inff();
     float t0, t1, t2, t3;
     const float4 *nd = reinterpret_cast<const float4 *>(reinterpret_cast<const char *>(wide) + __umul24(cur, 16u * LDS_NODE_F4));
     PT_NODE_LOAD(nd)
+    const uint32_t e_top = stk.peek();
     const uint32_t w0 = __float_as_uint(cw.x), w1 = __float_as_uint(cw.y), w2 = __float_as_uint(cw.z), w3 = __float_as_uint(cw.w);
     PT_SLAB4(t0, x)
     PT_SLAB4(t1, y)
@@ -67,10 +89,10 @@
     PT_KSWAP(k1, k2)
 #undef PT_KSWAP
     constexpr uint32_t KINF = 0x7F800000u;
-    if (k3 < KINF) { my_stack32[sp * STRIDE] = k3; sp++; }
-    if (k2 < KINF) { my_stack32[sp * STRIDE] = k2; sp++; }
-    if (k1 < KINF) { my_stack32[sp * STRIDE] = k1; sp++; }
-    return k0 < KINF ? (k0 & 0x3FFFu) : pop();
+    if (k3 < KINF) stk.push(k3);
+    if (k2 < KINF) stk.push(k2);
+    if (k1 < KINF) stk.push(k1);
+    return k0 < KINF ? (k0 & 0x3FFFu) : pop(e_top);
 }
 __device__ __forceinline__ void slab_setup(const ptm::f3 org, const ptm::f3 inv, ptm::f3 &invf, ptm::f3 &on, ptm::f3 &of)
 {
@@ -130,11 +152,11 @@
     constexpr uint32_t DONE = COMPACT ? C14_DONE : SENTINEL;
 
     extern __shared__ __attribute__((aligned(16))) char smem[];
-    uint2 *stack = reinterpret_cast<uint2 *>(smem);
+    uint2 *stack = reinterpret_cast<uint2 *>(smem + (LDS_SCENE ? lds_scene_bytes(n_wide, n_tris) : 0));
     const float4 *wide = g_wide;
     const float4 *tri4 = g_tri4;
     if (LDS_SCENE) {
-        float4 *s_wide = reinterpret_cast<float4 *>(smem + (size_t)lds_stack * TB * (COMPACT ? sizeof(uint32_t) : sizeof(uint2)));
+        float4 *s_wide = reinterpret_cast<float4 *>(smem);
         float4 *s_tri = s_wide + LDS_NODE_F4 * (size_t)n_wide;
         lds_stage_nodes<TB, COMPACT>(s_wide, g_wide, n_wide);
         lds_stage_tris<TB>(s_tri, g_tri4, n_tris);
@@ -148,7 +170,7 @@
         if (stats) atomicAdd(stats, (unsigned long long)n);
     }
     lds_u64 *my_stack = (lds_u64 *)reinterpret_cast<unsigned long long *>(stack) + threadIdx.x;
-    lds_u32 *my_stack32 = (lds_u32 *)reinterpret_cast<uint32_t *>(stack) + threadIdx.x;
+    LaneStack<TB> stk((lds_u32 *)reinterpret_cast<uint32_t *>(stack) + threadIdx.x);
     unsigned long long *my_spill = reinterpret_cast<unsigned long long *>(spill) + (size_t)blockIdx.x * TB + threadIdx.x;
     const float INF = __builtin_inff();
     const int lane = threadIdx.x & 63;
@@ -175,8 +197,7 @@
 
     auto push = [&](uint32_t w, float t) {
         if (COMPACT) {
-            my_stack32[sp * TB] = (__float_as_uint(t) & 0xFFFFC000u) | w;
-            sp++;
+            stk.push((__float_as_uint(t) & 0xFFFFC000u) | w);
             return;
         }
         const unsigned long long e = stack_entry(w, t);
@@ -184,13 +205,16 @@
         else my_spill[(size_t)(sp - lds_stack) * spill_stride] = e;
         sp++;
     };
+    auto clear_stack = [&] {
+        if (COMPACT) stk.clear();
+        else sp = 0;
+    };
     auto pop = [&]() -> uint32_t {
         if (COMPACT) {
-            while (sp > 0) {
+            while (stk.has_entries()) {
                 PT_COUNT_WAVE(c_pops);
                 if (COUNT) c_pop_lanes++;
-                sp--;
-                const uint32_t e = my_stack32[sp * TB];
+                const uint32_t e = stk.pop();
                 if (__uint_as_float(e & 0xFFFFC000u) <= best_t) return e & 0x3FFFu;
             }
             return DONE;
@@ -232,9 +256,9 @@
                         inv = { inv.x * nb.sx, inv.y * nb.sy, inv.z * nb.sz };
                         slab_setup(orgn, inv, invf, on, of);
                     }
-                    ax = inv.x < 0.f ? (LDS_SCENE ? 48u : 24u) : 0u;
-                    ay = inv.y < 0.f ? (LDS_SCENE ? 48u : 24u) : 0u;
-                    az = inv.z < 0.f ? (LDS_SCENE ? 48u : 24u) : 0u;
+                    ax = inv.x < 0.f ? (LDS_SCENE ? LDS_NEG_AXIS : 24u) : 0u;
+                    ay = inv.y < 0.f ? (LDS_SCENE ? LDS_NEG_AXIS : 24u) : 0u;
+                    az = inv.z < 0.f ? (LDS_SCENE ? LDS_NEG_AXIS : 24u) : 0u;
                     if (LDS_SCENE) {
                         tri_base = (uint32_t)pre.kz * 3u * n_tris;
                         orgp = { ptm::sel3(pre.kz, org.y, org.z, org.x), ptm::sel3(pre.kz, org.z, org.x, org.y),
@@ -243,7 +267,7 @@
                     best_t = ray_tmax ? ray_tmax[q] : tmax; best_V = 0.f; best_W = 0.f; best_det = 1.f;
                     best_pos = PT_MISS; best_prim = PT_MISS;
                     cur = 0u;
-                    sp = 0;
+                    clear_stack();
                     have = true;
                 }
             }
@@ -268,7 +292,7 @@
                 if (lane == __ffsll((long long)__ballot(1)) - 1) c_node_steps++;
             }
             if constexpr (LDS_SCENE && COMPACT) {
-                cur = compact_node_step<TB>(wide, cur, inv, invf, on, of, ax, ay, az, tmin, best_t, my_stack32, sp, pop);
+                cur = compact_node_step<TB>(wide, cur, inv, invf, on, of, ax, ay, az, tmin, best_t, stk, [&](uint32_t) { return pop(); });
             } else {
             float t0, t1, t2, t3;
             uint32_t w0, w1, w2, w3;
@@ -331,7 +355,7 @@
                     ptl::pair_leaf_test(tri4, (size_t)tri_base + 3 * (size_t)first, two, first, pre, orgp, tmin, tmax,
                                         [&](float t, float V, float W, float det, uint32_t pos, uint32_t) {
                                             if (ptl::closer_single_level(tri4, tri_base, t, V, W, det, pos, best_t, best_V, best_W, best_det, best_pos) && ray_tmax)
-                                                sp = 0;
+                                                clear_stack();
                                         },
                                         [&] {
                                             PT_COUNT_WAVE(c_hit_blocks);
@@ -365,13 +389,13 @@
                                          __float_as_uint(g_tri4[3 * (size_t)pos].w) < __float_as_uint(g_tri4[3 * (size_t)best_pos].w);
                             if (closer) {
                                 best_t = t; best_V = V; best_W = W; best_det = det; best_pos = pos;
-                                if (ray_tmax) sp = 0;
+                                if (ray_tmax) clear_stack();
                             }
                         } else {
                         const uint32_t prim = __float_as_uint(a.w);
                         if (t < best_t || (t == best_t && prim < best_prim)) {
                             best_t = t; best_V = V; best_W = W; best_det = det; best_pos = pos; best_prim = prim;
-                            if (ray_tmax) sp = 0;
+                            if (ray_tmax) clear_stack();
                         }
                         }
                     }
diff --git a/single-file-vulkan-pathtracing_amd/csrc/extend_launch.hip b/single-file-vulkan-pathtracing_amd/csrc/extend_launch.hip
--- a/single-file-vulkan-pathtracing_amd/csrc/extend_launch.hip
+++ b/single-file-vulkan-pathtracing_amd/csrc/extend_launch.hip
@@ -55,7 +55,7 @@
     if (s->n_inst) {
         if (want == PT_EXTEND_LDS) { ctx->err = "instanced scenes only have the HBM extend variant"; return PT_ERR_UNSUPPORTED; }
         pl.variant = PT_EXTEND_HBM;
-        const size_t blas_bytes = lds_scene_bytes(s->n_wide, s->n_tris);
+        const size_t blas_bytes = lds_scene128_bytes(s->n_wide, s->n_tris);
         pl.lds_scene = blas_bytes <= 24 * 1024;
         pl.smem = (size_t)LDS_STACK * TB * sizeof(uint2) + (pl.lds_scene ? blas_bytes : 0);
         int per_cu_i = 0;
@@ -91,8 +91,8 @@
         pl.spill_levels = bound_i > (uint32_t)LDS_STACK ? bound_i - (uint32_t)LDS_STACK : 0u;
         return ptw_reserve_spill(ctx, PT_MAX_PIPES * (size_t)std::max(pl.spill_levels, 1u) * (size_t)std::max(pl.grid, pl.grid_inst_fallback) * TB * sizeof(uint2));
     }
-    const size_t scene_bytes = lds_scene_bytes(s->n_wide, s->n_tris);
-    const bool auto8 = want == PT_EXTEND_AUTO && scene_bytes > 24 * 1024 && s->d_wide8 && (ctx->tune.hbm8 == 1 || auto8_big);
+    const size_t scene_bytes = lds_scene_bytes(s->n_wide, s->n_tris), class_bytes = lds_class_bytes(s->n_wide, s->n_tris);
+    const bool auto8 = want == PT_EXTEND_AUTO && class_bytes > 24 * 1024 && s->d_wide8 && (ctx->tune.hbm8 == 1 || auto8_big);
     if (want == PT_EXTEND_HBM8 || auto8) {
         pl.variant = PT_EXTEND_HBM8;
         pl.bvh8 = true;
@@ -111,15 +111,15 @@
         pl.spill_levels = bound8 > (uint32_t)pl.lds_stack ? bound8 - (uint32_t)pl.lds_stack : 0u;
         return ptw_reserve_spill(ctx, PT_MAX_PIPES * (size_t)std::max(pl.spill_levels, 1u) * (size_t)pl.grid * TB * sizeof(uint2));
     }
-    if (want == PT_EXTEND_LDS && scene_bytes > 96 * 1024) { ctx->err = "scene does not fit LDS"; return PT_ERR_UNSUPPORTED; }
-    pl.lds_scene = want == PT_EXTEND_LDS || (want == PT_EXTEND_AUTO && scene_bytes <= 24 * 1024);
+    if (want == PT_EXTEND_LDS && class_bytes > 96 * 1024) { ctx->err = "scene does not fit LDS"; return PT_ERR_UNSUPPORTED; }
+    pl.lds_scene = want == PT_EXTEND_LDS || (want == PT_EXTEND_AUTO && class_bytes <= 24 * 1024);
     pl.variant = pl.lds_scene ? PT_EXTEND_LDS : PT_EXTEND_HBM;
     pl.lds_stack = pl.lds_scene ? LDS_STACK : 12;
     pl.spill = !(pl.lds_scene && s->stack_need <= 16u && s->n_tris <= 2047u && s->n_wide <= 8191u);
     if (!pl.spill) pl.lds_stack = (int)std::max(s->stack_need, 1u);
     pl.pairs = !pl.spill && s->pair_leaves && ctx->tune.pair_kernel != 0;
     pl.smem_wide_entries = (size_t)pl.lds_stack * TB * sizeof(uint2) + (pl.lds_scene ? scene_bytes : 0);
-    pl.smem = pl.spill ? pl.smem_wide_entries : (size_t)pl.lds_stack * TB * sizeof(uint32_t) + scene_bytes;
+    pl.smem = pl.spill ? pl.smem_wide_entries : compact_stack_bytes(TB, pl.lds_stack) + scene_bytes;
     const auto kernel_of = [&](bool compact, bool count, bool shadow) {
         return pl.lds_scene ? reinterpret_cast<const void *>(pick_extend_lds(compact, pl.pairs, count, shadow)) : ptw_extend_hbm_fn(count, ctx->tune.rec64 != 0);
     };
diff --git a/single-file-vulkan-pathtracing_amd/csrc/fused.hip b/single-file-vulkan-pathtracing_amd/csrc/fused.hip
--- a/single-file-vulkan-pathtracing_amd/csrc/fused.hip
+++ b/single-file-vulkan-pathtracing_amd/csrc/fused.hip
@@ -119,9 +119,8 @@
                    "kernels' class: <= 2047 triangles in <= 24 KB, stack bound <= 16, tmin > 0)";
         return PT_ERR_UNSUPPORTED;
     }
-    fp.lds_stack = pl.lds_stack + 1;
-    fp.smem = (size_t)fp.lds_stack * FTB * sizeof(uint32_t) + lds_scene_bytes(s->n_wide, s->n_tris) + tables +
-              sizeof(uint32_t) * FS_FIELDS * FTB + sizeof(uint32_t) * (FTB / 64) * PT_FUSED_WTILES;
+    fp.lds_stack = pl.lds_stack;
+    fp.smem = fused_lds(s->n_wide, s->n_tris, (uint32_t)fp.lds_stack).extra;
     fp.pairs = pl.pairs;
     fp.block = FTB;
     int per_cu = 0;
diff --git a/single-file-vulkan-pathtracing_amd/csrc/fused_inst_kernel.h b/single-file-vulkan-pathtracing_amd/csrc/fused_inst_kernel.h
--- a/single-file-vulkan-pathtracing_amd/csrc/fused_inst_kernel.h
+++ b/single-file-vulkan-pathtracing_amd/csrc/fused_inst_kernel.h
@@ -38,8 +38,10 @@
     uint32_t *s_stack = reinterpret_cast<uint32_t *>(smem);
     uint32_t *s_blas = s_stack + (size_t)lds_stack * FITB;
     float4 *s_tri = reinterpret_cast<float4 *>(s_blas + (size_t)I16_NODE_DW * (n_blas_wide + n_tlas_lds));
-    float4 *s_shade = s_tri + 9 * (size_t)n_tris;
-    lds_u32 *my_state = (lds_u32 *)reinterpret_cast<uint32_t *>(s_shade + 3 * (size_t)n_tris) + threadIdx.x;
+    constexpr size_t SHADE_F4 = 3;
+    static_assert(lds_tris_bytes(1) == 9 * sizeof(float4) && SHADE_F4 >= ptl::D_FIRST_OVERREAD_F4, "k_fused_inst: s_shade directly behind s_tri (pair_leaf.h LOAD_D_FIRST)");
+    float4 *s_shade = s_tri + lds_tris_bytes(n_tris) / sizeof(float4);
+    lds_u32 *my_state = (lds_u32 *)reinterpret_cast<uint32_t *>(s_shade + SHADE_F4 * (size_t)n_tris) + threadIdx.x;
     for (uint32_t i = threadIdx.x; i < 4 * n_tlas_lds; i += FITB)
         *reinterpret_cast<uint4 *>(s_blas + (size_t)(n_blas_wide + (i >> 2)) * I16_NODE_DW + 4 * (i & 3u)) = tlas16[i];
     for (uint32_t i = threadIdx.x; i < 4 * n_blas_wide; i += FITB) {
diff --git a/single-file-vulkan-pathtracing_amd/csrc/fused_kernel.h b/single-file-vulkan-pathtracing_amd/csrc/fused_kernel.h
--- a/single-file-vulkan-pathtracing_amd/csrc/fused_kernel.h
+++ b/single-file-vulkan-pathtracing_amd/csrc/fused_kernel.h
@@ -24,6 +24,29 @@
 #ifndef PT_FUSED_WAVES_NEE
 #define PT_FUSED_WAVES_NEE 4
 #endif
+
+struct FusedLds { uint32_t wide, tri, shade, frame, stack, state, wtile, extra; };
+__host__ __device__ constexpr FusedLds fused_lds(uint32_t n_wide, uint32_t n_tris, uint32_t stack_levels)
+{
+    FusedLds l{};
+    l.wide = 0u;
+    l.tri = l.wide + (uint32_t)lds_nodes_bytes(n_wide);
+    l.shade = l.tri + (uint32_t)lds_tris_bytes(n_tris);
+    l.frame = l.shade + (uint32_t)sizeof(float4) * 3u * n_tris;
+    l.state = l.frame + (uint32_t)sizeof(float4) * 2u * n_tris;
+    l.wtile = l.state + (uint32_t)sizeof(uint32_t) * FS_FIELDS * FTB;
+    l.stack = l.wtile + (uint32_t)sizeof(uint32_t) * (FTB / 64) * PT_FUSED_WTILES;
+    l.extra = l.stack + (uint32_t)compact_stack_bytes(FTB, stack_levels);
+    return l;
+}
+constexpr bool fused_lds_covers_leaf_read(uint32_t n_wide, uint32_t n_tris)
+{
+    const FusedLds l = fused_lds(n_wide, n_tris, 1u);
+    return l.shade == l.tri + lds_tris_bytes(n_tris) && l.frame - l.shade >= sizeof(float4) * ptl::D_FIRST_OVERREAD_F4 && l.wide == 0u &&
+           l.stack >= l.state + sizeof(uint32_t) * FTB + 4u;
+}
+static_assert(fused_lds_covers_leaf_read(1, 1) && fused_lds_covers_leaf_read(1, 2) && fused_lds_covers_leaf_read(21, 36) && fused_lds_covers_leaf_read(85, 85),
+              "k_fused: s_shade directly behind s_tri (pair_leaf.h LOAD_D_FIRST), tables at LDS byte 0");
 
 #ifndef PT_FUSED_NODE_EXIT
 #define PT_FUSED_NODE_EXIT 3
@@ -89,11 +112,12 @@
         light_area = ptm::own_sgprs(light_area_arg);
     }
     extern __shared__ __attribute__((aligned(16))) char smem[];
-    float4 *s_wide = reinterpret_cast<float4 *>(smem + (size_t)lds_stack * FTB * sizeof(uint32_t));
-    float4 *s_tri = s_wide + LDS_NODE_F4 * (size_t)n_wide;
-    float4 *s_shade = s_tri + 9 * (size_t)n_tris;
-    float4 *s_frame = s_shade + 3 * (size_t)n_tris;
-    lds_u32 *my_state = (lds_u32 *)reinterpret_cast<uint32_t *>(s_frame + 2 * (size_t)n_tris) + threadIdx.x;
+    const FusedLds lds = fused_lds(n_wide, n_tris, (uint32_t)lds_stack);
+    float4 *s_wide = reinterpret_cast<float4 *>(smem + lds.wide);
+    float4 *s_tri = reinterpret_cast<float4 *>(smem + lds.tri);
+    float4 *s_shade = reinterpret_cast<float4 *>(smem + lds.shade);
+    float4 *s_frame = reinterpret_cast<float4 *>(smem + lds.frame);
+    lds_u32 *my_state = (lds_u32 *)reinterpret_cast<uint32_t *>(smem + lds.state) + threadIdx.x;
     lds_stage_nodes<FTB, true>(s_wide, g_wide, n_wide);
     lds_stage_tris<FTB, true>(s_tri, g_tri4, n_tris, s_shade, g_shade4);
     for (uint32_t i = threadIdx.x; i < 2 * n_tris; i += FTB) s_frame[i] = g_frame4[i];
@@ -101,19 +125,21 @@
     const float4 *wide = s_wide, *tri4 = s_tri;
     const float4 *verts = s_tri + 6 * (size_t)n_tris;
 
-    lds_u32 *my_stack32 = (lds_u32 *)reinterpret_cast<uint32_t *>(smem) + FTB + threadIdx.x;
+    LaneStack<FTB> stk((lds_u32 *)reinterpret_cast<uint32_t *>(smem + lds.stack) - FTB + threadIdx.x);
+    stk.arm_bottom();
+    stk.park();
     const int lane = threadIdx.x & 63;
 
     FusedDev dev;
     dev.kernel_begin();
-    lds_u32 *s_fb = (lds_u32 *)reinterpret_cast<uint32_t *>(s_frame + 2 * (size_t)n_tris) + FS_FIELDS * FTB + (FTB / 64) * PT_FUSED_WTILES + (threadIdx.x >> 6) * (2 * FB_N);
+    auto fb_of_wave = [&]() -> lds_u32 * { return (lds_u32 *)reinterpret_cast<uint32_t *>(smem + lds.extra) + (threadIdx.x >> 6) * (2 * FB_N); };
     if constexpr (COUNT) {
-        if (lane < 2 * FB_N) s_fb[lane] = 0u;
+        if (lane < 2 * FB_N) fb_of_wave()[lane] = 0u;
     }
 #define PT_FB(B)                                                                                        \
     if constexpr (COUNT) {                                                                              \
         const unsigned long long m_fb = __ballot(1);                                                    \
-        if (lane == __ffsll((long long)m_fb) - 1) { s_fb[2 * (B)] += 1u; s_fb[2 * (B) + 1] += (uint32_t)__popcll(m_fb); } \
+        if (lane == __ffsll((long long)m_fb) - 1) { lds_u32 *s_fb = fb_of_wave(); s_fb[2 * (B)] += 1u; s_fb[2 * (B) + 1] += (uint32_t)__popcll(m_fb); } \
     }
     bool out_of_slots = false;
     uint32_t n_rays_wave = 0;
@@ -123,43 +149,41 @@
     bool w_tails = false;
     const uint32_t n_tail_slots = HYB ? rc.lanes_active * rc.tail * rc.slots_per_lane : 0u;
     const uint32_t part_len = ((n_slots + PT_FUSED_PARTS - 1) / PT_FUSED_PARTS + 63u) & ~63u;
-    lds_u32 *s_wtile = (lds_u32 *)reinterpret_cast<uint32_t *>(s_frame + 2 * (size_t)n_tris) + FS_FIELDS * FTB + (threadIdx.x >> 6) * PT_FUSED_WTILES;
-    lds_u32 *my_nee = (lds_u32 *)reinterpret_cast<uint32_t *>(s_frame + 2 * (size_t)n_tris) + FS_FIELDS * FTB + (FTB / 64) * PT_FUSED_WTILES + threadIdx.x;
+    lds_u32 *s_wtile = (lds_u32 *)reinterpret_cast<uint32_t *>(smem + lds.wtile) + (threadIdx.x >> 6) * PT_FUSED_WTILES;
+    lds_u32 *my_nee = (lds_u32 *)reinterpret_cast<uint32_t *>(smem + lds.extra) + threadIdx.x;
     ptm::f3 inv{}, invf{}, on{}, of{}, orgp{};
     ptm::RayPre pre{};
     uint32_t ax = 0, ay = 0, az = 0, tri_base = 0;
     float best_t = tmax, best_V = 0.f, best_W = 0.f, best_det = 1.f;
     uint32_t best_pos = PT_MISS;
     uint32_t cur = DONE;
-    int sp = -1;
 
     constexpr uint32_t PENDING = 0xFFFFFFFFu;
     auto pop_pending = [&](uint32_t r) -> uint32_t {
         while (__ballot(r == PENDING)) {
             if (r == PENDING) {
                 PT_FB(FB_POP)
-                sp--;
-                const uint32_t e = my_stack32[sp * FTB];
-                const uint32_t miss = sp == 0 ? DONE : PENDING;
-                r = __uint_as_float(e & 0xFFFFC000u) <= best_t ? (e & 0x3FFFu) : miss;
+                const uint32_t e = stk.pop();
+                r = !(__uint_as_float(e & 0xFFFFC000u) > best_t) ? (e & 0x3FFFu) : PENDING;
             }
         }
         return r;
     };
-    auto pop = [&]() -> uint32_t { return pop_pending(sp > 0 ? PENDING : DONE); };
+    auto pop = [&]() -> uint32_t { return pop_pending(PENDING); };
 
     for (;;) {
         PT_FB(FB_ITER)
-        const bool have = cur != DONE, path = sp >= 0;
+        const bool have = cur != DONE, path = !stk.parked();
         const unsigned long long m_have = __ballot(have), m_path = __ballot(path);
         const unsigned long long m_in_blk = ~m_have & (out_of_slots ? m_path : ~0ull);
-        const bool in_blk = !have && (path || !out_of_slots);
         const int n_work = __popcll(m_in_blk);
         if (n_work && n_work * 64 >= refill * (n_work + __popcll(m_have))) {
             uint32_t slot = 0, ctr = 0, seed = 0, pxy = 0;
             float wr = 0.f, wg = 0.f, wb = 0.f;
             ptm::f3 org{}, dir{};
+            const bool in_blk = !have && (path || !out_of_slots);
             bool got_ray = false, need_primary = false, bounce = false;
+            bool freed = false;
             bool shadow = false;
             uint32_t bpos = 0u;
             float4 nc{};
@@ -259,15 +283,17 @@
                         if (!logs) rad.color[slot] = make_float4(__uint_as_float(my_state[FS_A * FTB]), __uint_as_float(my_state[FS_B * FTB]),
                                                                    __uint_as_float(my_state[FS_C * FTB]), 0.f);
                         else if (!dbg_no_nterm) rad.nterm[lslot] = my_state[FS_A * FTB];
-                        sp = -1;
+                        stk.park();
+                        freed = true;
                         dev.slot_end(slot);
                     }
                 }
                 ctr = sample | (depth << 16);
             }
-            const unsigned long long m_want = __ballot(in_blk && sp < 0);
+            const bool wants = in_blk && (!path || freed);
+            const unsigned long long m_want = __ballot(wants);
             if (m_want && !out_of_slots) {
-                if (in_blk && sp < 0) { PT_FB(FB_HANDOUT) }
+                if (wants) { PT_FB(FB_HANDOUT) }
                 if (w_next >= w_end) {
                     PT_FB(FB_DRAW)
                     for (;;) {
@@ -317,7 +343,7 @@
                 const uint32_t take = min((uint32_t)__popcll(m_want), w_end - w_next);
                 const uint32_t rank = (uint32_t)__popcll(m_want & ((1ull << lane) - 1ull));
                 uint32_t cull_n = 0u;
-                if (in_blk && sp < 0 && rank < take) {
+                if (wants && rank < take) {
                     PT_FB(FB_TAKE)
                     const uint32_t mine = w_next + rank;
                     uint32_t f, g, local;
@@ -352,7 +378,7 @@
                         my_state[FS_A * FTB] = 0u;
                         if (!GROUPED) { my_state[FS_B * FTB] = 0u; my_state[FS_C * FTB] = 0u; }
                         my_state[FS_MB * FTB] = (uint32_t)((int32_t)rc.spp * (rc.frame_base + (int32_t)f)) + 1u;
-                        sp = 0;
+                        stk.clear_to_bottom();
                         need_primary = true;
                         dev.slot_begin();
                     } else if (GROUPED) {
@@ -428,16 +454,16 @@
                 pre = ptm::ray_setup<true>(org, dir);
                 inv = { ptm::safe_inv(dir.x), ptm::safe_inv(dir.y), ptm::safe_inv(dir.z) };
                 slab_setup(org, inv, invf, on, of);
-                ax = inv.x < 0.f ? 48u : 0u;
-                ay = inv.y < 0.f ? 48u : 0u;
-                az = inv.z < 0.f ? 48u : 0u;
+                ax = inv.x < 0.f ? LDS_NEG_AXIS : 0u;
+                ay = inv.y < 0.f ? LDS_NEG_AXIS : 0u;
+                az = inv.z < 0.f ? LDS_NEG_AXIS : 0u;
                 tri_base = (uint32_t)pre.kz * 3u * n_tris;
                 orgp = { ptm::sel3(pre.kz, org.y, org.z, org.x), ptm::sel3(pre.kz, org.z, org.x, org.y), ptm::sel3(pre.kz, org.x, org.y, org.z) };
                 best_t = (NEE && shadow) ? nc.w : tmax;
                 best_V = 0.f; best_W = 0.f; best_det = 1.f;
                 best_pos = PT_MISS;
                 cur = 0u;
-                sp = 0;
+                stk.clear_to_bottom();
             }
             const uint32_t n_started = (uint32_t)__popcll(__ballot(got_ray));
             n_rays_wave += n_started;
@@ -445,7 +471,7 @@
         }
         const bool tracing = cur != DONE;
         const unsigned long long m_tracing = __ballot(tracing);
-        if (m_tracing == 0ull && __ballot(sp >= 0) == 0ull && out_of_slots) break;
+        if (m_tracing == 0ull && __ballot(!stk.parked()) == 0ull && out_of_slots) break;
 
         const int n_have = __popcll(m_tracing);
         if (tracing) { PT_FB(FB_TRACE) }
@@ -456,14 +482,10 @@
                 do {
                     if (dn) {
                         PT_FB(FB_NODE)
-                        const uint32_t e_top = my_stack32[(sp - 1) * FTB];
-                        cur = compact_node_step<FTB>(wide, cur, inv, invf, on, of, ax, ay, az, tmin, best_t, my_stack32, sp, [&]() -> uint32_t {
+                        cur = compact_node_step<FTB>(wide, cur, inv, invf, on, of, ax, ay, az, tmin, best_t, stk, [&](uint32_t e_top) -> uint32_t {
                             PT_FB(FB_POPTOP)
-                            const bool any = sp > 0;
-                            sp -= any ? 1 : 0;
-                            const uint32_t below = sp > 0 ? PENDING : DONE;
-                            const uint32_t top = __uint_as_float(e_top & 0xFFFFC000u) <= best_t ? (e_top & 0x3FFFu) : below;
-                            return pop_pending(any ? top : DONE);
+                            stk.drop();
+                            return pop_pending(!(__uint_as_float(e_top & 0xFFFFC000u) > best_t) ? (e_top & 0x3FFFu) : PENDING);
                         });
                     }
                     dn = cur < LEAF_BIT;
@@ -481,7 +503,7 @@
                                             [[maybe_unused]] const bool closer =
                                                 ptl::closer_single_level(tri4, tri_base, t, V, W, det, pos, best_t, best_V, best_W, best_det, best_pos);
                                             if constexpr (NEE) {
-                                                if (closer && my_nee[FS_NEE_POS * FTB] != PT_MISS) sp = 0;
+                                                if (closer && my_nee[FS_NEE_POS * FTB] != PT_MISS) stk.clear_to_bottom();
                                             }
                                         },
                                         [&] { PT_FB(FB_DIV) });
@@ -498,7 +520,7 @@
                                 closer = best_pos == PT_MISS || __float_as_uint(a.w) < __float_as_uint(tri4[(size_t)tri_base + 3 * (size_t)best_pos].w);
                             if (closer) {
                                 best_t = t; best_V = V; best_W = W; best_det = det; best_pos = pos;
-                                if (NEE && my_nee[FS_NEE_POS * FTB] != PT_MISS) sp = 0;
+                                if (NEE && my_nee[FS_NEE_POS * FTB] != PT_MISS) stk.clear_to_bottom();
                             }
                         }
                     }
@@ -514,7 +536,7 @@
     if (lane == 0 && n_cull_wave) atomicAdd(stats + 19, (unsigned long long)n_cull_wave);
     dev.kernel_end(lane, n_rays_wave, FTB);
     if constexpr (COUNT) {
-        if (lane < 2 * FB_N) atomicAdd(stats + PT_N_STATS + lane, (unsigned long long)s_fb[lane]);
+        if (lane < 2 * FB_N) atomicAdd(stats + PT_N_STATS + lane, (unsigned long long)fb_of_wave()[lane]);
     }
 #undef PT_FB
 }
diff --git a/single-file-vulkan-pathtracing_amd/csrc/lds_scene.h b/single-file-vulkan-pathtracing_amd/csrc/lds_scene.h
--- a/single-file-vulkan-pathtracing_amd/csrc/lds_scene.h
+++ b/single-file-vulkan-pathtracing_amd/csrc/lds_scene.h
@@ -4,15 +4,21 @@
 
 namespace {
 
-constexpr uint32_t LDS_NODE_F4 = 9;
+constexpr uint32_t LDS_NODE_F4 = 10;
+constexpr uint32_t LDS_NODE_AXIS_F4 = 3;
+constexpr uint32_t LDS_NODE_CW_F4 = 9;
+constexpr uint32_t LDS_NODE128_F4 = 9;
 constexpr uint32_t C14_LEAF = 0x2000u, C14_DONE = 0x3FFFu;
 constexpr uint32_t I16_EXIT = 0x7FFFu, I16_DONE = 0xFFFFu, I16_LEAF = 0x8000u;
 constexpr uint32_t I16_NODE_DW = 20;
 
 __host__ __device__ constexpr size_t lds_nodes_bytes(size_t n_wide) { return 16 * LDS_NODE_F4 * n_wide; }
+__host__ __device__ constexpr size_t lds_nodes128_bytes(size_t n_wide) { return 16 * LDS_NODE128_F4 * n_wide; }
 __host__ __device__ constexpr size_t lds_nodes16_bytes(size_t n_nodes) { return sizeof(uint32_t) * I16_NODE_DW * n_nodes; }
 __host__ __device__ constexpr size_t lds_tris_bytes(size_t n_tris) { return sizeof(float4) * 9 * n_tris; }
 __host__ __device__ constexpr size_t lds_scene_bytes(size_t n_wide, size_t n_tris) { return lds_nodes_bytes(n_wide) + lds_tris_bytes(n_tris); }
+__host__ __device__ constexpr size_t lds_scene128_bytes(size_t n_wide, size_t n_tris) { return lds_nodes128_bytes(n_wide) + lds_tris_bytes(n_tris); }
+__host__ __device__ constexpr size_t lds_class_bytes(size_t n_wide, size_t n_tris) { return lds_nodes128_bytes(n_wide) + lds_tris_bytes(n_tris); }
 __host__ __device__ constexpr size_t lds_scene16_bytes(size_t n_wide, size_t n_tris) { return lds_nodes16_bytes(n_wide) + lds_tris_bytes(n_tris); }
 
 template <int BLOCK, bool COMPACT>
@@ -20,16 +26,30 @@
 {
     for (uint32_t i = threadIdx.x; i < 8 * n_wide; i += BLOCK) {
         float4 v = g_wide[i];
-        if (COMPACT && (i & 7u) == 6u) {
-            auto cw = [](float f) {
-                const uint32_t w = __float_as_uint(f);
-                const uint32_t c = (w & PT_LEAF) ? (C14_LEAF | (((w >> 28) & 3u) << 11) | (w & 0x7FFu)) : (w & 0x1FFFu);
-                return __uint_as_float(w == SENTINEL ? C14_DONE : c);
-            };
-            v = make_float4(cw(v.x), cw(v.y), cw(v.z), cw(v.w));
+        const uint32_t f = i & 7u;
+        float4 *nd = s_wide + (i >> 3) * LDS_NODE_F4;
+        if (f < 3u) {
+            nd[LDS_NODE_AXIS_F4 * f] = v;
+            nd[LDS_NODE_AXIS_F4 * f + 2u] = v;
+        } else if (f < 6u) {
+            nd[LDS_NODE_AXIS_F4 * (f - 3u) + 1u] = v;
+        } else if (f == 6u) {
+            if (COMPACT) {
+                auto cw = [](float c_) {
+                    const uint32_t w = __float_as_uint(c_);
+                    const uint32_t c = (w & PT_LEAF) ? (C14_LEAF | (((w >> 28) & 3u) << 11) | (w & 0x7FFu)) : (w & 0x1FFFu);
+                    return __uint_as_float(w == SENTINEL ? C14_DONE : c);
+                };
+                v = make_float4(cw(v.x), cw(v.y), cw(v.z), cw(v.w));
+            }
+            nd[LDS_NODE_CW_F4] = v;
         }
-        s_wide[(i >> 3) * LDS_NODE_F4 + (i & 7u)] = v;
     }
+}
+template <int BLOCK>
+__device__ __forceinline__ void lds_stage_nodes128(float4 *s_wide, const float4 *g_wide, uint32_t n_wide)
+{
+    for (uint32_t i = threadIdx.x; i < 8 * n_wide; i += BLOCK) s_wide[(i >> 3) * LDS_NODE128_F4 + (i & 7u)] = g_wide[i];
 }
 
 __device__ __forceinline__ uint32_t lds_code16(uint32_t w)
diff --git a/single-file-vulkan-pathtracing_amd/csrc/pair_leaf.h b/single-file-vulkan-pathtracing_amd/csrc/pair_leaf.h
--- a/single-file-vulkan-pathtracing_amd/csrc/pair_leaf.h
+++ b/single-file-vulkan-pathtracing_amd/csrc/pair_leaf.h
@@ -3,6 +3,7 @@
 
 namespace ptl {
 
+constexpr unsigned D_FIRST_OVERREAD_F4 = 3;
 template <bool LOAD_D_FIRST = false, class Accept, class HitBlock>
 __device__ __forceinline__ void pair_leaf_test(const float4 *tri4, size_t ti, bool two, uint32_t first, const ptm::RayPre &pre,
                                                const ptm::f3 &orgp, float tmin, float tmax, Accept &&accept, HitBlock &&hit_block)
```

Result: faster. 60130 Mrays/s, median of 6 (+2.6%).
